# zkHubHQ/distributed-groth16

Hardware: AMD Instinct MI355X
Metric: groth16_constraints_per_sec (higher is better)
Workload: dtype u32; 1 GPU; BN254 Groth16 prove from the matrices, synthetic R1CS with 2^20 - 2 constraints (3 nonzeros per row of A and B), 2^20 wires, 2 instance variables; r, s != 0 (R1CS x witness + 6 NTTs of 2^20 + 4 G1 MSMs + 1 G2 MSM); proving key RESIDENT as window tables (built once per key outside the timed region); curve=bn254, log_domain=20, parallelism=single GPU, key_table_bytes=6039807360, key_table_stride=1

## Files before the change

### distributed-groth16_amd/csrc/capi.hip

```cpp
#include <stdio.h>
#include <stdlib.h>
#include <string.h>

#include "bounds.h"
#include "ctx.h"

using namespace dg16;

namespace dg16 {
size_t fq_bytes(int curve) { return curve == DG16_BN254 ? 32 : 48; }
size_t affine_bytes(int curve, int group) { return 2 * fq_bytes(curve) * (group == 2 ? 2 : 1); }
#ifdef DG16_BOUNDS
unsigned* bounds_sink_device() {
  static unsigned* sink = [] {
    unsigned* p = nullptr;
    if (hipMalloc((void**)&p, kBoundsWords * sizeof(unsigned)) != hipSuccess) return (unsigned*)nullptr;
    (void)hipMemset(p, 0, kBoundsWords * sizeof(unsigned));
    return p;
  }();
  return sink;
}
#endif
static void check_curve_group(int curve, int group) {
  DG_REQUIRE(curve >= 0 && curve <= 2, DG16_ERR_BAD_CURVE, "unknown curve id");
  DG_REQUIRE(group == 1 || group == 2, DG16_ERR_BAD_ARG, "group must be 1 (G1) or 2 (G2)");
}
}

extern "C" {

int dg16_ctx_create(int device, dg16_ctx** out) {
  if (!out) return DG16_ERR_BAD_ARG;
  *out = nullptr;
  dg16_ctx* ctx = new dg16_ctx();
  int rc = guarded(ctx, [&] {
    int count = 0;
    DG_HIP(hipGetDeviceCount(&count));
    DG_REQUIRE(count > 0, DG16_ERR_HIP, "no HIP device visible: libdg16 has no CPU path");
    DG_REQUIRE(device >= 0 && device < count, DG16_ERR_BAD_ARG, "device index out of range");
    DG_HIP(hipSetDevice(device));
    hipDeviceProp_t p;
    DG_HIP(hipGetDeviceProperties(&p, device));
    ctx->device = device;
    ctx->compute_units = p.multiProcessorCount;
    ctx->name = p.gcnArchName;
    int prio_lo = 0, prio_hi = 0;
    DG_HIP(hipDeviceGetStreamPriorityRange(&prio_lo, &prio_hi));
    for (int i = 0; i < kChannels; i++) {
      DG_HIP(hipStreamCreateWithPriority(&ctx->ch[i].own, hipStreamNonBlocking, i > 0 ? prio_hi : prio_lo));
      ctx->ch[i].cur = ctx->ch[i].own;
      for (int e = 0; e < 4; e++) DG_HIP(hipEventCreate(&ctx->ch[i].ev[e]));
    }
    for (auto& e : ctx->pipe_ev) DG_HIP(hipEventCreateWithFlags(&e, hipEventDisableTiming));
    DG_HIP(hipStreamCreateWithPriority(&ctx->aux[0], hipStreamNonBlocking, prio_hi));
    DG_HIP(hipHostMalloc((void**)&ctx->dev_flag_host, sizeof(unsigned), hipHostMallocMapped));
    *ctx->dev_flag_host = 0;
    DG_HIP(hipHostGetDevicePointer((void**)&ctx->dev_flag, ctx->dev_flag_host, 0));
    DG_HIP(hipMalloc((void**)&ctx->kclk, kChannels * 2 * sizeof(unsigned long long)));
    DG_HIP(hipMemset(ctx->kclk, 0, kChannels * 2 * sizeof(unsigned long long)));
  });
  if (rc != DG16_OK) {
    static thread_local std::string last;
    last = ctx->err;
    delete ctx;
    return rc;
  }
  *out = ctx;
  return DG16_OK;
}

void dg16_ctx_destroy(dg16_ctx* ctx) {
  if (!ctx) return;
  hipSetDevice(ctx->device);
  hipDeviceSynchronize();
  for (int i = 0; i < kChannels; i++) {
    for (int s = 0; s < kSlots; s++)
      if (ctx->ch[i].slot[s]) hipFree(ctx->ch[i].slot[s]);
    for (int e = 0; e < 4; e++)
      if (ctx->ch[i].ev[e]) hipEventDestroy(ctx->ch[i].ev[e]);
    if (ctx->ch[i].own) hipStreamDestroy(ctx->ch[i].own);
  }
  for (auto& x : ctx->xws)
    for (int s = 0; s < kSlots; s++)
      if (x.slot[s]) hipFree(x.slot[s]);
  for (auto& e : ctx->pipe_ev)
    if (e) hipEventDestroy(e);
  for (auto& st : ctx->aux)
    if (st) hipStreamDestroy(st);
  if (ctx->dev_flag_host) hipHostFree(ctx->dev_flag_host);
  if (ctx->kclk) hipFree(ctx->kclk);
  for (auto& kv : ctx->twiddles) {
    hipFree(kv.second.lo);
    hipFree(kv.second.hi);
    if (kv.second.hi_scaled) hipFree(kv.second.hi_scaled);
    hipFree(kv.second.small);
    hipFree(kv.second.n_inv);
    for (void* q : {kv.second.lo_i, kv.second.hi_i, kv.second.hi_scaled_i, kv.second.small_i, kv.second.n_inv_i,
                    kv.second.full[0], kv.second.full[1], kv.second.shift_full})
      if (q) hipFree(q);
  }
  delete ctx;
}

const char* dg16_last_error(dg16_ctx* ctx) {
  if (!ctx) return "null context";
  std::lock_guard<std::mutex> g(ctx->mu);
  static thread_local std::string copy;
  copy = ctx->err;
  return copy.c_str();
}

int dg16_set_stream(dg16_ctx* ctx, int channel, void* hip_stream) {
  int rc = guard_channel(ctx, channel);
  if (rc) return rc;
  std::lock_guard<std::mutex> g(ctx->ch[channel].mu);
  ctx->ch[channel].cur = hip_stream ? (hipStream_t)hip_stream : ctx->ch[channel].own;
  return DG16_OK;
}

int dg16_sync(dg16_ctx* ctx, int channel) {
  int rc = guard_channel(ctx, channel);
  if (rc) return rc;
  return guarded(ctx, [&] {
    DG_HIP(hipSetDevice(ctx->device));
    DG_HIP(hipStreamSynchronize(ctx->ch[channel].cur));
    if (ctx->dev_flag_host && *ctx->dev_flag_host) {
      const unsigned f = *ctx->dev_flag_host;
      *ctx->dev_flag_host = 0;
      throw StatusError{DG16_ERR_BAD_ARG, f & 1 ? "dg16_qap: coefficient out of range (column >= num_vars or bad row_ptr)"
                                                : "device-side argument check failed"};
    }
#ifdef DG16_BOUNDS
    if (unsigned* sink = bounds_sink_device()) {
      unsigned rec[kBoundsWords] = {};
      DG_HIP(hipDeviceSynchronize());
      DG_HIP(hipMemcpy(rec, sink, sizeof rec, hipMemcpyDeviceToHost));
      if (rec[0]) {
        DG_HIP(hipMemset(sink, 0, sizeof rec));
        char msg[256];
        snprintf(msg, sizeof msg, "DG16_BOUNDS: %u violation(s); first: site %u index %llu limit %llu (workgroup %u, lane %u)", rec[0],
                 rec[1], (unsigned long long)(rec[2] | ((uint64_t)rec[3] << 32)),
                 (unsigned long long)(rec[4] | ((uint64_t)rec[5] << 32)), rec[6], rec[7]);
        fprintf(stderr, "[dg16] %s\n", msg);
        throw StatusError{DG16_ERR_HIP, msg};
      }
    }
#endif
  });
}

int dg16_device_info(dg16_ctx* ctx, char* name, size_t name_len, int* compute_units) {
  if (!ctx) return DG16_ERR_BAD_ARG;
  if (name && name_len) {
    strncpy(name, ctx->name.c_str(), name_len - 1);
    name[name_len - 1] = 0;
  }
  if (compute_units) *compute_units = ctx->compute_units;
  return DG16_OK;
}

int dg16_last_kernel_ms(dg16_ctx* ctx, int channel, int which, float* ms) {
  int rc = guard_channel(ctx, channel);
  if (rc) return rc;
  if (!ms || which < 0 || which > 2) return DG16_ERR_BAD_ARG;
  return guarded(ctx, [&] {
    Channel& c = ctx->ch[channel];
    std::lock_guard<std::mutex> g(c.mu);
    *ms = 0.f;
    if (which == 2) {
      if (!c.ev_valid[1] || !ctx->kclk) return;
      DG_HIP(hipSetDevice(ctx->device));
      DG_HIP(hipEventSynchronize(c.ev[3]));
      unsigned long long t[2] = {0, 0};
      DG_HIP(hipMemcpy(t, ctx->kclk + 2 * channel, sizeof t, hipMemcpyDeviceToHost));
      if (t[1]) *ms = (float)((double)t[0] / (double)t[1] * 100.0);
      return;
    }
    if (!c.ev_valid[which]) return;
    DG_HIP(hipSetDevice(ctx->device));
    hipEvent_t a = c.ev[which == 0 ? 0 : 2], b = c.ev[which == 0 ? 1 : 3];
    DG_HIP(hipEventSynchronize(b));
    DG_HIP(hipEventElapsedTime(ms, a, b));
  });
}

int dg16_field_op(dg16_ctx* ctx, int field_id, int op, const void* a, const void* b, void* out,
                  size_t n, unsigned flags, int channel) {
  int rc = guard_channel(ctx, channel);
  if (rc) return rc;
  return guarded(ctx, [&] {
    int curve = field_id & 15;
    DG_REQUIRE((field_id & ~16) >= 0 && curve <= 2 && (field_id >> 4) <= 1, DG16_ERR_BAD_CURVE,
               "field id must be curve (Fq) or 16 + curve (Fr)");
    DG_REQUIRE(op >= 0 && op <= 7, DG16_ERR_BAD_ARG, "unknown field op");
    DG_REQUIRE(a && out && (b || op >= 3), DG16_ERR_BAD_ARG, "null operand");
    bool dev = flags & DG16_F_DEVICE_PTRS;
    size_t eb = (field_id & 16) ? 32 : fq_bytes(curve);
    Call k(ctx, channel);
// ... 331 lines not shown
```

### distributed-groth16_amd/csrc/ctx.h

```cpp
#pragma once
#include <hip/hip_runtime.h>
#include <stdint.h>

#include <map>
#include <atomic>
#include <mutex>
#include <string>
#include <vector>

#include "../../include/dg16.h"

namespace dg16 {

constexpr int kChannels = 3;
constexpr int kSlots = 32;

struct Channel {
  hipStream_t own = nullptr;
  hipStream_t cur = nullptr;
  std::mutex mu;
  void* slot[kSlots] = {};
  size_t slot_bytes[kSlots] = {};
  hipEvent_t ev[4] = {};
  bool ev_valid[2] = {false, false};
};

struct TwiddleKey {
  int curve;
  unsigned log_n;
  int inverse;
  bool operator<(const TwiddleKey& o) const {
    if (curve != o.curve) return curve < o.curve;
    if (log_n != o.log_n) return log_n < o.log_n;
    return inverse < o.inverse;
  }
};
struct TwiddleSet {
  void* lo = nullptr;
  void* hi = nullptr;
  void* hi_scaled = nullptr;
  void* small = nullptr;
  void* n_inv = nullptr;
  unsigned lb = 0, sm = 0;
  void *lo_i = nullptr, *hi_i = nullptr, *hi_scaled_i = nullptr, *small_i = nullptr, *n_inv_i = nullptr;
  void* full[2] = {nullptr, nullptr};
  void* shift_full = nullptr;
  bool shift_full_tried = false;
};

}

struct dg16_ctx {
  int device = 0;
  int compute_units = 0;
  std::string name;
  dg16::Channel ch[dg16::kChannels];
  std::mutex mu;
  std::mutex mpc_mu;
  std::string err;
  hipEvent_t pipe_ev[24] = {};
  std::atomic<bool> tail_pending{false};
  hipStream_t aux[1] = {};
  dg16::Channel xws[2];
  unsigned* dev_flag_host = nullptr;
  unsigned* dev_flag = nullptr;
  unsigned long long* kclk = nullptr;
  size_t table_budget = 0;
  std::map<dg16::TwiddleKey, dg16::TwiddleSet> twiddles;
};

struct dg16_bases {
  dg16_ctx* ctx = nullptr;
  int curve = 0, group = 1;
  size_t n = 0;
  unsigned c = 0, nwin = 0;
  unsigned stride = 1;
  void* table = nullptr;
  size_t bytes = 0;
};

namespace dg16 {

struct StatusError {
  int code;
  std::string msg;
};

#define DG_HIP(expr)                                                                        \
  do {                                                                                      \
    hipError_t e_ = (expr);                                                                 \
    if (e_ != hipSuccess)                                                                   \
      throw dg16::StatusError{e_ == hipErrorOutOfMemory ? DG16_ERR_OOM : DG16_ERR_HIP,      \
                              std::string(#expr) + ": " + hipGetErrorString(e_)};           \
  } while (0)

#define DG_REQUIRE(cond, code, text)                                                        \
  do {                                                                                      \
    if (!(cond)) throw dg16::StatusError{code, text};                                       \
  } while (0)

inline void* ws(Channel& c, int slot, size_t bytes) {
  if (bytes == 0) bytes = 16;
  if (c.slot_bytes[slot] < bytes) {
    if (c.slot[slot]) {
      DG_HIP(hipDeviceSynchronize());
      DG_HIP(hipFree(c.slot[slot]));
      c.slot[slot] = nullptr;
      c.slot_bytes[slot] = 0;
    }
    size_t want = bytes + bytes / 8;
    DG_HIP(hipMalloc(&c.slot[slot], want));
    c.slot_bytes[slot] = want;
  }
  return c.slot[slot];
}

struct Call {
  dg16_ctx* ctx;
  Channel& c;
  std::unique_lock<std::mutex> lk;
  Call(dg16_ctx* ctx_, int channel, bool tail_ok = false)
      : ctx(ctx_), c(ctx_->ch[channel]), lk(ctx_->ch[channel].mu) {
    DG_HIP(hipSetDevice(ctx->device));
    if (!tail_ok && ctx->tail_pending.load(std::memory_order_acquire))
      DG_HIP(hipStreamWaitEvent(c.cur, ctx->pipe_ev[18], 0));
    c.ev_valid[0] = c.ev_valid[1] = false;
    DG_HIP(hipEventRecord(c.ev[0], c.cur));
  }
  void begin_dominant() { DG_HIP(hipEventRecord(c.ev[2], c.cur)); }
  void end_dominant() {
    DG_HIP(hipEventRecord(c.ev[3], c.cur));
    c.ev_valid[1] = true;
  }
  void finish() {
    DG_HIP(hipEventRecord(c.ev[1], c.cur));
    c.ev_valid[0] = true;
  }
  hipStream_t s() const { return c.cur; }
};

inline int guard_channel(dg16_ctx* ctx, int channel) {
  if (!ctx) return DG16_ERR_BAD_ARG;
  if (channel < 0 || channel >= kChannels) {
    std::lock_guard<std::mutex> g(ctx->mu);
    ctx->err = "channel must be 0..2";
    return DG16_ERR_BAD_ARG;
  }
  return DG16_OK;
}

template <class Fn>
int guarded(dg16_ctx* ctx, Fn&& fn) {
  try {
    fn();
    return DG16_OK;
  } catch (const StatusError& e) {
    if (ctx) {
      std::lock_guard<std::mutex> g(ctx->mu);
      ctx->err = e.msg;
    }
    return e.code;
  } catch (const std::exception& e) {
    if (ctx) {
      std::lock_guard<std::mutex> g(ctx->mu);
      ctx->err = e.what();
    }
    return DG16_ERR_HIP;
  } catch (...) {
    return DG16_ERR_HIP;
  }
}

inline const void* stage_in(Call& k, int slot, const void* p, size_t bytes, bool device_ptrs) {
  if (device_ptrs || bytes == 0) return p;
  void* d = ws(k.c, slot, bytes);
  DG_HIP(hipMemcpyAsync(d, p, bytes, hipMemcpyHostToDevice, k.s()));
  return d;
}
inline void stage_out(Call& k, void* host_dst, const void* dev_src, size_t bytes, bool device_ptrs) {
  if (device_ptrs) {
    if (host_dst != dev_src) DG_HIP(hipMemcpyAsync(host_dst, dev_src, bytes, hipMemcpyDeviceToDevice, k.s()));
  } else {
    DG_HIP(hipMemcpyAsync(host_dst, dev_src, bytes, hipMemcpyDeviceToHost, k.s()));
  }
}

void field_op_launch(Call& k, int field_id, int op, const void* a, const void* b, void* out, size_t n);
void qap_launch(Call& k, int curve, const unsigned* a_ptr, const unsigned* a_col, const void* a_val,
                const unsigned* b_ptr, const unsigned* b_col, const void* b_val, const void* w, bool w_mont, size_t nc,
                size_t ni, size_t nv, size_t m, size_t row_start, size_t row_stride, void* a, void* b, void* c);
void h_poly_dist_stage(Call& k, int curve, unsigned log_m, unsigned rank, unsigned n_ranks, int stage,
                       const void* const* in, void* out);
void h_poly_dist_launch(Call& k, int curve, const dg16_comm* comm, const void* a, const void* b, const void* c,
                        unsigned log_m, void* out);
void ntt_dist_stage(Call& k, int curve, unsigned log_n_total, unsigned rank, unsigned n_ranks, int inverse, int stage,
                    const void* in, void* out);
void ntt_dist_launch(Call& k, int curve, const dg16_comm* comm, const void* in, void* out, unsigned log_n_total,
                     int inverse);
void ntt_launch(Call& k, int curve, void* data, unsigned log_n, int inverse, const void* coset_host);
void h_poly_launch(Call& k, int curve, const void* a, const void* b, const void* c, unsigned log_m,
                   void* out);
bool net_is_rccl(const dg16_net* net);
inline unsigned msm_mode(unsigned flags) {
  return ((flags & DG16_F_SCALARS_MONT) ? 1u : 0u) | ((flags & DG16_F_BASES_IN_SUBGROUP) ? 2u : 0u);
}
void msm_launch(Call& k, int curve, int group, const void* bases, const void* scalars, size_t n,
                unsigned mode, bool out_affine, void* out_dev);
// ... 11 lines not shown
```

### distributed-groth16_amd/csrc/msm_group.hip

```cpp
#include "msm_impl.h"
#include "dist_impl.h"

#define DG_CAT2(a, b) a##b
#define DG_CAT(a, b) DG_CAT2(a, b)
#define DG_FN(stem) DG_CAT(stem, DG_NAME)

namespace dg16 {
using CT = CurveTypes<DG_CURVE>;
#if DG_GROUP == 1
using GF = CT::Fq;
using GC = CT::G1c;
#else
using GF = CT::Fq2;
using GC = CT::G2c;
#endif

template void msm_accumulate_phase<GF>(hipStream_t, const MsmSort&, const MsmBuffers<GF>&, const void* const*);
template void msm_finalize_phase<GF>(hipStream_t, const MsmSort&, const MsmBuffers<GF>&);
template void msm_tail_phase<GF>(hipStream_t, const MsmSort&, const MsmBuffers<GF>&, bool, void*);
template void* msm_build_table<GF>(hipStream_t, const void*, size_t, unsigned, unsigned);
template MsmSort msm_sort_on<CT::Fr, CT::SCALAR_BITS>(hipStream_t, Channel&, const void*, size_t, unsigned, bool, unsigned,
                                                      unsigned);

void DG_FN(msm_)(Call& k, const void* bases, const void* scalars, size_t n, unsigned mode, bool affine, void* out) {
  msm_run<GF, CT::Fr, CT::SCALAR_BITS>(k, bases, scalars, n, mode, affine, out);
}
void DG_FN(gen_bases_)(Call& k, uint64_t seed, size_t n, void* out) { gen_bases_run<GF, GC>(k, seed, n, out); }
void DG_FN(to_affine_)(Call& k, const void* jac, void* out, size_t n) { to_affine_run<GF>(k, jac, out, n); }

void* DG_FN(bases_table_)(Call& k, const void* bases_dev, size_t n, size_t budget, unsigned* c_out, unsigned* rows_out,
                          unsigned* stride_out) {
  const unsigned c = msm_window_bits(n ? n : 1, true, CT::SCALAR_BITS);
  const unsigned nwin = (CT::SCALAR_BITS + 1 + c - 1) / c;
  const unsigned stride = table_stride_for((size_t)nwin * (n ? n : 1) * sizeof(Affine<GF>), budget, nwin);
  const unsigned rows = (nwin + stride - 1) / stride;
  *c_out = c;
  *rows_out = rows;
  *stride_out = stride;
  return msm_build_table<GF>(k.s(), bases_dev, n, c * stride, rows);
}
void DG_FN(msm_resident_)(Call& k, const void* table, size_t n, unsigned c, unsigned stride, const void* scalars,
                          bool mont, bool affine, void* out) {
  MsmSort st = msm_sort<CT::Fr, CT::SCALAR_BITS>(k, scalars, n, mont, true, c, stride);
  msm_reduce<GF>(k, st, table, affine, out);
}

template <class F, class Fr>
__global__ void __launch_bounds__(512) matvec_points_wave_kernel(const Fr* __restrict__ Mc, unsigned rows, unsigned cols,
                                                                   const Affine<F>* __restrict__ in,
                                                                   Affine<F>* __restrict__ out) {
  __shared__ ScalarMulLds<F> lds[8];
  __shared__ XYZZ29<F> part[8];
  const unsigned wave = threadIdx.x >> 6, lane = threadIdx.x & 63;
  const size_t e = blockIdx.x / rows;
  const unsigned r = blockIdx.x % rows;
  __builtin_amdgcn_s_setprio(DG16_CHAIN_PRIO);
  {
    const Affine<F> q = in[e * cols + wave];
    XYZZ29<F> v = XYZZ29<F>::inf();
    if (!q.is_inf()) v = XYZZ29<F>::from_xyzz32(XYZZ<F>::from_affine(q));
    const Fr k = Mc[(size_t)r * cols + wave];
    v = scalar_mul_wave29<F, Fr::NL, false>(v, k.l, &lds[wave]);
    if (lane == 0) part[wave] = v;
  }
  __syncthreads();
  if (wave != 0) return;
  const Affine<F> acc = sum_points_affine_wave<F>(part, cols);
  if (lane == 0) out[blockIdx.x] = acc;
}
template <class F, class Fr>
static void matvec_points(hipStream_t s, const Fr* Mc, unsigned rows, unsigned cols, const Affine<F>* in, Affine<F>* out,
                          size_t count) {
  if (count * rows <= 256 && cols >= 1 && cols <= 8)
    hipLaunchKernelGGL((matvec_points_wave_kernel<F, Fr>), dim3((unsigned)(count * rows)), dim3(64 * cols), 0, s, Mc, rows, cols,
                       in, out);
  else
    hipLaunchKernelGGL((matvec_points_kernel<F, Fr>), dim3((unsigned)((count * rows + 63) / 64)), dim3(64), 0, s, Mc, rows,
                       cols, in, out, count);
}

void DG_FN(d_msm_)(Call& k, const dg16_pss* pp, const dg16_net* net, int sid, const void* bases, const void* scalars,
                   size_t n, unsigned mode, void* out_jac, const void* table, unsigned table_c, unsigned table_stride) {
  const bool mont = mode & 1u;
  using F = GF;
  using Fr = CT::Fr;
  const unsigned np = pp->n;
  Affine<F>* c_share = (Affine<F>*)ws(k.c, 18, sizeof(Affine<F>));
  if (table)
    DG_FN(msm_resident_)(k, table, n, table_c, table_stride, scalars, mont, true, c_share);
  else
    msm_run<F, Fr, CT::SCALAR_BITS>(k, bases, scalars, n, mode, true, c_share);
  const bool king = net->party_id(net->self) == 0;
  Affine<F>* shares = king ? (Affine<F>*)ws(k.c, 19, np * sizeof(Affine<F>)) : nullptr;
  if (net->gather_to_king(net->self, sid, c_share, sizeof(Affine<F>), shares, k.s()) != DG16_OK)
    throw StatusError{DG16_ERR_NET, "send_to_king failed"};
  Affine<F>* send = nullptr;
  if (king) {
    send = (Affine<F>*)ws(k.c, 20, np * sizeof(Affine<F>));
    const Fr* v2 = (const Fr*)pp->mats + 6 * pp->n * pp->l;
    matvec_points<F, Fr>(k.s(), v2, 1u, np, shares, send, (size_t)1);
    for (unsigned p = 1; p < np; p++)
      DG_HIP(hipMemcpyAsync(send + p, send, sizeof(Affine<F>), hipMemcpyDeviceToDevice, k.s()));
    DG_HIP(hipGetLastError());
  }
  Affine<F>* got = (Affine<F>*)ws(k.c, 21, sizeof(Affine<F>));
  if (net->scatter_from_king(net->self, sid, send, sizeof(Affine<F>), got, k.s()) != DG16_OK)
    throw StatusError{DG16_ERR_NET, "recv_from_king failed"};
  hipLaunchKernelGGL(affine_to_jacobian_kernel<F>, dim3(1), dim3(1), 0, k.s(), got, (Jacobian<F>*)out_jac);
  DG_HIP(hipGetLastError());
}
template <class F, class Fr>
__global__ void __launch_bounds__(512) mpc_combine_kernel(const Jacobian<F>* __restrict__ terms,
                                                           const Fr* __restrict__ scalars, unsigned n_terms,
                                                           unsigned mask, int mont, Jacobian<F>* __restrict__ out) {
  __shared__ XYZZ29<F> part[8];
  __shared__ ScalarMulLds<F> lds[8];
  const unsigned wave = threadIdx.x >> 6, lane = threadIdx.x & 63;
  XYZZ29<F> v = XYZZ29<F>::from_xyzz32(XYZZ<F>::from_jacobian(terms[wave]));
  {
    Fr kk = Fr::zero();
    kk.l[0] = 1;
    if ((mask >> wave) & 1) {
      kk = scalars[wave];
      if (mont) kk = kk.from_mont();
    }
    v = scalar_mul_wave29<F, Fr::NL, false>(v, kk.l, &lds[wave]);
  }
  if (lane == 0) part[wave] = v;
  __syncthreads();
  if (wave != 0) return;
  const XYZZ29<F> acc = sum_points_wave<F>(part, n_terms);
  if (lane == 0) *out = acc.to_xyzz32().to_jacobian();
}
void DG_FN(mpc_combine_)(Call& k, const void* terms, const void* scalars, unsigned n_terms, unsigned mask, bool mont,
                         void* out_jac) {
  DG_REQUIRE(n_terms >= 1 && n_terms <= 8, DG16_ERR_BAD_ARG, "mpc_combine: 1..8 terms");
  hipLaunchKernelGGL((mpc_combine_kernel<GF, CT::Fr>), dim3(1), dim3(64 * n_terms), 0, k.s(), (const Jacobian<GF>*)terms,
                     (const CT::Fr*)scalars, n_terms, mask, (int)mont, (Jacobian<GF>*)out_jac);
  DG_HIP(hipGetLastError());
}
void DG_FN(affine_to_jac_)(Call& k, const void* aff, void* jac) {
  hipLaunchKernelGGL(affine_to_jacobian_kernel<GF>, dim3(1), dim3(1), 0, k.s(), (const Affine<GF>*)aff, (Jacobian<GF>*)jac);
  DG_HIP(hipGetLastError());
}
void DG_FN(packexp_)(Call& k, const dg16_pss* pp, int which, const void* in, size_t count, void* out) {
  using F = GF;
  using Fr = CT::Fr;
  const unsigned cols = which == 0 ? pp->l : pp->n, rows = which == 0 ? pp->n : pp->l;
  const Fr* Mc = (const Fr*)pp->mats + 3 * pp->n * pp->l + (size_t)which * pp->n * pp->l;
  matvec_points<F, Fr>(k.s(), Mc, rows, cols, (const Affine<F>*)in, (Affine<F>*)out, count);
  DG_HIP(hipGetLastError());
}
}
```

### distributed-groth16_amd/csrc/msm_impl.h

```cpp
#pragma once
#include <atomic>
#include <utility>
#include "glv.h"
#include <stdio.h>

#include <chrono>

#include "bounds.h"
#include "ctx.h"
#include "ec29.h"
#include "lane29.h"
#include "types.h"

#ifndef DG16_CHAIN_PRIO
#define DG16_CHAIN_PRIO 3
#endif
namespace dg16 {

constexpr unsigned kMinSegLog = 3, kMaxSegLog = 9;
constexpr unsigned kMinLanesLog = 18;
constexpr unsigned kGiantSegs = 64;
constexpr unsigned kGiantSlices = 64;
constexpr unsigned kGiantSliceSegs = 512;

// ... 126 lines not shown
      v >>= off;
    }
    int d = (int)((unsigned)v & ((1u << c) - 1)) + (int)carry;
    if ((unsigned)d > half) { d -= (int)(1u << c); carry = 1; } else { carry = 0; }
    if (flip) d = -d;
    if (live) digits[(size_t)w * n + i] = d;
    unsigned b = d ? (unsigned)(d < 0 ? -d : d) - 1 : 0u;
    unsigned slot = ((w % g.bw) << g.log_nb) + b;
    wave_atomic_inc(counts, slot, live && d != 0);
  }
}

constexpr unsigned kScanBlock = 4096;
template <int TU>
__global__ void __launch_bounds__(1024) msm_scan_local_kernel(const unsigned* __restrict__ counts,
                                                               unsigned* __restrict__ offsets,
                                                               unsigned* __restrict__ seg_off,
                                                               unsigned* __restrict__ block_tot, unsigned log_nb,
                                                               unsigned seg_log) {
  __shared__ unsigned sh[1024];
  __shared__ unsigned sh2[1024];
  const unsigned nb = 1u << log_nb;
  const unsigned seg_round = (1u << seg_log) - 1;
  const size_t base = (size_t)blockIdx.y << log_nb;
  const unsigned lo = blockIdx.x * kScanBlock + threadIdx.x * 4;
  unsigned cn[4], sum = 0, ssum = 0;
#pragma unroll
  for (unsigned j = 0; j < 4; j++) {
    cn[j] = (lo + j < nb) ? counts[base + lo + j] : 0;
    sum += cn[j];
    ssum += (cn[j] + seg_round) >> seg_log;
  }
  sh[threadIdx.x] = sum;
  sh2[threadIdx.x] = ssum;
  __syncthreads();
  for (unsigned d = 1; d < 1024; d <<= 1) {
    unsigned v = threadIdx.x >= d ? sh[threadIdx.x - d] : 0;
    unsigned v2 = threadIdx.x >= d ? sh2[threadIdx.x - d] : 0;
    __syncthreads();
    sh[threadIdx.x] += v;
    sh2[threadIdx.x] += v2;
    __syncthreads();
  }
  unsigned run = sh[threadIdx.x] - sum, srun = sh2[threadIdx.x] - ssum;
#pragma unroll
  for (unsigned j = 0; j < 4; j++)
    if (lo + j < nb) {
      offsets[base + lo + j] = run;
      seg_off[base + lo + j] = srun;
      run += cn[j];
      srun += (cn[j] + seg_round) >> seg_log;
    }
  if (threadIdx.x == 1023) {
    size_t t = ((size_t)blockIdx.y * gridDim.x + blockIdx.x) * 2;
    block_tot[t] = sh[1023];
    block_tot[t + 1] = sh2[1023];
  }
}
template <int TU>
__global__ void __launch_bounds__(1024) msm_scan_tops_kernel(unsigned* __restrict__ block_tot, unsigned nblocks,
                                                              unsigned* __restrict__ seg_total) {
  __shared__ unsigned sh[1024];
  __shared__ unsigned sh2[1024];
  unsigned* t = block_tot + (size_t)blockIdx.x * nblocks * 2;
  unsigned a = threadIdx.x < nblocks ? t[threadIdx.x * 2] : 0;
  unsigned b = threadIdx.x < nblocks ? t[threadIdx.x * 2 + 1] : 0;
  sh[threadIdx.x] = a;
  sh2[threadIdx.x] = b;
  __syncthreads();
  for (unsigned d = 1; d < 1024; d <<= 1) {
    unsigned v = threadIdx.x >= d ? sh[threadIdx.x - d] : 0;
    unsigned v2 = threadIdx.x >= d ? sh2[threadIdx.x - d] : 0;
    __syncthreads();
    sh[threadIdx.x] += v;
    sh2[threadIdx.x] += v2;
    __syncthreads();
  }
  if (threadIdx.x < nblocks) {
    t[threadIdx.x * 2] = sh[threadIdx.x] - a;
    t[threadIdx.x * 2 + 1] = sh2[threadIdx.x] - b;
  }
  if (threadIdx.x == 1023) seg_total[blockIdx.x] = sh2[1023];
}
template <int TU>
__global__ void __launch_bounds__(1024) msm_scan_fix_kernel(unsigned* __restrict__ offsets,
                                                             unsigned* __restrict__ seg_off,
                                                             unsigned* __restrict__ cursor,
                                                             const unsigned* __restrict__ block_tot, unsigned log_nb) {
  const unsigned nb = 1u << log_nb;
  const size_t base = (size_t)blockIdx.y << log_nb;
  const size_t t = ((size_t)blockIdx.y * gridDim.x + blockIdx.x) * 2;
  const unsigned add = block_tot[t], sadd = block_tot[t + 1];
  const unsigned lo = blockIdx.x * kScanBlock + threadIdx.x * 4;
#pragma unroll
  for (unsigned j = 0; j < 4; j++)
    if (lo + j < nb) {
      offsets[base + lo + j] += add;
      seg_off[base + lo + j] += sadd;
      cursor[base + lo + j] = 0;
    }
}

template <int TU>
__global__ void __launch_bounds__(256) msm_scatter_kernel(const int* __restrict__ digits, size_t n, MsmGeom g,
                                                           const unsigned* __restrict__ offsets,
                                                           const unsigned* __restrict__ seg_off,
                                                           unsigned* __restrict__ cursor,
                                                           unsigned* __restrict__ entries) {
  size_t i = (size_t)blockIdx.x * blockDim.x + threadIdx.x;
  const bool live = i < n;
  const unsigned w = blockIdx.y;
  int d = live ? digits[(size_t)w * n + i] : 0;
  const bool act = d != 0;
  unsigned b = act ? (unsigned)(d < 0 ? -d : d) - 1 : 0u;
  const unsigned bwin = w % g.bw;
  unsigned slot = (bwin << g.log_nb) + b;
  unsigned rank = wave_atomic_inc(cursor, slot, act);
  if (!act) return;
  unsigned ref = (unsigned)((size_t)(w / g.bw) * n + i);
  entries[DG_IDX(15, (size_t)bwin * g.region + offsets[slot] + rank, (size_t)g.bw * g.region)] = ref | (d < 0 ? 0x80000000u : 0u);
}

constexpr unsigned kPartScalars = 1024;
constexpr unsigned kPartMax = 256;
constexpr unsigned kPartMaxLowBits = 12;
constexpr unsigned kPartTileLog = 11;
constexpr unsigned kPartBlocks = 32;

struct PartGeom {
  unsigned low_bits, nparts, nblk1;
};

template <class Fr>
__device__ __forceinline__ int msm_digit(const Fr& s, unsigned w, unsigned c, unsigned& carry) {
  const unsigned half = 1u << (c - 1);
  unsigned bit = w * c;
  unsigned limb = bit >> 5, off = bit & 31;
  uint64_t v = 0;
  if (limb < (unsigned)Fr::NL) {
    v = s.l[limb];
    if (limb + 1 < (unsigned)Fr::NL) v |= (uint64_t)s.l[limb + 1] << 32;
    v >>= off;
  }
  int d = (int)((unsigned)v & ((1u << c) - 1)) + (int)carry;
  if ((unsigned)d > half) { d -= (int)(1u << c); carry = 1; } else { carry = 0; }
  return d;
}

template <class Fr>
__global__ void __launch_bounds__(256) msm_part_hist_kernel(const Fr* __restrict__ scalars, size_t n, int mont,
                                                             MsmGeom g, PartGeom pg,
                                                             unsigned* __restrict__ blockhist) {
  __shared__ unsigned hist[kPartMax];
  hist[threadIdx.x] = 0;
  __syncthreads();
  for (unsigned k = 0; k < kPartScalars / 256; k++) {
    size_t i = (size_t)blockIdx.x * kPartScalars + k * 256 + threadIdx.x;
    if (i >= n) continue;
    Fr s = scalars[i];
    if (mont & 1) s = s.from_mont();
    unsigned carry = 0;
    for (unsigned w = 0; w < g.nwin; w++) {
      int d = msm_digit(s, w, g.c, carry);
      if (d == 0) continue;
      unsigned slot = ((w % g.bw) << g.log_nb) + (unsigned)(d < 0 ? -d : d) - 1;
      atomicAdd(&hist[slot >> pg.low_bits], 1u);
    }
  }
  __syncthreads();
  if (threadIdx.x < pg.nparts) blockhist[(size_t)threadIdx.x * pg.nblk1 + blockIdx.x] = hist[threadIdx.x];
}

template <class Fr>
__global__ void __launch_bounds__(256) msm_part_scatter_kernel(const Fr* __restrict__ scalars, size_t n, int mont,
                                                                MsmGeom g, PartGeom pg,
                                                                const unsigned* __restrict__ blockoff,
                                                                uint2* __restrict__ part) {
  __shared__ unsigned cur[kPartMax];
  if (threadIdx.x < pg.nparts) cur[threadIdx.x] = blockoff[(size_t)threadIdx.x * pg.nblk1 + blockIdx.x];
  __syncthreads();
  for (unsigned k = 0; k < kPartScalars / 256; k++) {
    size_t i = (size_t)blockIdx.x * kPartScalars + k * 256 + threadIdx.x;
    if (i >= n) continue;
    Fr s = scalars[i];
    if (mont & 1) s = s.from_mont();
    const bool flip = (mont & 2) && (s.l[Fr::NL - 1] >> 31);
    unsigned carry = 0;
    for (unsigned w = 0; w < g.nwin; w++) {
      int d = msm_digit(s, w, g.c, carry);
      if (d == 0) continue;
      unsigned slot = ((w % g.bw) << g.log_nb) + (unsigned)(d < 0 ? -d : d) - 1;
      unsigned ref = (unsigned)((size_t)(w / g.bw) * n + i);
      unsigned pos = atomicAdd(&cur[slot >> pg.low_bits], 1u);
      part[DG_IDX(14, pos, (size_t)g.nwin * n)] = make_uint2(ref | (((d < 0) != flip) ? 0x80000000u : 0u), slot);
    }
  }
}

template <int TU>
__global__ void __launch_bounds__(1024) scan_chunk_kernel(unsigned* __restrict__ a, size_t len,
                                                           unsigned* __restrict__ tot) {
  __shared__ unsigned sh[1024];
  const size_t lo = (size_t)blockIdx.x * 4096 + threadIdx.x * 4;
  unsigned v[4], sum = 0;
#pragma unroll
  for (unsigned j = 0; j < 4; j++) {
    v[j] = lo + j < len ? a[lo + j] : 0;
    sum += v[j];
  }
  sh[threadIdx.x] = sum;
  __syncthreads();
  for (unsigned d = 1; d < 1024; d <<= 1) {
    unsigned t = threadIdx.x >= d ? sh[threadIdx.x - d] : 0;
    __syncthreads();
    sh[threadIdx.x] += t;
    __syncthreads();
  }
  unsigned run = sh[threadIdx.x] - sum;
#pragma unroll
  for (unsigned j = 0; j < 4; j++)
    if (lo + j < len) {
      a[lo + j] = run;
      run += v[j];
    }
  if (threadIdx.x == 1023) tot[blockIdx.x] = sh[1023];
}
template <int TU>
__global__ void __launch_bounds__(1024) scan_tops_kernel(unsigned* __restrict__ tot, unsigned nchunks) {
  __shared__ unsigned sh[1024];
  const unsigned per = (nchunks + 1023) / 1024;
  const unsigned lo = threadIdx.x * per;
  unsigned sum = 0;
  for (unsigned j = 0; j < per; j++)
    if (lo + j < nchunks) sum += tot[lo + j];
  sh[threadIdx.x] = sum;
  __syncthreads();
  for (unsigned d = 1; d < 1024; d <<= 1) {
    unsigned t = threadIdx.x >= d ? sh[threadIdx.x - d] : 0;
    __syncthreads();
    sh[threadIdx.x] += t;
    __syncthreads();
  }
  unsigned run = sh[threadIdx.x] - sum;
  for (unsigned j = 0; j < per; j++)
    if (lo + j < nchunks) {
      unsigned t = tot[lo + j];
      tot[lo + j] = run;
      run += t;
    }
}
template <int TU>
__global__ void __launch_bounds__(1024) scan_add_kernel(unsigned* __restrict__ a, size_t len,
                                                         const unsigned* __restrict__ tot) {
  const size_t lo = (size_t)blockIdx.x * 4096 + threadIdx.x * 4;
  const unsigned add = tot[blockIdx.x];
#pragma unroll
  for (unsigned j = 0; j < 4; j++)
    if (lo + j < len) a[lo + j] += add;
}

template <int TU>
__global__ void __launch_bounds__(256) msm_part_count_kernel(const uint2* __restrict__ part,
                                                              const unsigned* __restrict__ blockoff, PartGeom pg,
                                                              unsigned* __restrict__ counts) {
  __shared__ unsigned hist[1u << kPartMaxLowBits];
  const unsigned p = blockIdx.y;
  const unsigned lo = blockoff[(size_t)p * pg.nblk1];
  const unsigned size = blockoff[(size_t)(p + 1) * pg.nblk1] - lo;
  if (((size_t)blockIdx.x << kPartTileLog) >= size) return;
  const unsigned nlow = 1u << pg.low_bits;
  for (unsigned b = threadIdx.x; b < nlow; b += 256) hist[b] = 0;
  __syncthreads();
  for (size_t t = (size_t)blockIdx.x << kPartTileLog; t < size; t += (size_t)gridDim.x << kPartTileLog)
    for (unsigned j = 0; j < (1u << kPartTileLog) / 256; j++) {
      size_t idx = t + j * 256 + threadIdx.x;
      if (idx < size) atomicAdd(&hist[part[lo + idx].y & (nlow - 1)], 1u);
    }
  __syncthreads();
  for (unsigned b = threadIdx.x; b < nlow; b += 256)
    if (hist[b]) atomicAdd(&counts[((size_t)p << pg.low_bits) + b], hist[b]);
}

template <int TU>
__global__ void __launch_bounds__(256) msm_part_place_kernel(const uint2* __restrict__ part,
                                                              const unsigned* __restrict__ blockoff, PartGeom pg,
                                                              MsmGeom g, const unsigned* __restrict__ offsets,
                                                              const unsigned* __restrict__ seg_off,
                                                              unsigned* __restrict__ cursor,
                                                              unsigned* __restrict__ entries) {
  __shared__ unsigned cnt[1u << kPartMaxLowBits];
  __shared__ unsigned rank0[1u << kPartMaxLowBits];
  __shared__ unsigned dst0[1u << kPartMaxLowBits];
  const unsigned p = blockIdx.y;
  const unsigned lo = blockoff[(size_t)p * pg.nblk1];
  const unsigned size = blockoff[(size_t)(p + 1) * pg.nblk1] - lo;
  if (((size_t)blockIdx.x << kPartTileLog) >= size) return;
  const unsigned nlow = 1u << pg.low_bits;
  constexpr unsigned PER = (1u << kPartTileLog) / 256;
  for (size_t t = (size_t)blockIdx.x << kPartTileLog; t < size; t += (size_t)gridDim.x << kPartTileLog) {
    for (unsigned b = threadIdx.x; b < nlow; b += 256) cnt[b] = 0;
    __syncthreads();
    uint2 e[PER];
    unsigned lr[PER];
#pragma unroll
    for (unsigned j = 0; j < PER; j++) {
      size_t idx = t + j * 256 + threadIdx.x;
      e[j] = make_uint2(0u, 0xFFFFFFFFu);
      if (idx < size) {
        e[j] = part[lo + idx];
        lr[j] = atomicAdd(&cnt[e[j].y & (nlow - 1)], 1u);
      }
    }
    __syncthreads();
    for (unsigned b = threadIdx.x; b < nlow; b += 256)
      if (cnt[b]) {
        const size_t slot = ((size_t)p << pg.low_bits) + b;
        rank0[b] = atomicAdd(&cursor[slot], cnt[b]);
        dst0[b] = (unsigned)((slot >> g.log_nb) * g.region) + offsets[slot];
      }
    __syncthreads();
#pragma unroll
    for (unsigned j = 0; j < PER; j++) {
      if (e[j].y == 0xFFFFFFFFu) continue;
      const unsigned slot = e[j].y, b = slot & (nlow - 1);
      const unsigned rank = rank0[b] + lr[j];
      entries[DG_IDX(13, dst0[b] + rank, (size_t)g.bw * g.region)] = e[j].x;
    }
    __syncthreads();
  }
}

template <class F>
__device__ __forceinline__ Affine29<F> load_internal(const uint32_t* __restrict__ bases, unsigned idx) {
  constexpr int PW = 2 * FieldOf<F>::WORDS;
  uint32_t w[PW];
  const uint4* src = reinterpret_cast<const uint4*>(bases + (size_t)idx * PW);
#pragma unroll
  for (int i = 0; i < PW / 4; i++) {
    const uint4 v = src[i];
    w[4 * i] = v.x; w[4 * i + 1] = v.y; w[4 * i + 2] = v.z; w[4 * i + 3] = v.w;
  }
  return Affine29<F>::load(w);
}

template <class F>
struct RawPoint {
  uint4 v[2 * FieldOf<F>::WORDS / 4];
};
template <class F>
__device__ __forceinline__ RawPoint<F> load_raw(const uint32_t* __restrict__ bases, unsigned idx) {
  constexpr int PW = 2 * FieldOf<F>::WORDS;
  RawPoint<F> r;
  const uint4* src = reinterpret_cast<const uint4*>(bases + (size_t)idx * PW);
#pragma unroll
  for (int i = 0; i < PW / 4; i++) r.v[i] = src[i];
  return r;
}
template <class F>
__device__ __forceinline__ Affine29<F> unpack_raw(const RawPoint<F>& r) {
  constexpr int PW = 2 * FieldOf<F>::WORDS;
  uint32_t w[PW];
#pragma unroll
  for (int i = 0; i < PW / 4; i++) {
    w[4 * i] = r.v[i].x; w[4 * i + 1] = r.v[i].y; w[4 * i + 2] = r.v[i].z; w[4 * i + 3] = r.v[i].w;
  }
  return Affine29<F>::load(w);
}

struct SegRange {
  size_t bslot;
  unsigned first, cnt;
  unsigned j, k;
};
__device__ __forceinline__ SegRange msm_segment(const MsmGeom& g, unsigned w, unsigned t,
                                                const unsigned* __restrict__ counts,
                                                const unsigned* __restrict__ seg_off) {
  const unsigned* so = seg_off + ((size_t)w << g.log_nb);
  unsigned lo = 0, hi = 1u << g.log_nb;
  while (hi - lo > 1) {
    const unsigned mid = (lo + hi) >> 1;
    if (so[mid] <= t) lo = mid; else hi = mid;
  }
  SegRange r;
  r.bslot = DG_IDX(1, ((size_t)w << g.log_nb) + lo, (size_t)g.bw << g.log_nb);
  const unsigned c = counts[r.bslot];
  const unsigned k = (c + (1u << g.seg_log) - 1) >> g.seg_log;
  const unsigned j = t - so[lo];
  r.first = (unsigned)(((uint64_t)j * c) / k);
  r.cnt = (unsigned)(((uint64_t)(j + 1) * c) / k) - r.first;
  r.j = j;
  r.k = k;
  return r;
}

__device__ __forceinline__ unsigned msm_nparts(unsigned first_slot, unsigned k, unsigned wg_log) {
  return k ? ((first_slot + k - 1) >> wg_log) - (first_slot >> wg_log) + 1 : 0;
}
__device__ __forceinline__ unsigned msm_part_slot(unsigned first_slot, unsigned s, unsigned wg_log) {
  return s ? ((first_slot >> wg_log) + s) << wg_log : first_slot;
}
template <class F, int BLOCK>
struct ColAcc {
  using S = typename FieldOf<F>::Store;
  static constexpr int WORDS = sizeof(S) / 4;
  uint32_t (*sh)[BLOCK];
  unsigned lane;
  __device__ __forceinline__ S get(int coord) const {
    S v;
    uint32_t* w = reinterpret_cast<uint32_t*>(&v);
#pragma unroll
    for (int i = 0; i < WORDS; i++) w[i] = sh[coord * WORDS + i][lane];
    return v;
  }
  __device__ __forceinline__ void put(int coord, const S& v) const {
    const uint32_t* w = reinterpret_cast<const uint32_t*>(&v);
#pragma unroll
    for (int i = 0; i < WORDS; i++) sh[coord * WORDS + i][lane] = w[i];
  }
};
template <class F, int BLOCK>
#ifdef DG16_TREE_ADD_OUTLINE
__device__ __attribute__((noinline))
#else
__device__ __forceinline__
#endif
void wg_tree_add(uint32_t (*sh)[BLOCK], unsigned a, unsigned b) {
#ifdef DG16_TREE_ADD_INTO
  XYZZ29<F>::add_into(ColAcc<F, BLOCK>{sh, a}, ColAcc<F, BLOCK>{sh, b});
#else
  XYZZ29<F>::add_acc(ColAcc<F, BLOCK>{sh, a}, ColAcc<F, BLOCK>{sh, a}, ColAcc<F, BLOCK>{sh, b});
#endif
}
template <class F, int BLOCK>
__device__ __forceinline__ void wg_bucket_tree(uint32_t (*sh)[BLOCK], unsigned short* list, unsigned* wcnt,
                                                         unsigned lane, unsigned q, unsigned el) {
  constexpr unsigned NW = BLOCK / 64;
  if (lane == 0) wcnt[NW] = 0;
  __syncthreads();
  atomicMax(&wcnt[NW], el - (lane - q));
  __syncthreads();
  const unsigned maxlen = wcnt[NW];
#pragma unroll 1
  for (unsigned d = 1; d < maxlen; d <<= 1) {
    const bool act = (q & (2 * d - 1)) == 0 && lane + d < el;
    const unsigned long long m = __ballot(act);
    const unsigned wv = lane >> 6;
    if ((lane & 63) == 0) wcnt[wv] = (unsigned)__popcll(m);
    __syncthreads();
    unsigned base = 0, total = 0;
#pragma unroll
    for (unsigned i = 0; i < NW; i++) {
      const unsigned c = wcnt[i];
      base += i < wv ? c : 0u;
      total += c;
    }
    if (act) list[base + (unsigned)__popcll(m & ((1ull << (lane & 63)) - 1))] = (unsigned short)lane;
    __syncthreads();
    if (lane < total) {
      const unsigned a = list[lane];
      wg_tree_add<F, BLOCK>(sh, a, (unsigned)DG_IDX(16, a + d, BLOCK));
    }
    __syncthreads();
  }
}

constexpr unsigned kMaxInst = 4;
struct MsmBases {
  const uint32_t* p[kMaxInst];
};
template <class F>
constexpr bool msm_acc_tree();
template <class F>
constexpr unsigned msm_acc_block_log() {
  if constexpr (sizeof(F) > 48) return sizeof(typename FieldOf<F>::Store) * 4 * 256 <= 80 * 1024 ? 8u : 7u;
  else if constexpr (!msm_acc_tree<F>()) return 8u;
#ifdef DG16_G1_BLOCK_LOG
  else return DG16_G1_BLOCK_LOG;
#else
  else return sizeof(typename FieldOf<F>::Store) * 4 * 256 <= 40 * 1024 ? 8u : 7u;
#endif
}
// ... 868 lines not shown
      w[4] = 0;
      const bool neg_half = ((lane ? h[1][7] : h[0][7]) >> 31) != 0;
      len = wnaf4_words<5>(w, 128, neg_half, lds->naf[lane]);
    }
    __syncthreads();
    {
      Fp<P> beta32;
#pragma unroll
      for (int i = 0; i < Fp<P>::NL; i++) beta32.l[i] = GC::BETA[i];
      const uint32_t beta = FO::template from_regs<XYZZ29<F>::BS>(kc, FieldOf<F>::from32(beta32));
      const uint32_t* src = reinterpret_cast<const uint32_t*>(&lds->tab[kc.row]);
      uint32_t* dst = reinterpret_cast<uint32_t*>(&lds->tab[4 + kc.row]);
      const bool on = kc.l16 < 9u;
      const unsigned i = on ? kc.l16 : 0u;
      const uint32_t bx = lane29::mul(kc, on ? src[i] : 0u, beta);
      if (on) {
        dst[i] = bx;
        dst[9 + i] = src[9 + i];
        dst[18 + i] = src[18 + i];
        dst[27 + i] = src[27 + i];
      }
    }
    len = max(__shfl(len, 0), __shfl(len, 1));
  } else {
    if (lane == 0) len = wnaf4_words<NW>(k, NW * 32, false, lds->naf[0]);
    len = __shfl(len, 0);
  }
  __syncthreads();
  LPt acc = lane29::inf_pt<FO>(kc);
#pragma unroll 1
  for (int i = len - 1; i >= 0; i--) {
    acc = lane29::dbl_pt<FO>(kc, acc);
#pragma unroll 1
    for (int hf = 0; hf < (SPLIT ? 2 : 1); hf++) {
      const int d = lds->naf[hf][i];
      if (d == 0) continue;
      LPt o = lane29::load_pt<F>(kc, &lds->tab[4 * hf + ((d < 0 ? -d : d) >> 1)]);
      if (d < 0) o = lane29::neg_pt<FO>(kc, o);
      acc = lane29::add_pt<FO>(kc, acc, o);
    }
  }
  return p_inf ? p_in : lane29::from_pt<F>(kc, acc);
}
template <class F, int NW>
__device__ __forceinline__ XYZZ29<F> scalar_mul_two_waves_lane29(const XYZZ29<F>& p_in, const uint32_t* k,
                                                                 ScalarMulLds<F>* lds, XYZZ29<F>* xchg) {
  using P = typename FieldOf<F>::Params;
  using GC = typename GlvOf<F>::C;
  using FO = lane29::Ops<F>;
  using LPt = lane29::Pt<FO>;
  static_assert(!FO::EXT, "the endomorphism split of a cofactor-one G1");
  const unsigned lane = __lane_id(), h = (threadIdx.x >> 6) & 1u;
  typename FO::KT kc;
  kc.init();
  const bool p_inf = p_in.is_inf();
  LPt p = lane29::to_pt<F>(kc, p_in);
  if (p_inf) p = {FO::one(kc), FO::one(kc), FO::one(kc), FO::one(kc), false};
  {
    Fp<P> beta32;
#pragma unroll
    for (int i = 0; i < Fp<P>::NL; i++) beta32.l[i] = GC::BETA[i];
    const uint32_t beta = FO::template from_regs<XYZZ29<F>::BS>(kc, FieldOf<F>::from32(beta32));
    if (h) p.x = lane29::mul(kc, p.x, beta);
    const LPt p2 = lane29::dbl_pt<FO>(kc, p);
    LPt m = p;
#pragma unroll 1
    for (int j = 0; j < 4; j++) {
      if (j) m = lane29::add_pt<FO>(kc, m, p2);
      lane29::store_pt_raw<F>(kc, &lds->tab[4 * h + j], m);
    }
  }
  uint32_t hv[2][8];
  glv::split<GC>(k, hv[0], hv[1]);
  int len = 0;
  if (lane == 0) {
    uint32_t w[5];
#pragma unroll
    for (int i = 0; i < 4; i++) w[i] = h ? hv[1][i] : hv[0][i];
    w[4] = 0;
    len = wnaf4_words<5>(w, 128, ((h ? hv[1][7] : hv[0][7]) >> 31) != 0, lds->naf[h]);
  }
  len = __shfl(len, 0);
  __syncthreads();
  LPt acc = lane29::inf_pt<FO>(kc);
#pragma unroll 1
  for (int i = len - 1; i >= 0; i--) {
    acc = lane29::dbl_pt<FO>(kc, acc);
    const int d = lds->naf[h][i];
    if (d == 0) continue;
    LPt o = lane29::load_pt<F>(kc, &lds->tab[4 * h + ((d < 0 ? -d : d) >> 1)]);
    if (d < 0) o = lane29::neg_pt<FO>(kc, o);
    acc = lane29::add_pt<FO>(kc, acc, o);
  }
  if (h == 1) lane29::store_pt_raw<F>(kc, xchg, acc);
  __syncthreads();
  if (h == 0) acc = lane29::add_pt<FO>(kc, acc, lane29::load_pt<F>(kc, xchg));
  return p_inf ? p_in : lane29::from_pt<F>(kc, acc);
}
template <class F>
__device__ __forceinline__ XYZZ29<F> sum_points_wave(const XYZZ29<F>* pts, unsigned n) {
  if constexpr (lane29::enabled<F>()) {
    using FO = lane29::Ops<F>;
    typename FO::KT kc;
    kc.init();
    lane29::Pt<FO> acc = lane29::inf_pt<FO>(kc);
#pragma unroll 1
    for (unsigned i = 0; i < n; i++) acc = lane29::add_pt<FO>(kc, acc, lane29::load_pt<F>(kc, &pts[i]));
    return lane29::from_pt<F>(kc, acc);
  } else {
    XYZZ29<F> acc = XYZZ29<F>::inf();
#pragma unroll 1
    for (unsigned i = 0; i < n; i++) acc = add_wave29(acc, pts[i]);
    return acc;
  }
}

template <class F>
__device__ __forceinline__ Affine<F> sum_points_affine_wave(const XYZZ29<F>* pts, unsigned n) {
  if constexpr (lane29::enabled<F>()) {
    using FO = lane29::Ops<F>;
    typename FO::KT kc;
    kc.init();
    lane29::Pt<FO> acc = lane29::inf_pt<FO>(kc);
#pragma unroll 1
    for (unsigned i = 0; i < n; i++) acc = lane29::add_pt<FO>(kc, acc, lane29::load_pt<F>(kc, &pts[i]));
    return lane29::to_affine<F>(kc, acc);
  } else {
    return sum_points_wave<F>(pts, n).to_xyzz32().to_affine();
  }
}

constexpr unsigned kRowLog = 8;
struct RowGeom {
  unsigned row_log;
  unsigned rows_log;
};
inline RowGeom row_geometry(const MsmGeom& g) {
  RowGeom r;
  r.row_log = g.log_nb < kRowLog ? g.log_nb : kRowLog;
  r.rows_log = g.log_nb - r.row_log;
  return r;
}

struct MsmSort {
  MsmGeom g;
  size_t n = 0;
  int* digits = nullptr;
  unsigned *entries = nullptr, *counts = nullptr, *offsets = nullptr, *seg_off = nullptr, *cursor = nullptr;
  unsigned* seg_total = nullptr;
};

template <class Fr, int SCALAR_BITS>
MsmSort msm_sort_on(hipStream_t s, Channel& wsch, const void* scalars, size_t n, unsigned scalars_mont, bool table,
                    unsigned c_fixed, unsigned stride);
template <class Fr, int SCALAR_BITS>
MsmSort msm_sort(Call& k, const void* scalars, size_t n, unsigned scalars_mont, bool table, unsigned c_fixed = 0,
                 unsigned stride = 1) {
  return msm_sort_on<Fr, SCALAR_BITS>(k.s(), k.c, scalars, n, scalars_mont, table, c_fixed, stride);
}
template <class Fr, int SCALAR_BITS>
MsmSort msm_sort_on(hipStream_t s, Channel& wsch, const void* scalars, size_t n, unsigned scalars_mont, bool table,
                    unsigned c_fixed, unsigned stride) {
  MsmSort r;
  DG_BOUNDS_BIND();
  r.n = n;
  r.g = msm_geometry(n ? n : 1, SCALAR_BITS, table, c_fixed, stride);
  const MsmGeom& g = r.g;
  const size_t nbw = (size_t)g.bw << g.log_nb;
  DG_REQUIRE((size_t)g.nwin * n < ((size_t)1 << 31), DG16_ERR_BAD_ARG, "W * n must be < 2^31");
  unsigned lg_nbw = 0;
  while (((size_t)1 << lg_nbw) < nbw) lg_nbw++;
  static const int force_path = [] { const char* e = getenv("DG16_MSM_SORT"); return e ? atoi(e) : 0; }();
  PartGeom pg;
  pg.low_bits = lg_nbw > 8 ? lg_nbw - 8 : 0;
  const bool partitioned = pg.low_bits <= kPartMaxLowBits &&
                           (force_path == 2 || (force_path != 1 && (size_t)g.nwin * n >= ((size_t)1 << 18)));
  pg.nparts = (unsigned)((nbw + ((size_t)1 << pg.low_bits) - 1) >> pg.low_bits);
  pg.nblk1 = (unsigned)((n + kPartScalars - 1) / kPartScalars);
  r.digits = (int*)ws(wsch, 4, (size_t)g.nwin * n * (partitioned ? 8 : 4));
  r.entries = (unsigned*)ws(wsch, 5, (size_t)g.nwin * n * 4);
  unsigned* tabs = (unsigned*)ws(wsch, 6, (nbw * 4 + g.bw) * 4);
  r.counts = tabs;
  r.offsets = r.counts + nbw;
  r.seg_off = r.offsets + nbw;
  r.cursor = r.seg_off + nbw;
  r.seg_total = r.cursor + nbw;
  unsigned* blockoff = nullptr;
  if (n && partitioned) {
    const size_t len = (size_t)pg.nparts * pg.nblk1 + 1;
    blockoff = (unsigned*)ws(wsch, 25, (len + (unsigned)((len + 4095) / 4096)) * 4);
  }
  const unsigned scan_nblocks = ((1u << g.log_nb) + kScanBlock - 1) / kScanBlock;
  unsigned* block_tot = (unsigned*)ws(wsch, 9, (size_t)g.bw * scan_nblocks * 2 * 4);
  DG_HIP(hipMemsetAsync(r.counts, 0, nbw * 4, s));
  uint2* part = (uint2*)r.digits;
  if (n && partitioned) {
    const size_t len = (size_t)pg.nparts * pg.nblk1 + 1;
    const unsigned nchunks = (unsigned)((len + 4095) / 4096);
    unsigned* tot = blockoff + len;
    DG_HIP(hipMemsetAsync(blockoff + len - 1, 0, 4, s));
    hipLaunchKernelGGL(msm_part_hist_kernel<Fr>, dim3(pg.nblk1), dim3(256), 0, s, (const Fr*)scalars, n,
                       (int)scalars_mont, g, pg, blockoff);
    hipLaunchKernelGGL(scan_chunk_kernel<0>, dim3(nchunks), dim3(1024), 0, s, blockoff, len, tot);
    hipLaunchKernelGGL(scan_tops_kernel<0>, dim3(1), dim3(1024), 0, s, tot, nchunks);
    hipLaunchKernelGGL(scan_add_kernel<0>, dim3(nchunks), dim3(1024), 0, s, blockoff, len, tot);
    hipLaunchKernelGGL(msm_part_scatter_kernel<Fr>, dim3(pg.nblk1), dim3(256), 0, s, (const Fr*)scalars, n,
                       (int)scalars_mont, g, pg, blockoff, part);
    hipLaunchKernelGGL(msm_part_count_kernel<0>, dim3(kPartBlocks, pg.nparts), dim3(256), 0, s, part, blockoff, pg,
                       r.counts);
  } else if (n) {
    hipLaunchKernelGGL(msm_digits_kernel<Fr>, dim3((unsigned)((n + 255) / 256)), dim3(256), 0, s, (const Fr*)scalars,
                       n, (int)scalars_mont, g, r.digits, r.counts);
  }
  {
    const unsigned nblocks = ((1u << g.log_nb) + kScanBlock - 1) / kScanBlock;
    hipLaunchKernelGGL(msm_scan_local_kernel<0>, dim3(nblocks, g.bw), dim3(1024), 0, s, r.counts, r.offsets,
                       r.seg_off, block_tot, g.log_nb, g.seg_log);
    hipLaunchKernelGGL(msm_scan_tops_kernel<0>, dim3(g.bw), dim3(1024), 0, s, block_tot, nblocks, r.seg_total);
    hipLaunchKernelGGL(msm_scan_fix_kernel<0>, dim3(nblocks, g.bw), dim3(1024), 0, s, r.offsets, r.seg_off, r.cursor,
                       block_tot, g.log_nb);
  }
  if (n && partitioned)
    hipLaunchKernelGGL(msm_part_place_kernel<0>, dim3(kPartBlocks, pg.nparts), dim3(256), 0, s, part, blockoff, pg, g,
                       r.offsets, r.seg_off, r.cursor, r.entries);
  else if (n)
    hipLaunchKernelGGL(msm_scatter_kernel<0>, dim3((unsigned)((n + 255) / 256), g.nwin), dim3(256), 0, s, r.digits, n, g,
                       r.offsets, r.seg_off, r.cursor, r.entries);
  DG_HIP(hipGetLastError());
  return r;
}

constexpr size_t kLaneReduceMaxBuckets = 32768;
template <class F>
inline bool lane_reduce_applies(size_t buckets_over_all_windows) {
  if constexpr (!lane29::enabled<F>()) return false;
  else {
    static const bool off = [] { const char* e = getenv("DG16_NO_LANE_REDUCE"); return e && atoi(e) != 0; }();
    return !off && buckets_over_all_windows <= kLaneReduceMaxBuckets;
  }
}
template <class F>
struct MsmBuffers {
  XYZZ29<F>* buckets;
  XYZZ29<F>* seg_sum;
  XYZZ29<F>* row_w;
  XYZZ29<F>* row_r;
  XYZZ29<F>* fold;
  XYZZ29<F>* window_sums;
  XYZZ29<F>* lane_tmp;
  XYZZ29<F>* top_tmp;
  hipStream_t finalize_stream = nullptr;
  bool busy_chip = false;
  unsigned* giant;
  unsigned giant_cap;
  size_t nbw, nrows;
  unsigned ninst;
  RowGeom rg;
  unsigned long long* clk = nullptr;
  hipEvent_t acc_done = nullptr;
};

template <class F>
MsmBuffers<F> msm_buffers(Channel& wsch, const MsmGeom& g, unsigned ninst = 1) {
  MsmBuffers<F> b;
  DG_REQUIRE(ninst >= 1 && ninst <= kMaxInst, DG16_ERR_BAD_ARG, "1..4 MSM instances per sort");
  b.ninst = ninst;
  const size_t bwi = (size_t)g.bw * ninst;
  b.nbw = bwi << g.log_nb;
  const size_t nseg_slots = bwi * g.seg_cap;
  b.giant_cap = (unsigned)(nseg_slots / kGiantSegs + 1);
  DG_REQUIRE(nseg_slots / kGiantSegs + 1 < ((size_t)1 << 26), DG16_ERR_BAD_ARG, "giant list: id slot must fit 26 bits");
  static_assert(kGiantSlices <= 64, "a work item keeps its slice in six bits");
  static_assert(kGiantSliceSegs >= kGiantSegs, "work items <= 2 giant_cap needs slices no shorter than kGiantSegs partials");
  DG_REQUIRE(nseg_slots / kGiantSliceSegs + 1 + b.giant_cap <= 2 * (size_t)b.giant_cap + 1, DG16_ERR_BAD_ARG,
             "giant list: work-item capacity");
  b.buckets = (XYZZ29<F>*)ws(wsch, 7, b.nbw * sizeof(XYZZ29<F>));
  b.seg_sum = (XYZZ29<F>*)ws(wsch, 17, nseg_slots * sizeof(XYZZ29<F>));
  b.rg = row_geometry(g);
  b.nrows = bwi << b.rg.rows_log;
  const size_t nfold = bwi * 3 * 256;
  const size_t nlane = lane_reduce_applies<F>(b.nbw) ? b.nbw / 2 + 4 : 0;
  const size_t ntop = lane29::enabled<F>() ? bwi * 96 + 8 : 0;
  uint8_t* p15 = (uint8_t*)ws(wsch, 15, (2 * b.nrows + nfold + bwi + nlane + ntop) * sizeof(XYZZ29<F>));
  b.row_w = (XYZZ29<F>*)p15;
  b.row_r = b.row_w + b.nrows;
  b.fold = b.row_r + b.nrows;
  b.window_sums = b.fold + nfold;
  b.lane_tmp = nlane ? b.window_sums + bwi : nullptr;
  b.top_tmp = ntop ? b.window_sums + bwi + nlane : nullptr;
  b.giant = (unsigned*)ws(wsch, 10, ((size_t)b.giant_cap * 3 + 2) * 4);
  return b;
}

inline int msm_finalize_lds_lpb();
template <class F>
struct MsmBuffers;
template <class F>
void msm_finalize_lds_phase(hipStream_t s, const MsmSort& st, const MsmBuffers<F>& b);
template <class F>
void msm_accumulate_phase(hipStream_t s, const MsmSort& st, const MsmBuffers<F>& b, const void* const* bases) {
  const MsmGeom& g = st.g;
  DG_BOUNDS_BIND();
  MsmBases mb{};
  for (unsigned i = 0; i < b.ninst; i++) mb.p[i] = (const uint32_t*)bases[i];
  if (b.clk) DG_HIP(hipMemsetAsync(b.clk, 0, 16, s));
  if constexpr (sizeof(F) > 48) {
    constexpr int BLOCK = 1 << msm_acc_block_log<F>();
    const dim3 grid((g.seg_cap + BLOCK - 1) / BLOCK, g.bw * b.ninst);
    if constexpr (sizeof(F) > 64) {
      hipLaunchKernelGGL((msm_accumulate_steps_kernel<F, BLOCK>), grid, dim3(BLOCK), 0, s, mb, st.n, g, st.offsets,
                         st.counts, st.seg_off, st.seg_total, st.entries, b.seg_sum, b.buckets, b.clk);
    } else {
      hipLaunchKernelGGL((msm_accumulate_lds_kernel<F, BLOCK>), grid, dim3(BLOCK), 0, s, mb, st.n, g, st.offsets, st.counts,
                         st.seg_off, st.seg_total, st.entries, b.seg_sum, b.buckets, b.clk);
    }
    if (b.acc_done) DG_HIP(hipEventRecord(b.acc_done, s));
    if (b.finalize_stream && b.acc_done) {
      DG_HIP(hipStreamWaitEvent(b.finalize_stream, b.acc_done, 0));
      msm_finalize_lds_phase<F>(b.finalize_stream, st, b);
    } else {
      msm_finalize_lds_phase<F>(s, st, b);
    }
  } else {
    constexpr int BLOCK = 1 << msm_acc_block_log<F>();
    hipLaunchKernelGGL((msm_accumulate_kernel<F, BLOCK>), dim3((g.seg_cap + BLOCK - 1) / BLOCK, g.bw * b.ninst),
                       dim3(BLOCK), 0, s, mb, st.n, g, st.offsets, st.counts, st.seg_off, st.seg_total, st.entries,
                       b.seg_sum, b.buckets, b.clk);
    if (b.acc_done) DG_HIP(hipEventRecord(b.acc_done, s));
  }
  DG_HIP(hipGetLastError());
}
template <class F>
void msm_accumulate_phase(hipStream_t s, const MsmSort& st, const MsmBuffers<F>& b, const void* bases) {
  const void* one[1] = {bases};
  msm_accumulate_phase<F>(s, st, b, one);
}

template <class F>
__global__ void __launch_bounds__(64) msm_tail_kernel(const XYZZ29<F>* __restrict__ window_sums, MsmGeom g,
                                                       int affine, F* __restrict__ out) {
  __builtin_amdgcn_s_setprio(DG16_CHAIN_PRIO);
  window_sums += (size_t)blockIdx.x * g.bw;
  out += (size_t)blockIdx.x * (affine ? 2 : 3);
  XYZZ29<F> acc = XYZZ29<F>::inf();
  if constexpr (lane29::enabled<F>()) {
    using FO = lane29::Ops<F>;
    typename FO::KT kc;
    kc.init();
    lane29::Pt<FO> a = lane29::inf_pt<FO>(kc);
#pragma unroll 1
    for (int w = (int)g.bw - 1; w >= 0; w--) {
#pragma unroll 1
      for (unsigned k = 0; k < g.c; k++) a = lane29::dbl_pt<FO>(kc, a);
      a = lane29::add_pt<FO>(kc, a, lane29::load_pt<F>(kc, &window_sums[w]));
    }
    if (affine) {
      const Affine<F> r = lane29::to_affine<F>(kc, a);
      if (threadIdx.x == 0) {
        out[0] = r.x;
        out[1] = r.y;
      }
      return;
    }
    acc = lane29::from_pt<F>(kc, a);
  } else {
#pragma unroll 1
    for (int w = (int)g.bw - 1; w >= 0; w--) {
#pragma unroll 1
      for (unsigned k = 0; k < g.c; k++) acc = dbl_wave29(acc);
      acc = add_wave29(acc, window_sums[w]);
    }
  }
  if (threadIdx.x != 0) return;
  using FO = FieldOf<F>;
  if (affine) {
    Affine<F> a = acc.to_xyzz32().to_affine();
    out[0] = a.x;
    out[1] = a.y;
  } else if (acc.is_inf()) {
    out[0] = F::one();
    out[1] = F::one();
    out[2] = F::zero();
  } else {
    out[0] = FO::to32(fit<FO::BS>(acc.x * acc.zz));
    out[1] = FO::to32(fit<FO::BS>(acc.y * acc.zzz));
    out[2] = FO::to32(acc.zz);
  }
}

template <class F>
void msm_tail_phase(hipStream_t s, const MsmSort& st, const MsmBuffers<F>& b, bool out_affine, void* out_dev) {
  hipLaunchKernelGGL(msm_tail_kernel<F>, dim3(b.ninst), dim3(64), 0, s, b.window_sums, st.g, (int)out_affine, (F*)out_dev);
}

__device__ __forceinline__ void giant_geometry(unsigned nseg, unsigned& slices, unsigned& per) {
  slices = (nseg + kGiantSliceSegs - 1) / kGiantSliceSegs;
  if (slices > kGiantSlices) slices = kGiantSlices;
  per = (nseg + slices - 1) / slices;
  slices = (nseg + per - 1) / per;
}
__device__ __forceinline__ void msm_register_giant(unsigned gid, unsigned np, unsigned* __restrict__ giant_count,
                                                   unsigned* __restrict__ giant_list, unsigned giant_cap) {
  const unsigned slot = atomicAdd(giant_count, 1u);
  if (!DG_OK(8, slot, giant_cap) || slot >= giant_cap) return;
  giant_list[slot] = gid;
  unsigned slices, per;
  giant_geometry(np, slices, per);
  const unsigned wb = atomicAdd(giant_count + 1, slices);
  if (!DG_OK(9, (size_t)wb + slices, 2 * (size_t)giant_cap + 1) || (size_t)wb + slices > 2 * (size_t)giant_cap) return;
  unsigned* work = giant_list + giant_cap;
  for (unsigned i = 0; i < slices; i++) work[wb + i] = (slot << 6) | i;
}


template <class F, int TU = 0>
__global__ void __launch_bounds__(256) msm_finalize_thr_kernel(MsmGeom g, size_t total, unsigned wg_log,
                                                                const unsigned* __restrict__ counts,
                                                                const unsigned* __restrict__ seg_off,
                                                                const XYZZ29<F>* __restrict__ seg_sum,
                                                                XYZZ29<F>* __restrict__ buckets,
                                                                unsigned* __restrict__ giant_count,
                                                                unsigned* __restrict__ giant_list, unsigned giant_cap) {
  const size_t gid = (size_t)blockIdx.x * blockDim.x + threadIdx.x;
  if (gid >= total) return;
  const unsigned wy = (unsigned)(gid >> g.log_nb);
  const size_t gs = ((size_t)(wy % g.bw) << g.log_nb) + (gid & (((size_t)1 << g.log_nb) - 1));
  const unsigned k = (counts[gs] + (1u << g.seg_log) - 1) >> g.seg_log;
  const unsigned first = seg_off[gs];
  const unsigned np = msm_nparts(first, k, wg_log);
  if (np == 0) {
    buckets[gid] = XYZZ29<F>::inf();
    return;
  }
  if (np == 1) return;
  if (np > kGiantSegs) {
    msm_register_giant((unsigned)gid, np, giant_count, giant_list, giant_cap);
    return;
  }
  const XYZZ29<F>* sp = seg_sum + (size_t)wy * g.seg_cap;
  XYZZ29<F> acc = sp[DG_IDX(7, first, g.seg_cap)];
#pragma unroll 1
  for (unsigned s = 1; s < np; s++) acc = acc.add(sp[DG_IDX(7, msm_part_slot(first, s, wg_log), g.seg_cap)]);
  buckets[gid] = acc;
}
constexpr size_t kLaneFinalizeMaxPartials = (size_t)1 << 18;
template <class F>
__global__ void __launch_bounds__(64) msm_finalize_lane_kernel(MsmGeom g, unsigned wg_log,
                                                                const unsigned* __restrict__ counts,
                                                                const unsigned* __restrict__ seg_off,
                                                                const XYZZ29<F>* __restrict__ seg_sum,
                                                                XYZZ29<F>* __restrict__ buckets,
                                                                unsigned* __restrict__ giant_count,
                                                                unsigned* __restrict__ giant_list, unsigned giant_cap) {
  if constexpr (lane29::enabled<F>()) {
    using FO = lane29::Ops<F>;
    using LPt = lane29::Pt<FO>;
    const size_t gid = blockIdx.x;
    const unsigned wy = (unsigned)(gid >> g.log_nb);
    const size_t gs = ((size_t)(wy % g.bw) << g.log_nb) + (gid & (((size_t)1 << g.log_nb) - 1));
    const unsigned k = (counts[gs] + (1u << g.seg_log) - 1) >> g.seg_log;
    const unsigned first = seg_off[gs];
    const unsigned np = msm_nparts(first, k, wg_log);
    if (np == 0) {
      if (threadIdx.x == 0) buckets[gid] = XYZZ29<F>::inf();
      return;
    }
    if (np == 1) return;
    if (np > kGiantSegs) {
      if (threadIdx.x == 0) msm_register_giant((unsigned)gid, np, giant_count, giant_list, giant_cap);
      return;
    }
    typename FO::KT kc;
    kc.init();
    const XYZZ29<F>* sp = seg_sum + (size_t)wy * g.seg_cap;
    LPt acc = lane29::load_pt<F>(kc, &sp[DG_IDX(7, first, g.seg_cap)]);
    LPt nx = lane29::load_pt_words<F>(kc, &sp[DG_IDX(7, msm_part_slot(first, 1, wg_log), g.seg_cap)]);
#pragma unroll 1
    for (unsigned s = 1; s < np; s++) {
      const LPt cur = lane29::with_inf_flag<FO>(nx);
      if (s + 1 < np) nx = lane29::load_pt_words<F>(kc, &sp[DG_IDX(7, msm_part_slot(first, s + 1, wg_log), g.seg_cap)]);
      acc = lane29::add_pt<FO>(kc, acc, cur);
    }
    lane29::store_pt<F>(kc, &buckets[gid], acc);
  }
}
template <class F, int BLOCK>
struct PartialAcc {
  using S = typename FieldOf<F>::Store;
  const XYZZ29<F>* p;
  ColAcc<F, BLOCK> col;
  __device__ __forceinline__ S get(int coord) const {
    if (p) return coord == 0 ? p->x : coord == 1 ? p->y : coord == 2 ? p->zz : p->zzz;
    return col.get(coord);
  }
  __device__ __forceinline__ void launder() { asm volatile("" : "+v"(p)); }
};
template <class F, int BLOCK>
__global__ void __launch_bounds__(BLOCK, (BLOCK == 256 ? 2 : 1))
msm_finalize_lds_kernel(MsmGeom g, size_t total, unsigned wg_log, unsigned lpb_log,
                        const unsigned* __restrict__ counts,
                        const unsigned* __restrict__ seg_off, const XYZZ29<F>* __restrict__ seg_sum,
                        XYZZ29<F>* __restrict__ buckets, unsigned* __restrict__ giant_count,
                        unsigned* __restrict__ giant_list, unsigned giant_cap) {
  using FO = FieldOf<F>;
  constexpr int WORDS = sizeof(typename FO::Store) / 4;
  __shared__ uint32_t sh[4 * WORDS][BLOCK];
  __shared__ unsigned max_serial;
  if constexpr (sizeof(F) > 64) asm volatile("" ::: DG_ACC_FILE_CLOBBERS);
  const unsigned LPB = 1u << lpb_log;
  const unsigned lane = threadIdx.x, sub = lane & (LPB - 1);
  const size_t gid = ((size_t)blockIdx.x * BLOCK + lane) >> lpb_log;
  const ColAcc<F, BLOCK> me{sh, lane};
  unsigned np = 0, first = 0;
  unsigned wy = 0;
  if (lane == 0) max_serial = 0;
  if (gid < total) {
    wy = (unsigned)(gid >> g.log_nb);
    const size_t gs = DG_IDX(6, ((size_t)(wy % g.bw) << g.log_nb) + (gid & (((size_t)1 << g.log_nb) - 1)), (size_t)g.bw << g.log_nb);
    const unsigned k = (counts[gs] + (1u << g.seg_log) - 1) >> g.seg_log;
    first = seg_off[gs];
    np = msm_nparts(first, k, wg_log);
    if (sub == 0) {
      if (np == 0) buckets[gid] = XYZZ29<F>::inf();
      if (np > kGiantSegs) msm_register_giant((unsigned)gid, np, giant_count, giant_list, giant_cap);
    }
  }
  const bool work = np >= 2 && np <= kGiantSegs;
  const XYZZ29<F>* sp = seg_sum + (size_t)wy * g.seg_cap;
  const unsigned lo = work ? (unsigned)(((uint64_t)sub * np) >> lpb_log) : 0u;
  const unsigned hi = work ? (unsigned)(((uint64_t)(sub + 1) * np) >> lpb_log) : 0u;
  if (lo < hi) {
    const XYZZ29<F>* q = &sp[DG_IDX(7, msm_part_slot(first, lo, wg_log), g.seg_cap)];
    me.put(0, q->x); me.put(1, q->y); me.put(2, q->zz); me.put(3, q->zzz);
  } else {
    me.put(2, FO::zero());
  }
  const unsigned nser = lo < hi ? hi - lo - 1 : 0u;
  __syncthreads();
  atomicMax(&max_serial, nser);
  __syncthreads();
  const unsigned ms = max_serial;
#pragma unroll 1
  for (unsigned step = 0; step < ms + lpb_log; step++) {
    const bool tree = step >= ms;
    if (tree) __syncthreads();
    const unsigned d = tree ? 1u << (step - ms) : 0u;
    const bool on = tree ? (work && (sub & (2 * d - 1)) == 0) : step < nser;
    if (on) {
      const PartialAcc<F, BLOCK> b{tree ? nullptr : &sp[DG_IDX(7, msm_part_slot(first, lo + 1 + step, wg_log), g.seg_cap)],
                                   ColAcc<F, BLOCK>{sh, (unsigned)DG_IDX(10, lane + d, BLOCK)}};
      if constexpr (sizeof(F) > 64) xyzz_add_into_steps<F>(me, b);
      else XYZZ29<F>::add_into(me, b);
    }
  }
  if (work && sub == 0) {
    XYZZ29<F> out = XYZZ29<F>::inf();
    if (!limbs_all_zero(me.get(2))) out = XYZZ29<F>{me.get(0), me.get(1), me.get(2), me.get(3)};
    buckets[gid] = out;
  }
}
inline int msm_finalize_lds_lpb() { return 2; }
template <class F>
void msm_finalize_lds_phase(hipStream_t s, const MsmSort& st, const MsmBuffers<F>& b) {
  constexpr int BLOCK = 1 << msm_acc_block_log<F>();
  const int lpb = msm_finalize_lds_lpb();
  const unsigned lpb_log = lpb == 4 ? 2u : lpb == 2 ? 1u : 0u;
  DG_HIP(hipMemsetAsync(b.giant, 0, 8, s));
  const unsigned blocks = (unsigned)((b.nbw * (size_t)lpb + BLOCK - 1) / BLOCK);
  hipLaunchKernelGGL((msm_finalize_lds_kernel<F, BLOCK>), dim3(blocks), dim3(BLOCK), 0, s, st.g, b.nbw,
                     msm_acc_wg_log<F>(), lpb_log, st.counts, st.seg_off, b.seg_sum, b.buckets, b.giant, b.giant + 2,
                     b.giant_cap);
}

template <class F, int TU = 0>
__global__ void __launch_bounds__(256) msm_stitch_kernel(MsmGeom g, unsigned wg_log, const unsigned* __restrict__ counts,
                                                          const unsigned* __restrict__ seg_off,
                                                          const unsigned* __restrict__ seg_total,
                                                          const XYZZ29<F>* __restrict__ seg_sum,
                                                          XYZZ29<F>* __restrict__ buckets,
                                                          unsigned* __restrict__ giant_count,
                                                          unsigned* __restrict__ giant_list, unsigned giant_cap) {
  const unsigned wy = blockIdx.y, w = wy % g.bw;
  const unsigned bd = blockIdx.x * blockDim.x + threadIdx.x + 1;
  const unsigned slot = bd << wg_log;
  if (slot >= seg_total[w]) return;
  const unsigned* so = seg_off + ((size_t)w << g.log_nb);
  unsigned lo = 0, hi = 1u << g.log_nb;
  while (hi - lo > 1) {
    const unsigned mid = (lo + hi) >> 1;
    if (so[mid] <= slot) lo = mid; else hi = mid;
  }
  const unsigned first = so[lo];
  if (first == slot || (first >> wg_log) != bd - 1) return;
  const size_t gs = ((size_t)w << g.log_nb) + lo;
  const size_t gid = ((size_t)wy << g.log_nb) + lo;
  const unsigned k = (counts[gs] + (1u << g.seg_log) - 1) >> g.seg_log;
  const unsigned np = msm_nparts(first, k, wg_log);
  if (np > kGiantSegs) {
    msm_register_giant((unsigned)gid, np, giant_count, giant_list, giant_cap);
    return;
  }
  const XYZZ29<F>* sp = seg_sum + (size_t)wy * g.seg_cap;
  XYZZ29<F> acc = sp[DG_IDX(7, first, g.seg_cap)];
#pragma unroll 1
  for (unsigned s = 1; s < np; s++) acc = acc.add(sp[DG_IDX(7, msm_part_slot(first, s, wg_log), g.seg_cap)]);
  buckets[gid] = acc;
}
template <class F>
__global__ void __launch_bounds__(256) msm_empty_buckets_kernel(MsmGeom g, size_t total, const unsigned* __restrict__ counts,
                                                                 XYZZ29<F>* __restrict__ buckets) {
  const size_t gid = (size_t)blockIdx.x * blockDim.x + threadIdx.x;
  if (gid >= total) return;
  const unsigned wy = (unsigned)(gid >> g.log_nb);
  const size_t gs = ((size_t)(wy % g.bw) << g.log_nb) + (gid & (((size_t)1 << g.log_nb) - 1));
  if (counts[gs]) return;
  uint4* dst = reinterpret_cast<uint4*>(buckets + gid);
  static_assert(sizeof(XYZZ29<F>) % 16 == 0, "vector stores");
#pragma unroll
  for (unsigned i = 0; i < sizeof(XYZZ29<F>) / 16; i++) dst[i] = make_uint4(0u, 0u, 0u, 0u);
}
template <class F>
void msm_finalize_phase(hipStream_t s, const MsmSort& st, const MsmBuffers<F>& b) {
  DG_BOUNDS_BIND();
  if constexpr (msm_acc_tree<F>()) {
    hipLaunchKernelGGL(msm_empty_buckets_kernel<F>, dim3((unsigned)((b.nbw + 255) / 256)), dim3(256), 0, s, st.g, b.nbw,
                       st.counts, b.buckets);
    const unsigned nbd = (st.g.seg_cap >> msm_acc_wg_log<F>()) + 1;
    hipLaunchKernelGGL(msm_stitch_kernel<F>, dim3((nbd + 255) / 256, st.g.bw * b.ninst), dim3(256), 0, s, st.g,
                       msm_acc_wg_log<F>(), st.counts, st.seg_off, st.seg_total, b.seg_sum, b.buckets, b.giant,
                       b.giant + 2, b.giant_cap);
  } else {
    bool lane = false;
    if constexpr (lane29::enabled<F>()) {
      static const bool off = [] { const char* e = getenv("DG16_NO_LANE_FINALIZE"); return e && atoi(e) != 0; }();
      const size_t partials = ((st.g.region * st.g.bw * b.ninst) >> st.g.seg_log) + b.nbw;
      lane = !off && !b.busy_chip && partials <= kLaneFinalizeMaxPartials && b.nbw < ((size_t)1 << 31);
    }
    if (lane)
      hipLaunchKernelGGL(msm_finalize_lane_kernel<F>, dim3((unsigned)b.nbw), dim3(64), 0, s, st.g, msm_acc_wg_log<F>(),
                         st.counts, st.seg_off, b.seg_sum, b.buckets, b.giant, b.giant + 2, b.giant_cap);
    else
      hipLaunchKernelGGL(msm_finalize_thr_kernel<F>, dim3((unsigned)((b.nbw + 255) / 256)), dim3(256), 0, s, st.g, b.nbw,
                         msm_acc_wg_log<F>(), st.counts, st.seg_off, b.seg_sum, b.buckets, b.giant, b.giant + 2,
                         b.giant_cap);
  }
  DG_HIP(hipGetLastError());
}

template <class F>
void msm_bucket_phase(hipStream_t s, const MsmSort& st, const MsmBuffers<F>& b, bool out_affine, void* out_dev);

template <class F>
void msm_reduce(Call& k, const MsmSort& st, const void* bases, bool out_affine, void* out_dev) {
  MsmBuffers<F> b = msm_buffers<F>(k.c, st.g);
  k.begin_dominant();
  b.acc_done = k.c.ev[3];
  if (k.ctx->kclk) b.clk = k.ctx->kclk + 2 * (&k.c - k.ctx->ch);
  msm_accumulate_phase<F>(k.s(), st, b, bases);
  k.c.ev_valid[1] = true;
  msm_bucket_phase<F>(k.s(), st, b, out_affine, out_dev);
}

template <class F> struct GlvOf { static constexpr bool enabled = false; };
template <class F> struct GlvCofactorOne { static constexpr bool value = false; };
template <> struct GlvCofactorOne<Fp<bn254_fq_params>> { static constexpr bool value = true; };
template <class P, class GC>
struct GlvG1 {
  static constexpr bool enabled = true;
  static constexpr int DIM = 2;
  using C = GC;
  DG_HD static void endo(Affine<Fp<P>>& p) {
    Fp<P> beta;
#pragma unroll
    for (int k = 0; k < Fp<P>::NL; k++) beta.l[k] = GC::BETA[k];
    p.x = p.x * beta;
  }
};
template <> struct GlvOf<Fp<bn254_fq_params>> : GlvG1<bn254_fq_params, bn254_glv_consts> {};
template <> struct GlvOf<Fp<bls12_381_fq_params>> : GlvG1<bls12_381_fq_params, bls12_381_glv_consts> {};
template <> struct GlvOf<Fp<bls12_377_fq_params>> : GlvG1<bls12_377_fq_params, bls12_377_glv_consts> {};
template <class P, class GC, int D>
struct GlvG2 {
  static constexpr bool enabled = true;
  static constexpr int DIM = D;
  using C = GC;
  using Fq = Fp<P>;
  DG_HD static void endo(Affine<Fp2<Fq>>& p) {
    if (p.is_inf()) return;
    Fp2<Fq> gx, gy;
#pragma unroll
    for (int k = 0; k < Fq::NL; k++) {
      gx.c0.l[k] = GC::GAMMA_X_C0[k]; gx.c1.l[k] = GC::GAMMA_X_C1[k];
      gy.c0.l[k] = GC::GAMMA_Y_C0[k]; gy.c1.l[k] = GC::GAMMA_Y_C1[k];
    }
    p.x = Fp2<Fq>{p.x.c0, p.x.c1.neg()} * gx;
    p.y = Fp2<Fq>{p.y.c0, p.y.c1.neg()} * gy;
  }
};
template <> struct GlvOf<Fp2<Fp<bn254_fq_params>>> : GlvG2<bn254_fq_params, bn254_g2_glv_consts, 2> {};
template <> struct GlvOf<Fp2<Fp<bls12_381_fq_params>>> : GlvG2<bls12_381_fq_params, bls12_381_g2_glv4_consts, 4> {};
template <> struct GlvOf<Fp2<Fp<bls12_377_fq_params>>> : GlvG2<bls12_377_fq_params, bls12_377_g2_glv4_consts, 4> {};
constexpr int kGlvBits = 127;
constexpr int kGlv4Bits = 65;

template <class Fr, class GC>
__global__ void __launch_bounds__(256) glv_split_kernel(const Fr* __restrict__ scalars, size_t n, int mont,
                                                         Fr* __restrict__ halves ) {
  const size_t i = (size_t)blockIdx.x * blockDim.x + threadIdx.x;
  if (i >= n) return;
  Fr s = scalars[i];
  if (mont) s = s.from_mont();
  Fr h1, h2;
  glv::split<GC>(s.l, h1.l, h2.l);
  halves[i] = h1;
  halves[n + i] = h2;
}
template <class Fr, class GC>
__global__ void __launch_bounds__(256) glv_split4_kernel(const Fr* __restrict__ scalars, size_t n, int mont,
                                                          Fr* __restrict__ quarters ) {
  const size_t i = (size_t)blockIdx.x * blockDim.x + threadIdx.x;
  if (i >= n) return;
  Fr s = scalars[i];
  if (mont) s = s.from_mont();
  Fr h0, h1, h2, h3;
  glv::split4<GC>(s.l, h0.l, h1.l, h2.l, h3.l);
  quarters[i] = h0;
  quarters[n + i] = h1;
  quarters[2 * n + i] = h2;
  quarters[3 * n + i] = h3;
}
template <class F>
__global__ void __launch_bounds__(256) msm_to_internal_glv_kernel(const Affine<F>* __restrict__ in, size_t n,
                                                                   uint32_t* __restrict__ out) {
  const size_t i = (size_t)blockIdx.x * blockDim.x + threadIdx.x;
  if (i >= n) return;
  constexpr int PW = 2 * FieldOf<F>::WORDS;
  Affine<F> p = in[i];
  uint32_t w[PW];
  affine_to_internal(p, w);
  uint4* dst = reinterpret_cast<uint4*>(out + i * PW);
#pragma unroll
  for (int k = 0; k < PW / 4; k++) dst[k] = make_uint4(w[4 * k], w[4 * k + 1], w[4 * k + 2], w[4 * k + 3]);
#pragma unroll 1
  for (int img = 1; img < GlvOf<F>::DIM; img++) {
    GlvOf<F>::endo(p);
    affine_to_internal(p, w);
    dst = reinterpret_cast<uint4*>(out + ((size_t)img * n + i) * PW);
#pragma unroll
    for (int k = 0; k < PW / 4; k++) dst[k] = make_uint4(w[4 * k], w[4 * k + 1], w[4 * k + 2], w[4 * k + 3]);
  }
}

template <class F, class Fr, int SCALAR_BITS>
void msm_run(Call& k, const void* bases, const void* scalars, size_t n, unsigned mode, bool out_affine,
             void* out_dev) {
  const bool scalars_mont = mode & 1u;
  if (GlvOf<F>::enabled && (GlvCofactorOne<F>::value || (mode & 2u))) {
   if constexpr (GlvOf<F>::enabled) {
    constexpr size_t DIM = GlvOf<F>::DIM;
    if (n && DIM * n * 40 < ((size_t)1 << 31)) {
      using GC = typename GlvOf<F>::C;
      Fr* halves = (Fr*)ws(k.c, 30, DIM * n * sizeof(Fr));
      MsmSort st;
      if constexpr (DIM == 2) {
        hipLaunchKernelGGL((glv_split_kernel<Fr, GC>), dim3((unsigned)((n + 255) / 256)), dim3(256), 0, k.s(),
                           (const Fr*)scalars, n, (int)scalars_mont, halves);
        unsigned c_small = 0;
        {
          const unsigned c0 = msm_window_bits(2 * n, false);
          if constexpr (RR<typename FieldOf<F>::Params>::N == 9)
            if ((c0 == 7 || c0 == 9) && !getenv("DG16_MSM_C")) c_small = 8;
          if ((c0 == 14 || c0 == 15) && !getenv("DG16_MSM_C")) c_small = 16;
        }
        st = msm_sort<Fr, kGlvBits>(k, halves, 2 * n, 2u, false, c_small);
      } else {
        hipLaunchKernelGGL((glv_split4_kernel<Fr, GC>), dim3((unsigned)((n + 255) / 256)), dim3(256), 0, k.s(),
                           (const Fr*)scalars, n, (int)scalars_mont, halves);
        st = msm_sort<Fr, kGlv4Bits>(k, halves, 4 * n, 2u, false);
      }
      uint32_t* internal = (uint32_t*)ws(k.c, 24, DIM * n * sizeof(Affine<F>));
      hipLaunchKernelGGL(msm_to_internal_glv_kernel<F>, dim3((unsigned)((n + 255) / 256)), dim3(256), 0, k.s(),
                         (const Affine<F>*)bases, n, internal);
// ... 23 lines not shown
    for (unsigned w = 1; w < nwin; w++) put((size_t)w * n + i, p);
    return;
  }
  XYZZ<F> pts[kMaxTableWin];
  F pref[kMaxTableWin];
  XYZZ<F> cur = XYZZ<F>::from_affine(p);
  F run = F::one();
  for (unsigned w = 1; w < nwin; w++) {
    for (unsigned j = 0; j < c; j++) cur = cur.dbl();
    pts[w] = cur;
    pref[w] = run;
    run = run * (cur.is_inf() ? F::one() : cur.zzz);
  }
  F inv = run.inv();
  for (unsigned w = nwin - 1; w >= 1; w--) {
    if (pts[w].is_inf()) { put((size_t)w * n + i, Affine<F>::inf()); continue; }
    F zi3 = inv * pref[w];
    inv = inv * pts[w].zzz;
    F zi2 = (zi3 * pts[w].zz).sqr();
    put((size_t)w * n + i, Affine<F>{pts[w].x * zi2, pts[w].y * zi3});
  }
}

inline unsigned table_stride_for(size_t full_bytes, size_t budget, unsigned nwin) {
  if (!budget || full_bytes <= budget || nwin <= 1) return 1;
  const size_t row = full_bytes / nwin;
  size_t rows_fit = budget / (row ? row : 1);
  if (rows_fit < 1) rows_fit = 1;
  unsigned k = (unsigned)((nwin + rows_fit - 1) / rows_fit);
  return k < 1 ? 1 : k > nwin ? nwin : k;
}
template <class F>
void* msm_build_table(hipStream_t s, const void* bases, size_t n, unsigned c, unsigned nwin) {
  DG_REQUIRE(nwin <= kMaxTableWin, DG16_ERR_BAD_ARG, "too many table windows");
  void* t = nullptr;
  DG_HIP(hipMalloc(&t, (size_t)nwin * (n ? n : 1) * sizeof(Affine<F>)));
  if (n)
    hipLaunchKernelGGL(msm_table_kernel<F>, dim3((unsigned)((n + 63) / 64)), dim3(64), 0, s, (const Affine<F>*)bases, n,
                       c, nwin, (Affine<F>*)t);
  DG_HIP(hipGetLastError());
  return t;
}

constexpr unsigned kGenChunk = 64;

template <class F, class C>
__global__ void gen_setup_kernel(const uint32_t* k1_words, Affine<F>* d_out) {
  Affine<F> G = GenLoader<F, C>::get();
  XYZZ<F> d = scalar_mul<F, 4>(XYZZ<F>::from_affine(G), k1_words);
  *d_out = d.to_affine();
}

template <class F, class C>
__global__ void __launch_bounds__(64) gen_bases_kernel(const uint32_t* k0_words, const uint32_t* k1_words,
                                                        const Affine<F>* d_ptr, size_t n, Affine<F>* out) {
  size_t t = (size_t)blockIdx.x * blockDim.x + threadIdx.x;
  size_t lo = t * kGenChunk;
  if (lo >= n) return;
  size_t hi = lo + kGenChunk < n ? lo + kGenChunk : n;
  uint32_t kk[8] = {0, 0, 0, 0, 0, 0, 0, 0};
  {
    uint32_t lo_w[2] = {(uint32_t)lo, (uint32_t)((uint64_t)lo >> 32)};
    uint64_t acc[8] = {0, 0, 0, 0, 0, 0, 0, 0};
    for (int i = 0; i < 4; i++)
      for (int j = 0; j < 2; j++) {
        uint64_t pr = (uint64_t)k1_words[i] * lo_w[j];
        acc[i + j] += (uint32_t)pr;
        acc[i + j + 1] += pr >> 32;
      }
    for (int i = 0; i < 4; i++) acc[i] += k0_words[i];
    uint64_t carry = 0;
    for (int i = 0; i < 8; i++) {
      uint64_t v = acc[i] + carry;
      kk[i] = (uint32_t)v;
      carry = v >> 32;
    }
  }
  Affine<F> G = GenLoader<F, C>::get();
  Affine<F> D = *d_ptr;
  XYZZ<F> cur = scalar_mul<F, 7>(XYZZ<F>::from_affine(G), kk);
  XYZZ<F> pts[kGenChunk];
  F pref[kGenChunk];
  F run = F::one();
  size_t cnt = hi - lo;
  for (size_t i = 0; i < cnt; i++) {
    pts[i] = cur;
    pref[i] = run;
    run = run * cur.zzz;
    cur = cur.madd(D, false);
  }
  F inv = run.inv();
  for (size_t i = cnt; i-- > 0;) {
    F zi3 = inv * pref[i];
    inv = inv * pts[i].zzz;
    F zi2 = (zi3 * pts[i].zz).sqr();
    out[lo + i] = {pts[i].x * zi2, pts[i].y * zi3};
  }
}

template <class F, class C>
void gen_bases_run(Call& k, uint64_t seed, size_t n, void* out_dev);

template <class F>
__global__ void __launch_bounds__(64) to_affine_kernel(const Jacobian<F>* __restrict__ in, Affine<F>* __restrict__ out,
                                                        size_t n) {
  size_t i = (size_t)blockIdx.x * blockDim.x + threadIdx.x;
  if (i >= n) return;
  out[i] = XYZZ<F>::from_jacobian(in[i]).to_affine();
}

inline uint64_t splitmix64(uint64_t x) {
  x += 0x9E3779B97F4A7C15ULL;
  x = (x ^ (x >> 30)) * 0xBF58476D1CE4E5B9ULL;
  x = (x ^ (x >> 27)) * 0x94D049BB133111EBULL;
  return x ^ (x >> 31);
}

template <class F, class C>
void gen_bases_run(Call& k, uint64_t seed, size_t n, void* out_dev) {
  uint64_t k0[2] = {splitmix64(seed ^ 0xA5A5), splitmix64(seed ^ 0x5A5A)};
  uint64_t k1[2] = {splitmix64(seed ^ 0x1234) | 1, splitmix64(seed ^ 0x4321)};
  uint32_t host_words[8] = {(uint32_t)k0[0], (uint32_t)(k0[0] >> 32), (uint32_t)k0[1], (uint32_t)(k0[1] >> 32),
                            (uint32_t)k1[0], (uint32_t)(k1[0] >> 32), (uint32_t)k1[1], (uint32_t)(k1[1] >> 32)};
  uint8_t* scratch = (uint8_t*)ws(k.c, 16, 64 + sizeof(Affine<F>));
  uint32_t* words = (uint32_t*)scratch;
  Affine<F>* d = (Affine<F>*)(scratch + 64);
  DG_HIP(hipMemcpyAsync(words, host_words, sizeof host_words, hipMemcpyHostToDevice, k.s()));
  DG_HIP(hipStreamSynchronize(k.s()));
  hipLaunchKernelGGL((gen_setup_kernel<F, C>), dim3(1), dim3(1), 0, k.s(), words + 4, d);
  size_t threads = (n + kGenChunk - 1) / kGenChunk;
  hipLaunchKernelGGL((gen_bases_kernel<F, C>), dim3((unsigned)((threads + 63) / 64)), dim3(64), 0, k.s(), words,
                     words + 4, d, n, (Affine<F>*)out_dev);
  DG_HIP(hipGetLastError());
}

template <class F>
void to_affine_run(Call& k, const void* jac, void* out, size_t n) {
  hipLaunchKernelGGL(to_affine_kernel<F>, dim3((unsigned)((n + 63) / 64)), dim3(64), 0, k.s(),
                     (const Jacobian<F>*)jac, (Affine<F>*)out, n);
  DG_HIP(hipGetLastError());
}

}

#define DG16_MSM_EXTERN_GROUP(F)                                                                                  \
  extern template void msm_accumulate_phase<F>(hipStream_t, const MsmSort&, const MsmBuffers<F>&, const void* const*); \
  extern template void msm_finalize_phase<F>(hipStream_t, const MsmSort&, const MsmBuffers<F>&);                   \
  extern template void msm_tail_phase<F>(hipStream_t, const MsmSort&, const MsmBuffers<F>&, bool, void*);         \
  extern template void* msm_build_table<F>(hipStream_t, const void*, size_t, unsigned, unsigned);
#define DG16_MSM_EXTERN(CT)                                                                                       \
  DG16_MSM_EXTERN_GROUP(CT::Fq)                                                                                   \
  DG16_MSM_EXTERN_GROUP(CT::Fq2)                                                                                  \
  extern template MsmSort msm_sort_on<CT::Fr, CT::SCALAR_BITS>(hipStream_t, Channel&, const void*, size_t, unsigned, bool, \
                                                              unsigned, unsigned);
```

### distributed-groth16_amd/csrc/msm_reduce_impl.h

```cpp
#pragma once
#include "msm_impl.h"

#ifndef DG16_REDUCE_PRIO
#define DG16_REDUCE_PRIO 0
#endif
namespace dg16 {


template <class T>
__device__ __forceinline__ T lane_xor_words(const T& v, int mask) {
  static_assert(sizeof(T) % 4 == 0, "word-sized type");
  T r;
  const uint32_t* src = reinterpret_cast<const uint32_t*>(&v);
  uint32_t* dst = reinterpret_cast<uint32_t*>(&r);
#pragma unroll
  for (unsigned i = 0; i < sizeof(T) / 4; i++) dst[i] = (uint32_t)__shfl_xor((int)src[i], mask);
  return r;
}

template <class F>
__global__ void __launch_bounds__(256) msm_giant_kernel(MsmGeom g, unsigned wg_log, const unsigned* __restrict__ counts,
                                                         const unsigned* __restrict__ seg_off,
                                                         XYZZ29<F>* __restrict__ seg_sum,
                                                         const unsigned* __restrict__ giant_count,
                                                         const unsigned* __restrict__ giant_list, unsigned giant_cap) {
  __builtin_amdgcn_s_setprio(DG16_REDUCE_PRIO);
  __shared__ XYZZ29<F> sh[256];
  unsigned nwork = giant_count[1];
  if (nwork > 2 * giant_cap) nwork = 2 * giant_cap;
  const unsigned* work = giant_list + giant_cap;
  for (unsigned wi = blockIdx.x; wi < nwork; wi += gridDim.x) {
    const unsigned item = work[wi];
    const unsigned gid = giant_list[DG_IDX(11, item >> 6, giant_cap)], slice = item & 63;
    const unsigned wy = gid >> g.log_nb;
    const size_t gs = ((size_t)(wy % g.bw) << g.log_nb) + (gid & ((1u << g.log_nb) - 1));
    const unsigned k = (counts[gs] + (1u << g.seg_log) - 1) >> g.seg_log, first = seg_off[gs];
    const unsigned nseg = msm_nparts(first, k, wg_log);
    unsigned slices, per;
    giant_geometry(nseg, slices, per);
    XYZZ29<F>* sp = seg_sum + (size_t)wy * g.seg_cap;
    const unsigned lo = slice * per;
    const unsigned hi = lo + per < nseg ? lo + per : nseg;
    sh[threadIdx.x] = XYZZ29<F>::inf();
    __syncthreads();
    const unsigned iters = (hi - lo + 255) >> 8;
#pragma unroll 1
    for (unsigned step = 0; step < iters + 8; step++) {
      const XYZZ29<F>* b;
      bool on;
      if (step < iters) {
        const unsigned s = lo + step * 256 + threadIdx.x;
        on = s < hi;
        b = &sp[DG_IDX(12, msm_part_slot(first, on ? s : lo, wg_log), g.seg_cap)];
      } else {
        const unsigned stride = 128u >> (step - iters);
        on = threadIdx.x < stride;
        b = &sh[(threadIdx.x + stride) & 255];
      }
      if (on) XYZZ29<F>::add_mem(&sh[threadIdx.x], &sh[threadIdx.x], b);
      __syncthreads();
    }
    if (threadIdx.x == 0) sp[DG_IDX(12, msm_part_slot(first, lo, wg_log), g.seg_cap)] = sh[0];
    __syncthreads();
  }
}

template <class F>
__global__ void __launch_bounds__(64) msm_giant_fold_kernel(MsmGeom g, unsigned wg_log, const unsigned* __restrict__ counts,
                                                             const unsigned* __restrict__ seg_off,
                                                             const XYZZ29<F>* __restrict__ seg_sum,
                                                             XYZZ29<F>* __restrict__ buckets,
                                                             const unsigned* __restrict__ giant_count,
                                                             const unsigned* __restrict__ giant_list,
                                                             unsigned giant_cap) {
  __builtin_amdgcn_s_setprio(DG16_REDUCE_PRIO);
  __shared__ XYZZ29<F> sh[kGiantSlices];
  unsigned ng = *giant_count;
  if (ng > giant_cap) ng = giant_cap;
  for (unsigned gi = blockIdx.x; gi < ng; gi += gridDim.x) {
    const unsigned gid = giant_list[gi];
    const unsigned wy = gid >> g.log_nb;
    const size_t gs = ((size_t)(wy % g.bw) << g.log_nb) + (gid & ((1u << g.log_nb) - 1));
    const unsigned k = (counts[gs] + (1u << g.seg_log) - 1) >> g.seg_log, first = seg_off[gs];
    const unsigned nseg = msm_nparts(first, k, wg_log);
    unsigned slices, per;
    giant_geometry(nseg, slices, per);
    const XYZZ29<F>* sp = seg_sum + (size_t)wy * g.seg_cap;
    sh[threadIdx.x] = threadIdx.x < slices ? sp[DG_IDX(12, msm_part_slot(first, threadIdx.x * per, wg_log), g.seg_cap)] : XYZZ29<F>::inf();
    __syncthreads();
#pragma unroll 1
    for (unsigned stride = kGiantSlices / 2; stride > 0; stride >>= 1) {
      if (threadIdx.x < stride) XYZZ29<F>::add_mem(&sh[threadIdx.x], &sh[threadIdx.x], &sh[threadIdx.x + stride]);
      __syncthreads();
    }
    if (threadIdx.x == 0) buckets[gid] = sh[0];
    __syncthreads();
  }
}


constexpr unsigned kCoopTreeMax = 64;
template <class F>
__device__ __forceinline__ void tree_step_coop(XYZZ29<F>* sh, unsigned base, unsigned d) {
  const unsigned row16 = (threadIdx.x >> 4) & 15u;
#pragma unroll 1
  for (unsigned i = row16; i < d; i += 16) {
    const XYZZ29<F> v = add_wave29(sh[base + i], sh[base + i + d]);
    if ((threadIdx.x & 15u) == 0) sh[base + i] = v;
  }
}

template <class F>
__global__ void __launch_bounds__(256) msm_row_kernel(MsmGeom g, RowGeom rg, const XYZZ29<F>* __restrict__ buckets,
                                                       XYZZ29<F>* __restrict__ row_w, XYZZ29<F>* __restrict__ row_r) {
  __builtin_amdgcn_s_setprio(DG16_REDUCE_PRIO);
  __shared__ XYZZ29<F> sh[256];
  const unsigned c = threadIdx.x, row = 1u << rg.row_log;
  const size_t rid = ((size_t)blockIdx.y << rg.rows_log) + blockIdx.x;
  sh[c] = c < row ? buckets[(rid << rg.row_log) + c] : XYZZ29<F>::inf();
  __syncthreads();
#pragma unroll 1
  for (unsigned step = 0; step < 2 * rg.row_log; step++) {
    const bool scan = step < rg.row_log;
    const unsigned d = scan ? 1u << step : row >> (step - rg.row_log + 1);
    const bool on = scan ? c + d < row : c < d;
    if (step == rg.row_log && c == 0) row_r[rid] = sh[0];
    if (!scan && d <= kCoopTreeMax) {
      __syncthreads();
      tree_step_coop<F>(sh, 0u, d);
      __syncthreads();
      continue;
    }
    XYZZ29<F> v;
    if (on) XYZZ29<F>::add_mem(&v, &sh[c], &sh[(c + d) & 255]);
    __syncthreads();
    if (on) sh[c] = v;
    __syncthreads();
  }
  if (c == 0) {
    if (rg.row_log == 0) row_r[rid] = sh[0];
    row_w[rid] = sh[0];
  }
}

template <class F, int LANES>
__global__ void __launch_bounds__(LANES) msm_rowchunk_kernel(unsigned log_nb, unsigned k_log,
                                                              const XYZZ29<F>* __restrict__ buckets,
                                                              XYZZ29<F>* __restrict__ fold ) {
  __builtin_amdgcn_s_setprio(DG16_REDUCE_PRIO);
  constexpr unsigned LL = LANES == 256 ? 8u : 7u;
  static_assert(LANES == 256 || LANES == 128, "workgroup of 256 or 128 lanes");
  __shared__ XYZZ29<F> s_r[LANES];
  __shared__ XYZZ29<F> s_w[LANES];
  const unsigned j = threadIdx.x, K = 1u << k_log;
  const XYZZ29<F>* B = buckets + ((size_t)blockIdx.y << log_nb) + (((size_t)blockIdx.x * LANES + j) << k_log);
  XYZZ29<F>* out = fold + (size_t)blockIdx.y * 3 * 256;
  s_r[j] = XYZZ29<F>::inf();
  s_w[j] = XYZZ29<F>::inf();
  __syncthreads();
  const unsigned s_scan = 2 * K, s_tree = s_scan + LL, n_steps = s_tree + LL;
#pragma unroll 1
  for (unsigned step = 0; step < n_steps; step++) {
    const XYZZ29<F>*a, *b;
    XYZZ29<F>* dst;
    bool on = true;
    if (step < s_scan) {
      const bool even = (step & 1) == 0;
      dst = even ? &s_r[j] : &s_w[j];
      a = dst;
      b = even ? &B[K - 1 - (step >> 1)] : &s_r[j];
    } else if (step < s_tree) {
      const unsigned d = 1u << (step - s_scan);
      on = j + d < (unsigned)LANES;
      dst = &s_r[j];
      a = dst;
      b = &s_r[(j + d) & (LANES - 1)];
    } else {
      if (step == s_tree) {
        if (j == 0) {
          out[1 * 256 + blockIdx.x] = s_r[0];
          s_r[0] = XYZZ29<F>::inf();
        }
        __syncthreads();
      }
      const unsigned d = (unsigned)LANES >> (step - s_tree + 1);
      const unsigned c = j & (LANES / 2 - 1);
      XYZZ29<F>* arr = j < LANES / 2 ? s_r : s_w;
      on = c < d;
      dst = &arr[c];
      a = dst;
      b = &arr[(c + d) & (LANES - 1)];
    }
    XYZZ29<F> v;
    if (on) XYZZ29<F>::add_mem(&v, a, b);
    __syncthreads();
    if (on) *dst = v;
    __syncthreads();
  }
  if (j == 0) out[2 * 256 + blockIdx.x] = s_r[0];
  if (j == LANES / 2) out[0 * 256 + blockIdx.x] = s_w[0];
}

template <class F>
__global__ void __launch_bounds__(64) msm_rowfold_kernel(RowGeom rg, const XYZZ29<F>* __restrict__ row_w,
                                                          const XYZZ29<F>* __restrict__ row_r,
                                                          XYZZ29<F>* __restrict__ fold ) {
  __builtin_amdgcn_s_setprio(DG16_REDUCE_PRIO);
  __shared__ XYZZ29<F> st[64][2];
  const unsigned gid = blockIdx.x * 64 + threadIdx.x;
  const unsigned half = gid >> 8, t = gid & 255;
  const unsigned per_log = rg.rows_log - 8, per = 1u << per_log;
  const size_t base = ((size_t)blockIdx.y << rg.rows_log) + (size_t)t * per;
  XYZZ29<F>* run = &st[threadIdx.x][0];
  XYZZ29<F>* acc = &st[threadIdx.x][1];
  *run = XYZZ29<F>::inf();
  *acc = XYZZ29<F>::inf();
#pragma unroll 1
  for (unsigned k = 0; k < 2 * per; k++) {
    const unsigned j = per - 1 - (k >> 1);
    const bool first = (k & 1) == 0;
    const bool on = first ? (half == 1 && j + 1 < per) : true;
    const XYZZ29<F>* b = first ? run : (half == 0 ? row_w : row_r) + base + j;
    if (on) XYZZ29<F>::add_mem(first ? acc : run, first ? acc : run, b);
  }
  XYZZ29<F>* out = fold + (size_t)blockIdx.y * 3 * 256;
  out[half * 256 + t] = *run;
  if (half == 1) out[2 * 256 + t] = *acc;
}

struct TopGeom {
  unsigned folded, per_log, lanes, final_log, rows_log;
};
template <class F, int HALVES>
__global__ void __launch_bounds__(256 * HALVES) msm_top_kernel(TopGeom tg, const XYZZ29<F>* __restrict__ row_w,
                                                                const XYZZ29<F>* __restrict__ row_r,
                                                                const XYZZ29<F>* __restrict__ fold,
                                                                XYZZ29<F>* __restrict__ window_sums) {
  __builtin_amdgcn_s_setprio(DG16_REDUCE_PRIO);
  __shared__ XYZZ29<F> sh[256 * HALVES];
  __shared__ XYZZ29<F> keep;
  const unsigned t = threadIdx.x & 255;
  const bool folded = tg.folded != 0;
  const unsigned per_log = tg.per_log;
  const unsigned lanes = tg.lanes;
  const size_t base = (size_t)blockIdx.x << tg.rows_log;
  const XYZZ29<F>* fb = fold + (size_t)blockIdx.x * 3 * 256;
  XYZZ29<F>* me = &sh[threadIdx.x];
#pragma unroll 1
  for (int pass = 0; pass < 3 - HALVES; pass++) {
    const unsigned half = HALVES == 2 ? threadIdx.x >> 8 : (unsigned)pass;
    *me = t < lanes ? (folded ? fb[half * 256 + t] : (half == 0 ? row_w : row_r)[base + t]) : XYZZ29<F>::inf();
    __syncthreads();
    const unsigned s_tree = 9 + per_log, s_fin = s_tree + 8;
#pragma unroll 1
    for (unsigned step = 0; step < s_fin; step++) {
      XYZZ29<F> v;
      bool on = false, is_dbl = false;
      const XYZZ29<F>* b = me;
      if (step < 8) {
        const unsigned d = 1u << step;
        on = half == 1 && t + d < 256;
        b = me + (on ? d : 0);
      } else if (step < 8 + per_log) {
        on = half == 1;
        is_dbl = true;
      } else if (step == 8 + per_log) {
        on = half == 1 && folded && t < lanes;
        b = fb + 2 * 256 + (on ? t : 0);
      } else {
        const unsigned stride = 128u >> (step - s_tree);
        if (stride <= kCoopTreeMax) {
          tree_step_coop<F>(sh, (threadIdx.x >> 8) << 8, stride);
          __syncthreads();
          continue;
        }
        on = t < stride;
        b = me + (on ? stride : 0);
      }
      if (step == 8 && half == 1 && t == 0) *me = XYZZ29<F>::inf();
      if (on) {
        if (is_dbl) XYZZ29<F>::dbl_mem(&v, me);
        else XYZZ29<F>::add_mem(&v, me, b);
      }
      __syncthreads();
      if (on) *me = v;
      __syncthreads();
    }
    if (HALVES == 1 && pass == 0) {
      if (threadIdx.x == 0) keep = sh[0];
      __syncthreads();
    }
  }
  constexpr unsigned RES = HALVES == 2 ? 256u : 0u;
  if ((threadIdx.x >> 6) == (RES >> 6)) {
    if constexpr (lane29::enabled<F>()) {
      using FO = lane29::Ops<F>;
      typename FO::KT kc;
      kc.init();
      lane29::Pt<FO> a = lane29::load_pt<F>(kc, &sh[RES]);
#pragma unroll 1
      for (unsigned k = 0; k < tg.final_log; k++) a = lane29::dbl_pt<FO>(kc, a);
      a = lane29::add_pt<FO>(kc, a, lane29::load_pt<F>(kc, HALVES == 2 ? &sh[0] : &keep));
      lane29::store_pt<F>(kc, &window_sums[blockIdx.x], a);
    } else {
      XYZZ29<F> acc = sh[RES];
#pragma unroll 1
      for (unsigned k = 0; k < tg.final_log; k++) acc = dbl_wave29(acc);
      acc = add_wave29(acc, HALVES == 2 ? sh[0] : keep);
      if ((threadIdx.x & 63) == 0) window_sums[blockIdx.x] = acc;
    }
  }
}


constexpr size_t kLaneParallelMaxEntries = 4096;
template <class F>
constexpr int lane_reduce_radix_log() {
  return (FieldOf<F>::EXT || RR<typename FieldOf<F>::Params>::N > 9) ? 3 : 4;
}
template <class F, int RB>
__global__ void __launch_bounds__(64 << RB) msm_lane_reduce_kernel(const XYZZ29<F>* __restrict__ in,
                                                                    const XYZZ29<F>* __restrict__ in2, unsigned in_per_bw_log,
                                                                    unsigned g_log, unsigned u_log, int mode, unsigned k_log,
                                                                    XYZZ29<F>* __restrict__ out,
                                                                    XYZZ29<F>* __restrict__ window_sums) {
  const int level0 = mode == 0;
  if constexpr (lane29::enabled<F>()) {
    using FO = lane29::Ops<F>;
    using LPt = lane29::Pt<FO>;
    __shared__ XYZZ29<F> sA[2][1 << RB];
    __shared__ XYZZ29<F> sB[2][1 << RB];
    __builtin_amdgcn_s_setprio(DG16_REDUCE_PRIO);
    const unsigned w = threadIdx.x >> 6, G = 1u << g_log;
    typename FO::KT kc;
    kc.init();
    const size_t e = ((size_t)blockIdx.y << in_per_bw_log) + ((size_t)blockIdx.x << g_log) + w;
    LPt R, Y;
    if (mode == 0) {
      R = lane29::load_pt<F>(kc, &in[e]);
      Y = R;
    } else if (mode == 1) {
      Y = lane29::load_pt<F>(kc, &in[2 * e]);
      R = lane29::load_pt<F>(kc, &in[2 * e + 1]);
    } else if (mode == 2) {
      Y = lane29::load_pt<F>(kc, &in[e]);
      R = lane29::load_pt<F>(kc, &in2[e]);
    } else {
      const size_t t = ((size_t)blockIdx.x << g_log) + w;
      const XYZZ29<F>* f = in + (size_t)blockIdx.y * 3 * 256;
      LPt loc = lane29::load_pt<F>(kc, &f[2 * 256 + t]);
#pragma unroll 1
      for (unsigned k = 0; k < k_log; k++) loc = lane29::dbl_pt<FO>(kc, loc);
      Y = lane29::add_pt<FO>(kc, lane29::load_pt<F>(kc, &f[t]), loc);
// ... 30 lines not shown
      if (w == 0) Y = lane29::load_pt<F>(kc, &sB[buf][0]);
    }
    if (w != 0) return;
#pragma unroll 1
    for (unsigned k = 0; k < u_log; k++) X = lane29::dbl_pt<FO>(kc, X);
    const LPt Wp = lane29::add_pt<FO>(kc, level0 ? R : Y, X);
    if (window_sums) {
      lane29::store_pt<F>(kc, &window_sums[blockIdx.y], Wp);
    } else {
      const size_t o = ((size_t)blockIdx.y << (in_per_bw_log - g_log)) + blockIdx.x;
      lane29::store_pt_raw<F>(kc, &out[2 * o], Wp);
      lane29::store_pt_raw<F>(kc, &out[2 * o + 1], R);
    }
  }
}
template <class F>
__global__ void __launch_bounds__(64) msm_lane_reduce_serial_kernel(const XYZZ29<F>* __restrict__ in, unsigned in_per_bw_log,
                                                                     unsigned g_log, unsigned u_log, int level0,
                                                                     XYZZ29<F>* __restrict__ out,
                                                                     XYZZ29<F>* __restrict__ window_sums) {
  if constexpr (lane29::enabled<F>()) {
    using FO = lane29::Ops<F>;
    using LPt = lane29::Pt<FO>;
#ifdef DG16_SERIAL_REDUCE_PRIO
    __builtin_amdgcn_s_setprio(DG16_SERIAL_REDUCE_PRIO);
#endif
    const unsigned G = 1u << g_log;
    typename FO::KT kc;
    kc.init();
    const size_t e0 = ((size_t)blockIdx.y << in_per_bw_log) + ((size_t)blockIdx.x << g_log);
    const XYZZ29<F>* base = level0 ? in + e0 : in + 2 * e0;
    const unsigned stride = level0 ? 1u : 2u, roff = level0 ? 0u : 1u;
    LPt run = lane29::inf_pt<FO>(kc), acc = run, wsum = run;
    LPt rj = lane29::load_pt_words<F>(kc, base + (size_t)(G - 1) * stride + roff), wj = rj;
    if (!level0) wj = lane29::load_pt_words<F>(kc, base + (size_t)(G - 1) * stride);
#pragma unroll 1
    for (unsigned j = G - 1; j >= 1; j--) {
      const LPt rn = lane29::load_pt_words<F>(kc, base + (size_t)(j - 1) * stride + roff);
      LPt wn = rn;
      if (!level0) wn = lane29::load_pt_words<F>(kc, base + (size_t)(j - 1) * stride);
      run = lane29::add_pt<FO>(kc, run, lane29::with_inf_flag<FO>(rj));
      acc = lane29::add_pt<FO>(kc, acc, run);
      if (!level0) wsum = lane29::add_pt<FO>(kc, wsum, lane29::with_inf_flag<FO>(wj));
      rj = rn;
      wj = wn;
    }
    rj = lane29::with_inf_flag<FO>(rj);
    wj = lane29::with_inf_flag<FO>(wj);
    const LPt Rp = lane29::add_pt<FO>(kc, run, rj);
    if (!level0) wsum = lane29::add_pt<FO>(kc, wsum, wj);
#pragma unroll 1
    for (unsigned k = 0; k < u_log; k++) acc = lane29::dbl_pt<FO>(kc, acc);
    const LPt Wp = lane29::add_pt<FO>(kc, level0 ? Rp : wsum, acc);
    if (window_sums) {
      lane29::store_pt<F>(kc, &window_sums[blockIdx.y], Wp);
    } else {
      const size_t o = ((size_t)blockIdx.y << (in_per_bw_log - g_log)) + blockIdx.x;
      lane29::store_pt_raw<F>(kc, &out[2 * o], Wp);
      lane29::store_pt_raw<F>(kc, &out[2 * o + 1], Rp);
    }
  }
}
template <class F>
bool msm_lane_reduce(hipStream_t s, const MsmGeom& g, const MsmBuffers<F>& b) {
  if constexpr (!lane29::enabled<F>()) return false;
  else {
    const unsigned bwi = g.bw * b.ninst;
    if (!b.lane_tmp || !lane_reduce_applies<F>((size_t)bwi << g.log_nb)) return false;
    static const bool busy_off = [] { const char* e = getenv("DG16_NO_LANE_REDUCE_BUSY"); return e && atoi(e) != 0; }();
    if (b.busy_chip && busy_off) return false;
    constexpr int RB = lane_reduce_radix_log<F>();
    XYZZ29<F>* pong[2] = {b.lane_tmp, b.lane_tmp + (((size_t)bwi << g.log_nb) / 4 + 2)};
    const XYZZ29<F>* in = b.buckets;
    unsigned rem = g.log_nb, u_log = 0, per_log = g.log_nb, lvl = 0;
    do {
      const unsigned g_log = rem < (unsigned)RB ? rem : (unsigned)RB;
      const bool last = rem == g_log;
      XYZZ29<F>* out = pong[lvl & 1];
      const bool one_wave = b.busy_chip || ((size_t)bwi << per_log) > kLaneParallelMaxEntries;
      if (one_wave)
        hipLaunchKernelGGL((msm_lane_reduce_serial_kernel<F>), dim3(1u << (per_log - g_log), bwi), dim3(64), 0, s, in, per_log,
                           g_log, u_log, (int)(lvl == 0), out, last ? b.window_sums : (XYZZ29<F>*)nullptr);
      else
        hipLaunchKernelGGL((msm_lane_reduce_kernel<F, RB>), dim3(1u << (per_log - g_log), bwi), dim3(64u << g_log), 0, s, in,
                           (const XYZZ29<F>*)nullptr, per_log, g_log, u_log, lvl == 0 ? 0 : 1, 0u, out,
                           last ? b.window_sums : (XYZZ29<F>*)nullptr);
      in = out;
      rem -= g_log;
      per_log -= g_log;
      u_log += g_log;
      lvl++;
    } while (rem);
    return true;
  }
}

template <class F>
bool msm_lane_top(hipStream_t s, const MsmGeom& g, const MsmBuffers<F>& b, const TopGeom& tg) {
  if constexpr (!lane29::enabled<F>()) return false;
  else {
    const unsigned bwi = g.bw * b.ninst;
    static const bool off = [] { const char* e = getenv("DG16_NO_LANE_TOP"); return e && atoi(e) != 0; }();
    if (off || !b.top_tmp || b.busy_chip || (size_t)bwi * tg.lanes > kLaneParallelMaxEntries) return false;
    unsigned ll = 0;
    while ((1u << ll) < tg.lanes) ll++;
    if ((1u << ll) != tg.lanes) return false;
    constexpr int RB = lane_reduce_radix_log<F>();
    XYZZ29<F>* pong[2] = {b.top_tmp, b.top_tmp + (size_t)bwi * 64 + 4};
    const XYZZ29<F>* in = tg.folded ? b.fold : b.row_w;
    const XYZZ29<F>* in2 = tg.folded ? nullptr : b.row_r;
    unsigned rem = ll, per_log = ll, lvl = 0;
    unsigned u_log = tg.folded ? tg.final_log + tg.per_log : tg.final_log;
    do {
      const unsigned g_log = rem < (unsigned)RB ? rem : (unsigned)RB;
      const bool last = rem == g_log;
      XYZZ29<F>* out = pong[lvl & 1];
      hipLaunchKernelGGL((msm_lane_reduce_kernel<F, RB>), dim3(1u << (per_log - g_log), bwi), dim3(64u << g_log), 0, s, in, in2,
                         per_log, g_log, u_log, lvl ? 1 : (tg.folded ? 3 : 2), tg.final_log, out,
                         last ? b.window_sums : (XYZZ29<F>*)nullptr);
      in = out;
      in2 = nullptr;
      rem -= g_log;
      per_log -= g_log;
      u_log += g_log;
      lvl++;
    } while (rem);
    return true;
  }
}

inline void trace_point(hipStream_t s, const char* what) {
  static const bool on = [] { const char* e = getenv("DG16_TRACE"); return e && atoi(e) != 0; }();
  if (!on) return;
  static thread_local std::chrono::steady_clock::time_point last = std::chrono::steady_clock::now();
  hipError_t e = hipStreamSynchronize(s);
  auto now = std::chrono::steady_clock::now();
  fprintf(stderr, "[dg16 trace] %-24s %9.3f ms  %s\n", what, std::chrono::duration<double, std::milli>(now - last).count(),
          e == hipSuccess ? "" : hipGetErrorString(e));
  last = now;
}

template <class F>
void msm_bucket_phase(hipStream_t s, const MsmSort& st, const MsmBuffers<F>& b, bool out_affine, void* out_dev) {
  const MsmGeom& g = st.g;
  const unsigned bwi = g.bw * b.ninst;
  DG_BOUNDS_BIND();
  trace_point(s, "(before bucket phase)");
  if constexpr (FieldOf<F>::EXT) {
  } else {
    DG_HIP(hipMemsetAsync(b.giant, 0, 8, s));
    msm_finalize_phase<F>(s, st, b);
  }
  trace_point(s, "finalize");
  hipLaunchKernelGGL(msm_giant_kernel<F>, dim3(256), dim3(256), 0, s, g, msm_acc_wg_log<F>(), st.counts, st.seg_off,
                     b.seg_sum, b.giant, b.giant + 2, b.giant_cap);
  hipLaunchKernelGGL(msm_giant_fold_kernel<F>, dim3(64), dim3(64), 0, s, g, msm_acc_wg_log<F>(), st.counts, st.seg_off,
                     b.seg_sum, b.buckets, b.giant, b.giant + 2, b.giant_cap);
  trace_point(s, "giant + fold");
  if (msm_lane_reduce<F>(s, g, b)) {
    trace_point(s, "lane reduce");
    msm_tail_phase<F>(s, st, b, out_affine, out_dev);
    trace_point(s, "tail");
    DG_HIP(hipGetLastError());
    return;
  }
  constexpr int CH_LANES = sizeof(XYZZ29<F>) * 2 * 256 <= 150 * 1024 ? 256 : 128;
  constexpr unsigned CH_LL = CH_LANES == 256 ? 8u : 7u;
  unsigned k_log = 0;
  if (b.rg.row_log == kRowLog && g.log_nb >= CH_LL + 1) {
    const size_t total_rows = (size_t)bwi << b.rg.rows_log;
    while (k_log < 3 && (total_rows >> (k_log + 1)) >= 256 && g.log_nb >= CH_LL + k_log + 1) k_log++;
    if (total_rows < 1024) k_log = 0;
    if (total_rows < 1024 && RR<typename FieldOf<F>::Params>::N > 9 && g.table && g.region >= ((size_t)1 << 23)) {
      k_log = g.log_nb - CH_LL < 3 ? g.log_nb - CH_LL : 3;
    }
    if (k_log > 3) k_log = 3;
    if (k_log && g.log_nb - k_log - CH_LL > 8) k_log = 0;
  }
  TopGeom tg{};
  tg.rows_log = b.rg.rows_log;
  tg.final_log = b.rg.row_log;
  if (k_log) {
    const unsigned nsr_log = g.log_nb - k_log - CH_LL;
    DG_REQUIRE(nsr_log <= 8, DG16_ERR_UNSUPPORTED, "row chunks: more than 256 per bucket-window");
    hipLaunchKernelGGL((msm_rowchunk_kernel<F, CH_LANES>), dim3(1u << nsr_log, bwi), dim3(CH_LANES), 0, s, g.log_nb, k_log,
                       b.buckets, b.fold);
    trace_point(s, "row (chunks)");
    tg.folded = 1;
    tg.per_log = CH_LL;
    tg.lanes = 1u << nsr_log;
    tg.final_log = k_log;
  } else {
    hipLaunchKernelGGL(msm_row_kernel<F>, dim3(1u << b.rg.rows_log, bwi), dim3(256), 0, s, g, b.rg, b.buckets, b.row_w,
                       b.row_r);
    trace_point(s, "row");
    tg.folded = b.rg.rows_log > 8;
    tg.per_log = tg.folded ? b.rg.rows_log - 8 : 0;
    tg.lanes = tg.folded ? 256u : 1u << b.rg.rows_log;
    if (b.rg.rows_log > 8)
      hipLaunchKernelGGL(msm_rowfold_kernel<F>, dim3(8, bwi), dim3(64), 0, s, b.rg, b.row_w, b.row_r, b.fold);
  }
  constexpr int HALVES = sizeof(XYZZ29<F>) * 513 <= 160 * 1024 ? 2 : 1;
  if (!msm_lane_top<F>(s, g, b, tg))
    hipLaunchKernelGGL((msm_top_kernel<F, HALVES>), dim3(bwi), dim3(256 * HALVES), 0, s, tg, b.row_w, b.row_r,
                       b.fold, b.window_sums);
  trace_point(s, "top");
  msm_tail_phase<F>(s, st, b, out_affine, out_dev);
  trace_point(s, "tail");
  DG_HIP(hipGetLastError());
}

}
```

### distributed-groth16_amd/csrc/prover_impl.h

```cpp
#pragma once
#include "ctx.h"
#include "types.h"

#include "msm_impl.h"
#include "pk.h"

namespace dg16 {

template <class Fr>
__global__ void prover_scalar_prep_kernel(const Fr* r_s, Fr* sc, size_t n, int mont, int carries_delta) {
  Fr r = r_s[0], s = r_s[1];
  if (!carries_delta) { r = Fr::zero(); s = Fr::zero(); }
  Fr rm = mont ? r : r.to_mont(), sm = mont ? s : s.to_mont();
  Fr nrs = (rm * sm).neg();
  sc[n] = r;
  sc[n + 1] = s;
  sc[n + 2] = mont ? nrs : nrs.from_mont();
}

template <class F, class Fr>
__device__ XYZZ<F> mul_by_fr(const XYZZ<F>& p, const Fr& k_canon) {
  return scalar_mul<F, Fr::NL>(p, k_canon.l);
}

// ... 106 lines not shown
__device__ __forceinline__ Jacobian<F> xyzz29_to_record_wave(const XYZZ29<F>& a) {
  using FO = FieldOf<F>;
  using P = typename FO::Params;
  if (a.is_inf()) return {F::one(), F::one(), F::zero()};
  const unsigned slot = (__lane_id() & 15) >> 2;
  const auto a1 = select(slot == 0, a.x, select(slot == 1, a.y, a.zz));
  const auto b1 = select(slot == 0, a.zz, select(slot == 1, a.zzz, FO::one()));
  const auto r1 = SlotMulCall::mul(a1, b1);
  const auto r2 = SlotMulCall::mul(r1, konst29((const F*)nullptr, RR<P>::TO32));
  return {words32(bcast29<0>(r2)), words32(bcast29<4>(r2)), words32(bcast29<8>(r2))};
}

template <class Fq, class Fq2>
__global__ void __launch_bounds__(256, 1) prover_assemble_kernel(const uint8_t* gathered, size_t n_shards, size_t rec_bytes,
                                                                  Jacobian<Fq>* out_a, Jacobian<Fq2>* out_b,
                                                                  Jacobian<Fq>* out_c) {
  __shared__ XYZZ29<Fq> part[4];
  __shared__ XYZZ29<Fq2> part_b;
  __builtin_amdgcn_s_setprio(DG16_CHAIN_PRIO);
  const unsigned w4 = threadIdx.x >> 6, lane = threadIdx.x & 63;
  const unsigned wave = blockIdx.x == 0 ? 2 + w4 : w4 == 2 ? 6u : w4;
  if (blockIdx.x == 1 && w4 == 3) return;
  if (wave == 1 || wave == 6) {
    const size_t half = (n_shards + 1) / 2;
    const size_t lo = wave == 1 ? 0 : half, cnt = wave == 1 ? half : n_shards - half;
    const size_t steps = cnt + (wave == 1 ? 1 : 0);
    XYZZ29<Fq2> b = XYZZ29<Fq2>::inf();
#pragma unroll 1
    for (size_t k = 0; k < steps; k++) {
      if (k == cnt) __syncthreads();
      XYZZ29<Fq2> o;
      if (k < cnt)
        o = record_to_xyzz29_wave(*(const Jacobian<Fq2>*)(gathered + (lo + k) * rec_bytes + kRecG1 * sizeof(Jacobian<Fq>)));
      else
        o = part_b;
      b = add_wave29<Fq2, SlotMulCall>(b, o);
    }
    if (wave == 6) {
      if (lane == 0) part_b = b;
      __syncthreads();
      return;
    }
    const Jacobian<Fq2> r = xyzz29_to_record_wave(b);
    if (lane == 0) *out_b = r;
    return;
  }
  const int slot = wave == 0 ? kRecA : wave == 2 ? kRecL : wave == 3 ? kRecH : wave == 4 ? kRecSA : kRecRB1;
  XYZZ29<Fq> a = XYZZ29<Fq>::inf();
  const size_t steps = n_shards + (wave == 2 ? 3 : 0);
#pragma unroll 1
  for (size_t k = 0; k < steps; k++) {
    if (k == n_shards) __syncthreads();
    XYZZ29<Fq> o;
    if (k < n_shards)
      o = record_to_xyzz29_wave(*((const Jacobian<Fq>*)(gathered + k * rec_bytes) + slot));
    else
      o = part[k - n_shards + 1];
    a = add_wave29<Fq, SlotMulCall>(a, o);
    if (k + 1 == n_shards && wave >= 3 && lane == 0) part[wave - 2] = a;
  }
  if (wave != 2) __syncthreads();
  if (wave == 0 || wave == 2) {
    const Jacobian<Fq> r = xyzz29_to_record_wave(a);
    if (lane == 0) *(wave == 0 ? out_a : out_c) = r;
  }
}

template <int CURVE>
static size_t msm_results_bytes() {
  using CT = CurveTypes<CURVE>;
  return kRecG1 * sizeof(Jacobian<typename CT::Fq>) + sizeof(Jacobian<typename CT::Fq2>);
}

template <int CURVE>
static bool msms_typed(dg16_ctx* ctx, Call& k0, Call& k1, Call& k2, const PkDev& pk, const void* a, const void* b,
                       const void* c, const void* witness, const void* r_s_host, bool mont, bool dev_ptrs,
                       uint8_t* res_dev, const dg16_comm* comm = nullptr, const void* h_given = nullptr,
                       bool overlap_tail = false) {
  using CT = CurveTypes<CURVE>;
  using Fq = typename CT::Fq;
  using Fq2 = typename CT::Fq2;
  using Fr = typename CT::Fr;
  const size_t nv = pk.num_vars, ni = pk.num_inputs, m = pk.m;
  const size_t n_ab = pk.ab_hi - pk.ab_lo;
  const size_t n_h = pk.h_hi - pk.h_lo;
  unsigned log_m = 0;
  while (((size_t)1 << log_m) < m) log_m++;
  const size_t g1j = sizeof(Jacobian<Fq>);

  const bool dist = !h_given && comm && comm->n_ranks(comm->self) > 1;
  if (dist) {
    DG_REQUIRE(pk.h_cyclic && comm->n_ranks(comm->self) == pk.nshards && comm->rank(comm->self) == pk.shard,
               DG16_ERR_BAD_ARG, "distributed prove: the key must be the DG16_F_H_CYCLIC shard `rank` of `n_ranks`");
  } else if (!h_given) {
    DG_REQUIRE(!(pk.h_cyclic && pk.nshards > 1), DG16_ERR_BAD_ARG,
               "a DG16_F_H_CYCLIC shard needs the sharded h-polynomial (dg16_groth16_prove_dist / _msms_h)");
  }
  const size_t rows = dist ? m / pk.nshards : m;
  const Fr* w_dev = (const Fr*)stage_in(k0, 18, witness, nv * sizeof(Fr), dev_ptrs);
  const void* a_dev = h_given ? nullptr : stage_in(k0, 19, a, rows * sizeof(Fr), dev_ptrs);
  const void* b_dev = h_given ? nullptr : stage_in(k0, 20, b, rows * sizeof(Fr), dev_ptrs);
  const void* c_dev = h_given ? nullptr : stage_in(k0, 21, c, rows * sizeof(Fr), dev_ptrs);
  const Fr* h_in = h_given ? (const Fr*)stage_in(k0, 19, h_given, n_h * sizeof(Fr), dev_ptrs) : nullptr;
  Fr* r_s = (Fr*)ws(k0.c, 22, 4096);
  Jacobian<Fq>* rec = (Jacobian<Fq>*)res_dev;
  Jacobian<Fq>* res_h = rec + kRecH;
  Jacobian<Fq2>* res_b2 = (Jacobian<Fq2>*)(res_dev + kRecG1 * g1j);
  const int first_shard = pk.shard == 0;
  Fr* sc_ab = (Fr*)ws(k0.c, 23, (n_ab + 3) * sizeof(Fr));
  hipStream_t main = k0.s(), side = k1.s(), side2 = k2.s();
  hipEvent_t* ev = ctx->pipe_ev;
  const Affine<Fq>* fixed_g1 = (const Affine<Fq>*)pk.fixed;
  const Affine<Fq2>* fixed_g2 = (const Affine<Fq2>*)((const uint8_t*)pk.fixed + 4 * sizeof(Affine<Fq>));
  hipStream_t xch = ctx->aux[0];

  const unsigned n_ranks = dist ? comm->n_ranks(comm->self) : 1, rank = dist ? comm->rank(comm->self) : 0;
  const size_t xbytes = 3 * rows * sizeof(Fr);
  void* xbuf_a = dist ? ws(k0.c, 26, xbytes) : nullptr;
  void* xbuf_b = dist ? ws(k0.c, 27, xbytes) : nullptr;
  auto exchange = [&](int ev_ready, int ev_done) {
    DG_HIP(hipEventRecord(ev[ev_ready], main));
    DG_HIP(hipStreamWaitEvent(xch, ev[ev_ready], 0));
    int rc = comm->all_to_all(comm->self, xbuf_a, xbuf_b, xbytes / n_ranks, xch);
    DG_REQUIRE(rc == DG16_OK, DG16_ERR_NET, "all-to-all of the sharded h-polynomial failed");
    DG_HIP(hipEventRecord(ev[ev_done], xch));
  };

  static const bool queue_join = [] { const char* e = getenv("DG16_QUEUE_JOIN"); return e && atoi(e) != 0; }();
  const bool queued = overlap_tail && !h_given && !dist && !queue_join;
  Fr* h_dev = h_given ? nullptr : (Fr*)ws(k0.c, 3, rows * sizeof(Fr));
  const Fr* h_scalars = h_in;
  auto whole_h = [&] {
    h_poly_launch(k0, CURVE, a_dev, b_dev, c_dev, log_m, h_dev);
    h_scalars = h_dev + pk.h_lo;
  };
  const hipStream_t pro = queued ? side : main;
  if (queued) {
    DG_HIP(hipEventRecord(ev[8], main));
    whole_h();
    DG_HIP(hipStreamWaitEvent(side, ev[8], 0));
    DG_HIP(hipStreamWaitEvent(side, ev[5], 0));
    DG_HIP(hipStreamWaitEvent(side, ev[7], 0));
  }
  DG_HIP(hipMemcpyAsync(r_s, r_s_host, 2 * sizeof(Fr), hipMemcpyHostToDevice, pro));
  DG_HIP(hipMemcpyAsync(sc_ab, w_dev + 1 + pk.ab_lo, n_ab * sizeof(Fr), hipMemcpyDeviceToDevice, pro));
  hipLaunchKernelGGL(prover_scalar_prep_kernel<Fr>, dim3(1), dim3(1), 0, pro, r_s, sc_ab, n_ab, (int)mont,
                     (int)(pk.shard + 1 == pk.nshards));
  DG_HIP(hipGetLastError());
  if (!queued) {
    DG_HIP(hipEventRecord(ev[8], main));
    DG_HIP(hipStreamWaitEvent(side, ev[8], 0));
  }

  MsmSort st_ab = msm_sort_on<Fr, CT::SCALAR_BITS>(side, k1.c, sc_ab, n_ab + 3, mont, true, pk.c_ab, pk.stride);
  DG_HIP(hipEventRecord(ev[13], side));
  MsmBuffers<Fq2> buf_b2 = msm_buffers<Fq2>(k2.c, st_ab.g);
  buf_b2.busy_chip = true;

  if (dist) {
    const void* rows_in[3] = {a_dev, b_dev, c_dev};
    h_poly_dist_stage(k0, CURVE, log_m, rank, n_ranks, 0, rows_in, xbuf_a);
    exchange(3, 4);
  } else if (!h_given && !queued) {
    whole_h();
  }
  MsmSort st_h;
  const bool tail_fence = overlap_tail && ctx->tail_pending.load(std::memory_order_acquire);
  if (!dist) {
    DG_HIP(hipEventRecord(ev[14], main));
    DG_HIP(hipStreamWaitEvent(side, ev[14], 0));
    if (tail_fence) DG_HIP(hipStreamWaitEvent(side, ev[18], 0));
    st_h = msm_sort_on<Fr, CT::SCALAR_BITS>(side, k0.c, h_scalars, n_h, true, true, pk.c_h, pk.stride);
    DG_HIP(hipEventRecord(ev[15], side));
  }

  DG_HIP(hipStreamWaitEvent(main, ev[13], 0));
  DG_HIP(hipEventRecord(k2.c.ev[2], main));
  buf_b2.acc_done = k2.c.ev[3];
  if (ctx->kclk) buf_b2.clk = ctx->kclk + 2 * 2;
  {
    static const int fin_env = [] { const char* e = getenv("DG16_G2_FINALIZE_SIDE"); return e ? atoi(e) : -1; }();
    const bool side_fin = fin_env >= 0 ? fin_env != 0 : RR<typename FieldOf<Fq>::Params>::N == 9;
    if (side_fin) buf_b2.finalize_stream = side2;
  }
  msm_accumulate_phase<Fq2>(main, st_ab, buf_b2, pk.b2_q);
  k2.c.ev_valid[1] = true;
  DG_HIP(hipEventRecord(ev[2], main));
  DG_HIP(hipStreamWaitEvent(side2, ev[2], 0));
  msm_bucket_phase<Fq2>(side2, st_ab, buf_b2, false, res_b2);
  hipLaunchKernelGGL(prover_stage1_g2_kernel<Fq2>, dim3(1), dim3(64), 0, side2, res_b2, fixed_g2, first_shard);
  DG_HIP(hipEventRecord(ev[5], side2));
  if (dist) {
    const void* in1[1] = {xbuf_b};
    DG_HIP(hipStreamWaitEvent(main, ev[4], 0));
    h_poly_dist_stage(k0, CURVE, log_m, rank, n_ranks, 1, in1, xbuf_a);
    exchange(9, 11);
  }

  static const int abl_env = [] { const char* e = getenv("DG16_ABL_MERGED"); return e ? atoi(e) : -1; }();
  const bool abl_merged = abl_env >= 0 ? abl_env != 0 : st_ab.g.region * st_ab.g.bw <= ((size_t)1 << 22);
  if (abl_merged) {
    MsmBuffers<Fq> buf3 = msm_buffers<Fq>(k0.c, st_ab.g, 3);
    buf3.busy_chip = true;
    const void* bases3[3] = {pk.a_q, pk.b1_q, pk.l_q};
    static_assert(kRecA == 0 && kRecB1 == 1 && kRecL == 2, "the three results land back to back in the record");
    DG_HIP(hipEventRecord(k1.c.ev[2], main));
    if (ctx->kclk) buf3.clk = ctx->kclk + 2 * 1;
    msm_accumulate_phase<Fq>(main, st_ab, buf3, bases3);
    DG_HIP(hipEventRecord(k1.c.ev[3], main));
    k1.c.ev_valid[1] = true;
    DG_HIP(hipEventRecord(ev[6], main));
    DG_HIP(hipStreamWaitEvent(side, ev[6], 0));
    if (tail_fence) DG_HIP(hipStreamWaitEvent(side, ev[18], 0));
    msm_bucket_phase<Fq>(side, st_ab, buf3, false, rec + kRecA);
    DG_HIP(hipEventRecord(ev[12], side));
    DG_HIP(hipStreamWaitEvent(xch, ev[12], 0));
    hipLaunchKernelGGL((prover_stage1_g1_kernel<Fq, Fr>), dim3(2), dim3(scalar_mul_splits<Fq>() ? 128 : 64), 0, xch, rec,
                       fixed_g1, r_s, (int)mont, first_shard);
    DG_HIP(hipEventRecord(ev[7], xch));
    DG_HIP(hipStreamWaitEvent(side, ev[7], 0));
    DG_HIP(hipEventRecord(ev[10], side));
  } else
  {
    MsmBuffers<Fq> buf_a = msm_buffers<Fq>(k0.c, st_ab.g);
    MsmBuffers<Fq> buf_b1 = msm_buffers<Fq>(k1.c, st_ab.g);
    MsmBuffers<Fq> buf_l = msm_buffers<Fq>(ctx->xws[1], st_ab.g);
    buf_a.busy_chip = buf_b1.busy_chip = buf_l.busy_chip = true;
    msm_accumulate_phase<Fq>(main, st_ab, buf_a, pk.a_q);
    DG_HIP(hipEventRecord(ev[0], main));
    DG_HIP(hipEventRecord(k1.c.ev[2], main));
    if (ctx->kclk) buf_b1.clk = ctx->kclk + 2 * 1;
    msm_accumulate_phase<Fq>(main, st_ab, buf_b1, pk.b1_q);
    DG_HIP(hipEventRecord(k1.c.ev[3], main));
    k1.c.ev_valid[1] = true;
    DG_HIP(hipEventRecord(ev[1], main));
    msm_accumulate_phase<Fq>(main, st_ab, buf_l, pk.l_q);
    DG_HIP(hipEventRecord(ev[6], main));
    DG_HIP(hipStreamWaitEvent(side, ev[0], 0));
    if (tail_fence) DG_HIP(hipStreamWaitEvent(side, ev[18], 0));
    msm_bucket_phase<Fq>(side, st_ab, buf_a, false, rec + kRecA);
    DG_HIP(hipEventRecord(ev[12], side));
    DG_HIP(hipStreamWaitEvent(xch, ev[1], 0));
    if (tail_fence) DG_HIP(hipStreamWaitEvent(xch, ev[18], 0));
    msm_bucket_phase<Fq>(xch, st_ab, buf_b1, false, rec + kRecB1);
    DG_HIP(hipStreamWaitEvent(xch, ev[12], 0));
    hipLaunchKernelGGL((prover_stage1_g1_kernel<Fq, Fr>), dim3(2), dim3(scalar_mul_splits<Fq>() ? 128 : 64), 0, xch, rec,
                       fixed_g1, r_s, (int)mont, first_shard);
    DG_HIP(hipEventRecord(ev[7], xch));
    DG_HIP(hipStreamWaitEvent(side, ev[6], 0));
    msm_bucket_phase<Fq>(side, st_ab, buf_l, false, rec + kRecL);
    DG_HIP(hipStreamWaitEvent(side, ev[7], 0));
    DG_HIP(hipEventRecord(ev[10], side));
  }

  if (dist) {
    const void* in2[1] = {xbuf_b};
    DG_HIP(hipStreamWaitEvent(main, ev[11], 0));
    h_poly_dist_stage(k0, CURVE, log_m, rank, n_ranks, 2, in2, h_dev);
    if (tail_fence) DG_HIP(hipStreamWaitEvent(main, ev[18], 0));
    st_h = msm_sort_on<Fr, CT::SCALAR_BITS>(main, k0.c, h_dev, n_h, true, true, pk.c_h, pk.stride);
  } else {
    DG_HIP(hipStreamWaitEvent(main, ev[15], 0));
  }
  MsmBuffers<Fq> buf_h = msm_buffers<Fq>(ctx->xws[0], st_h.g);
  const bool tail_on_side2 = overlap_tail && !h_given;
  buf_h.busy_chip = tail_on_side2;
  if (tail_fence) DG_HIP(hipStreamWaitEvent(main, ev[18], 0));
  msm_accumulate_phase<Fq>(main, st_h, buf_h, pk.h_q);
  if (tail_on_side2) {
    DG_HIP(hipEventRecord(ev[17], main));
    DG_HIP(hipStreamWaitEvent(side2, ev[17], 0));
    msm_bucket_phase<Fq>(side2, st_h, buf_h, false, res_h);
    DG_HIP(hipStreamWaitEvent(side2, ev[10], 0));
  } else {
    msm_bucket_phase<Fq>(main, st_h, buf_h, false, res_h);
  }
  if (!queued) {
    DG_HIP(hipStreamWaitEvent(main, ev[10], 0));
    DG_HIP(hipStreamWaitEvent(main, ev[5], 0));
  }
  DG_HIP(hipGetLastError());
  return tail_on_side2;
}

template <int CURVE>
static void assemble_typed(Call& k0, const uint8_t* gathered_dev, size_t n_shards, uint8_t* proof_dev,
                           hipStream_t stream = nullptr) {
  using CT = CurveTypes<CURVE>;
  using Fq = typename CT::Fq;
  using Fq2 = typename CT::Fq2;
  const size_t g1j = sizeof(Jacobian<Fq>), g2j = sizeof(Jacobian<Fq2>);
  hipLaunchKernelGGL((prover_assemble_kernel<Fq, Fq2>), dim3(2), dim3(256), 0, stream ? stream : k0.s(), gathered_dev, n_shards,
                     msm_results_bytes<CURVE>(), (Jacobian<Fq>*)proof_dev, (Jacobian<Fq2>*)(proof_dev + g1j),
                     (Jacobian<Fq>*)(proof_dev + g1j + g2j));
  DG_HIP(hipGetLastError());
}

template <int CURVE>
static void prove_typed(dg16_ctx* ctx, const PkDev& pk, const void* a, const void* b, const void* c,
                        const void* witness, const void* r_s_host, bool mont, bool dev_ptrs, void* proof_out,
                        bool overlap_tail = false) {
  using CT = CurveTypes<CURVE>;
  const size_t g1j = sizeof(Jacobian<typename CT::Fq>), g2j = sizeof(Jacobian<typename CT::Fq2>);
  DG_REQUIRE(pk.nshards == 1, DG16_ERR_BAD_ARG, "dg16_groth16_prove needs an unsharded key; use _msms + _assemble");
  overlap_tail = overlap_tail && dev_ptrs;
  Call k0(ctx, 0, overlap_tail), k1(ctx, 1, overlap_tail), k2(ctx, 2, overlap_tail);
  uint8_t* buf = (uint8_t*)ws(k0.c, 16, 8192);
  uint8_t* res_dev = buf;
  uint8_t* proof_dev = buf + 4096;
  k0.begin_dominant();
  const bool tail = msms_typed<CURVE>(ctx, k0, k1, k2, pk, a, b, c, witness, r_s_host, mont, dev_ptrs, res_dev, nullptr,
                                      nullptr, overlap_tail);
  if (tail) {
    k0.end_dominant();
    assemble_typed<CURVE>(k0, res_dev, 1, proof_dev, k2.s());
    if (proof_out != proof_dev)
      DG_HIP(hipMemcpyAsync(proof_out, proof_dev, 2 * g1j + g2j, hipMemcpyDeviceToDevice, k2.s()));
    DG_HIP(hipEventRecord(ctx->pipe_ev[18], k2.s()));
    ctx->tail_pending.store(true, std::memory_order_release);
    k0.finish();
    k1.finish();
    k2.finish();
    return;
  }
  assemble_typed<CURVE>(k0, res_dev, 1, proof_dev);
  k0.end_dominant();
  stage_out(k0, proof_out, proof_dev, 2 * g1j + g2j, dev_ptrs);
  k0.finish();
  k1.finish();
  k2.finish();
  if (!dev_ptrs) DG_HIP(hipStreamSynchronize(k0.s()));
}

template <int CURVE>
static void prove_dist_typed(dg16_ctx* ctx, const PkDev& pk, const dg16_comm* comm, const void* a, const void* b,
                             const void* c, const void* witness, const void* r_s_host, bool mont, bool dev_ptrs,
                             void* proof_out, bool overlap_tail = false) {
  using CT = CurveTypes<CURVE>;
  const size_t g1j = sizeof(Jacobian<typename CT::Fq>), g2j = sizeof(Jacobian<typename CT::Fq2>);
  const unsigned n = comm ? comm->n_ranks(comm->self) : 1;
  DG_REQUIRE(pk.nshards == n, DG16_ERR_BAD_ARG, "distributed prove: key shards != ranks");
  overlap_tail = overlap_tail && dev_ptrs;
  Call k0(ctx, 0, overlap_tail), k1(ctx, 1, overlap_tail), k2(ctx, 2, overlap_tail);
  uint8_t* buf = (uint8_t*)ws(k0.c, 16, 8192);
  uint8_t* res_dev = buf;
  uint8_t* proof_dev = buf + 4096;
  const size_t rec = msm_results_bytes<CURVE>();
  uint8_t* gathered = n > 1 ? (uint8_t*)ws(k0.c, 28, n * rec) : res_dev;
  k0.begin_dominant();
  const bool tail = msms_typed<CURVE>(ctx, k0, k1, k2, pk, a, b, c, witness, r_s_host, mont, dev_ptrs, res_dev, comm, nullptr,
                                      overlap_tail);
  hipStream_t ts = tail ? k2.s() : k0.s();
  if (n > 1) {
    int rc = comm->all_gather(comm->self, res_dev, rec, gathered, ts);
    DG_REQUIRE(rc == DG16_OK, DG16_ERR_NET, "all-gather of the MSM records failed");
  }
  assemble_typed<CURVE>(k0, gathered, n, proof_dev, ts);
  k0.end_dominant();
  if (tail) {
    if (proof_out != proof_dev)
      DG_HIP(hipMemcpyAsync(proof_out, proof_dev, 2 * g1j + g2j, hipMemcpyDeviceToDevice, ts));
    DG_HIP(hipEventRecord(ctx->pipe_ev[18], ts));
    ctx->tail_pending.store(true, std::memory_order_release);
  } else {
    stage_out(k0, proof_out, proof_dev, 2 * g1j + g2j, dev_ptrs);
  }
  k0.finish();
  k1.finish();
  k2.finish();
  if (!dev_ptrs) DG_HIP(hipStreamSynchronize(k0.s()));
}

template <int CURVE>
static void pk_build(dg16_ctx* ctx, PkDev& d, const void* a_query, const void* b_g1_query,
                     const void* b_g2_query, const void* h_query, const void* l_query, const void* fixed_host,
                     bool dev_ptrs) {
  using CT = CurveTypes<CURVE>;
  using Fq = typename CT::Fq;
  using Fq2 = typename CT::Fq2;
  const size_t p1 = sizeof(Affine<Fq>), p2 = sizeof(Affine<Fq2>);
  const size_t nv = d.num_vars, ni = d.num_inputs, m = d.m;
  hipMemcpyKind kind = dev_ptrs ? hipMemcpyDeviceToDevice : hipMemcpyHostToDevice;
  auto slice = [&](size_t n, size_t& lo, size_t& hi) {
    lo = n * d.shard / d.nshards;
    hi = n * (d.shard + 1) / d.nshards;
  };
  slice(nv - 1, d.ab_lo, d.ab_hi);
  d.l_lo = (d.ab_lo > ni - 1 ? d.ab_lo : ni - 1) - (ni - 1);
  d.l_hi = (d.ab_hi > ni - 1 ? d.ab_hi : ni - 1) - (ni - 1);
  slice(m, d.h_lo, d.h_hi);
  if (d.h_cyclic) {
    DG_REQUIRE(!(d.nshards & (d.nshards - 1)) && (size_t)d.nshards * d.nshards <= m, DG16_ERR_BAD_ARG,
               "DG16_F_H_CYCLIC: n_shards must be a power of two with n_shards^2 <= domain_size");
    d.h_lo = 0;
    d.h_hi = m / d.nshards;
  }
  const size_t n_ab = d.ab_hi - d.ab_lo, n_l = d.l_hi - d.l_lo, n_h = d.h_hi - d.h_lo;
  DG_HIP(hipSetDevice(ctx->device));
  void *a_plain = nullptr, *b1_plain = nullptr, *b2_plain = nullptr, *l_plain = nullptr, *h_plain = nullptr;
  struct PlainGuard {
    void **p[5];
    ~PlainGuard() {
      for (void** q : p)
        if (*q) { hipFree(*q); *q = nullptr; }
    }
  } plain_guard{{&a_plain, &b1_plain, &b2_plain, &l_plain, &h_plain}};
  DG_HIP(hipMalloc(&a_plain, (n_ab + 3) * p1));
  DG_HIP(hipMalloc(&b1_plain, (n_ab + 3) * p1));
  DG_HIP(hipMalloc(&b2_plain, (n_ab + 3) * p2));
  DG_HIP(hipMalloc(&l_plain, (n_ab + 3) * p1));
  DG_HIP(hipMalloc(&h_plain, (n_h ? n_h : 1) * p1));
  DG_HIP(hipMalloc(&d.fixed, 4 * p1 + 2 * p2));
  const uint8_t* fx = (const uint8_t*)fixed_host;
// ... 57 lines not shown
```

Baseline: 109.8 million constraints/s.

## Cap side-stream MSM kernel grids so they share CUs with the main stream

Adds a SideCap policy that limits the workgroup count of kernels launched on side streams: the partition histogram, scatter and count kernels, the place kernel, the giant-bucket kernel, and the row and rowchunk reductions. These kernels become persistent grid-stride loops over work items. The aim is to stop side-stream sort and bucket work from flooding the GPU and stalling the concurrent main-stream accumulate kernels, improving overlap between them. The cost is that capped kernels get less parallelism when they run alone, and the cap can be overridden with an environment variable.

```diff
diff --git a/distributed-groth16_amd/csrc/capi.hip b/distributed-groth16_amd/csrc/capi.hip
--- a/distributed-groth16_amd/csrc/capi.hip
+++ b/distributed-groth16_amd/csrc/capi.hip
@@ -44,6 +44,8 @@
     ctx->device = device;
     ctx->compute_units = p.multiProcessorCount;
     ctx->name = p.gcnArchName;
+    ctx->side_wgs = 0;
+    if (const char* e = getenv("DG16_SIDE_WGS")) ctx->side_wgs = atoi(e) < 0 ? -1 : atoi(e);
     int prio_lo = 0, prio_hi = 0;
     DG_HIP(hipDeviceGetStreamPriorityRange(&prio_lo, &prio_hi));
     for (int i = 0; i < kChannels; i++) {
diff --git a/distributed-groth16_amd/csrc/ctx.h b/distributed-groth16_amd/csrc/ctx.h
--- a/distributed-groth16_amd/csrc/ctx.h
+++ b/distributed-groth16_amd/csrc/ctx.h
@@ -48,11 +48,36 @@
   bool shift_full_tried = false;
 };
 
+struct SideCap {
+  unsigned cus = 0;
+  int forced = -1;
+  unsigned scale = 1;
+  unsigned grid(unsigned natural, size_t lds_bytes) const {
+    if (!cus || forced == 0) return natural;
+    unsigned s;
+    if (forced > 0) {
+      s = (unsigned)forced;
+    } else {
+      constexpr size_t kSlotLds = 40 * 1024;
+      const size_t fit = lds_bytes ? kSlotLds / lds_bytes : 4;
+      s = (cus / 4 ? cus / 4 : 1u) * (unsigned)(fit < 1 ? 1 : fit > 4 ? 4 : fit) * scale;
+    }
+    return natural < s ? natural : s;
+  }
+  SideCap scaled(unsigned k) const {
+    SideCap c = *this;
+    c.scale = k;
+    return c;
+  }
+};
+
 }
 
 struct dg16_ctx {
   int device = 0;
   int compute_units = 0;
+  int side_wgs = 0;
+  dg16::SideCap side_cap() const { return dg16::SideCap{(unsigned)compute_units, side_wgs, 1}; }
   std::string name;
   dg16::Channel ch[dg16::kChannels];
   std::mutex mu;
diff --git a/distributed-groth16_amd/csrc/msm_group.hip b/distributed-groth16_amd/csrc/msm_group.hip
--- a/distributed-groth16_amd/csrc/msm_group.hip
+++ b/distributed-groth16_amd/csrc/msm_group.hip
@@ -20,7 +20,7 @@
 template void msm_tail_phase<GF>(hipStream_t, const MsmSort&, const MsmBuffers<GF>&, bool, void*);
 template void* msm_build_table<GF>(hipStream_t, const void*, size_t, unsigned, unsigned);
 template MsmSort msm_sort_on<CT::Fr, CT::SCALAR_BITS>(hipStream_t, Channel&, const void*, size_t, unsigned, bool, unsigned,
-                                                      unsigned);
+                                                      unsigned, SideCap);
 
 void DG_FN(msm_)(Call& k, const void* bases, const void* scalars, size_t n, unsigned mode, bool affine, void* out) {
   msm_run<GF, CT::Fr, CT::SCALAR_BITS>(k, bases, scalars, n, mode, affine, out);
diff --git a/distributed-groth16_amd/csrc/msm_impl.h b/distributed-groth16_amd/csrc/msm_impl.h
--- a/distributed-groth16_amd/csrc/msm_impl.h
+++ b/distributed-groth16_amd/csrc/msm_impl.h
@@ -302,23 +302,25 @@
                                                              MsmGeom g, PartGeom pg,
                                                              unsigned* __restrict__ blockhist) {
   __shared__ unsigned hist[kPartMax];
-  hist[threadIdx.x] = 0;
-  __syncthreads();
-  for (unsigned k = 0; k < kPartScalars / 256; k++) {
-    size_t i = (size_t)blockIdx.x * kPartScalars + k * 256 + threadIdx.x;
-    if (i >= n) continue;
-    Fr s = scalars[i];
-    if (mont & 1) s = s.from_mont();
-    unsigned carry = 0;
-    for (unsigned w = 0; w < g.nwin; w++) {
-      int d = msm_digit(s, w, g.c, carry);
-      if (d == 0) continue;
-      unsigned slot = ((w % g.bw) << g.log_nb) + (unsigned)(d < 0 ? -d : d) - 1;
-      atomicAdd(&hist[slot >> pg.low_bits], 1u);
-    }
-  }
-  __syncthreads();
-  if (threadIdx.x < pg.nparts) blockhist[(size_t)threadIdx.x * pg.nblk1 + blockIdx.x] = hist[threadIdx.x];
+  for (unsigned blk = blockIdx.x; blk < pg.nblk1; blk += gridDim.x) {
+    hist[threadIdx.x] = 0;
+    __syncthreads();
+    for (unsigned k = 0; k < kPartScalars / 256; k++) {
+      size_t i = (size_t)blk * kPartScalars + k * 256 + threadIdx.x;
+      if (i >= n) continue;
+      Fr s = scalars[i];
+      if (mont & 1) s = s.from_mont();
+      unsigned carry = 0;
+      for (unsigned w = 0; w < g.nwin; w++) {
+        int d = msm_digit(s, w, g.c, carry);
+        if (d == 0) continue;
+        unsigned slot = ((w % g.bw) << g.log_nb) + (unsigned)(d < 0 ? -d : d) - 1;
+        atomicAdd(&hist[slot >> pg.low_bits], 1u);
+      }
+    }
+    __syncthreads();
+    if (threadIdx.x < pg.nparts) blockhist[(size_t)threadIdx.x * pg.nblk1 + blk] = hist[threadIdx.x];
+  }
 }
 
 template <class Fr>
@@ -327,23 +329,26 @@
                                                                 const unsigned* __restrict__ blockoff,
                                                                 uint2* __restrict__ part) {
   __shared__ unsigned cur[kPartMax];
-  if (threadIdx.x < pg.nparts) cur[threadIdx.x] = blockoff[(size_t)threadIdx.x * pg.nblk1 + blockIdx.x];
-  __syncthreads();
-  for (unsigned k = 0; k < kPartScalars / 256; k++) {
-    size_t i = (size_t)blockIdx.x * kPartScalars + k * 256 + threadIdx.x;
-    if (i >= n) continue;
-    Fr s = scalars[i];
-    if (mont & 1) s = s.from_mont();
-    const bool flip = (mont & 2) && (s.l[Fr::NL - 1] >> 31);
-    unsigned carry = 0;
-    for (unsigned w = 0; w < g.nwin; w++) {
-      int d = msm_digit(s, w, g.c, carry);
-      if (d == 0) continue;
-      unsigned slot = ((w % g.bw) << g.log_nb) + (unsigned)(d < 0 ? -d : d) - 1;
-      unsigned ref = (unsigned)((size_t)(w / g.bw) * n + i);
-      unsigned pos = atomicAdd(&cur[slot >> pg.low_bits], 1u);
-      part[DG_IDX(14, pos, (size_t)g.nwin * n)] = make_uint2(ref | (((d < 0) != flip) ? 0x80000000u : 0u), slot);
-    }
+  for (unsigned blk = blockIdx.x; blk < pg.nblk1; blk += gridDim.x) {
+    if (threadIdx.x < pg.nparts) cur[threadIdx.x] = blockoff[(size_t)threadIdx.x * pg.nblk1 + blk];
+    __syncthreads();
+    for (unsigned k = 0; k < kPartScalars / 256; k++) {
+      size_t i = (size_t)blk * kPartScalars + k * 256 + threadIdx.x;
+      if (i >= n) continue;
+      Fr s = scalars[i];
+      if (mont & 1) s = s.from_mont();
+      const bool flip = (mont & 2) && (s.l[Fr::NL - 1] >> 31);
+      unsigned carry = 0;
+      for (unsigned w = 0; w < g.nwin; w++) {
+        int d = msm_digit(s, w, g.c, carry);
+        if (d == 0) continue;
+        unsigned slot = ((w % g.bw) << g.log_nb) + (unsigned)(d < 0 ? -d : d) - 1;
+        unsigned ref = (unsigned)((size_t)(w / g.bw) * n + i);
+        unsigned pos = atomicAdd(&cur[slot >> pg.low_bits], 1u);
+        part[DG_IDX(14, pos, (size_t)g.nwin * n)] = make_uint2(ref | (((d < 0) != flip) ? 0x80000000u : 0u), slot);
+      }
+    }
+    __syncthreads();
   }
 }
 
@@ -409,26 +414,40 @@
     if (lo + j < len) a[lo + j] += add;
 }
 
+struct PartItem {
+  unsigned p, bx;
+};
+__device__ __forceinline__ PartItem part_item(unsigned item, const PartGeom& pg) {
+  const bool capped = gridDim.x < kPartBlocks * pg.nparts;
+  PartItem it;
+  it.p = capped ? item % pg.nparts : item / kPartBlocks;
+  it.bx = capped ? item / pg.nparts : item % kPartBlocks;
+  return it;
+}
+
 template <int TU>
 __global__ void __launch_bounds__(256) msm_part_count_kernel(const uint2* __restrict__ part,
                                                               const unsigned* __restrict__ blockoff, PartGeom pg,
                                                               unsigned* __restrict__ counts) {
   __shared__ unsigned hist[1u << kPartMaxLowBits];
-  const unsigned p = blockIdx.y;
-  const unsigned lo = blockoff[(size_t)p * pg.nblk1];
-  const unsigned size = blockoff[(size_t)(p + 1) * pg.nblk1] - lo;
-  if (((size_t)blockIdx.x << kPartTileLog) >= size) return;
   const unsigned nlow = 1u << pg.low_bits;
-  for (unsigned b = threadIdx.x; b < nlow; b += 256) hist[b] = 0;
-  __syncthreads();
-  for (size_t t = (size_t)blockIdx.x << kPartTileLog; t < size; t += (size_t)gridDim.x << kPartTileLog)
-    for (unsigned j = 0; j < (1u << kPartTileLog) / 256; j++) {
-      size_t idx = t + j * 256 + threadIdx.x;
-      if (idx < size) atomicAdd(&hist[part[lo + idx].y & (nlow - 1)], 1u);
-    }
-  __syncthreads();
-  for (unsigned b = threadIdx.x; b < nlow; b += 256)
-    if (hist[b]) atomicAdd(&counts[((size_t)p << pg.low_bits) + b], hist[b]);
+  for (unsigned item = blockIdx.x; item < kPartBlocks * pg.nparts; item += gridDim.x) {
+    const PartItem it = part_item(item, pg);
+    const unsigned p = it.p;
+    const unsigned lo = blockoff[(size_t)p * pg.nblk1];
+    const unsigned size = blockoff[(size_t)(p + 1) * pg.nblk1] - lo;
+    if (((size_t)it.bx << kPartTileLog) >= size) continue;
+    for (unsigned b = threadIdx.x; b < nlow; b += 256) hist[b] = 0;
+    __syncthreads();
+    for (size_t t = (size_t)it.bx << kPartTileLog; t < size; t += (size_t)kPartBlocks << kPartTileLog)
+      for (unsigned j = 0; j < (1u << kPartTileLog) / 256; j++) {
+        size_t idx = t + j * 256 + threadIdx.x;
+        if (idx < size) atomicAdd(&hist[part[lo + idx].y & (nlow - 1)], 1u);
+      }
+    __syncthreads();
+    for (unsigned b = threadIdx.x; b < nlow; b += 256)
+      if (hist[b]) atomicAdd(&counts[((size_t)p << pg.low_bits) + b], hist[b]);
+  }
 }
 
 template <int TU>
@@ -441,42 +460,44 @@
   __shared__ unsigned cnt[1u << kPartMaxLowBits];
   __shared__ unsigned rank0[1u << kPartMaxLowBits];
   __shared__ unsigned dst0[1u << kPartMaxLowBits];
-  const unsigned p = blockIdx.y;
-  const unsigned lo = blockoff[(size_t)p * pg.nblk1];
-  const unsigned size = blockoff[(size_t)(p + 1) * pg.nblk1] - lo;
-  if (((size_t)blockIdx.x << kPartTileLog) >= size) return;
   const unsigned nlow = 1u << pg.low_bits;
   constexpr unsigned PER = (1u << kPartTileLog) / 256;
-  for (size_t t = (size_t)blockIdx.x << kPartTileLog; t < size; t += (size_t)gridDim.x << kPartTileLog) {
-    for (unsigned b = threadIdx.x; b < nlow; b += 256) cnt[b] = 0;
-    __syncthreads();
-    uint2 e[PER];
-    unsigned lr[PER];
-#pragma unroll
-    for (unsigned j = 0; j < PER; j++) {
-      size_t idx = t + j * 256 + threadIdx.x;
-      e[j] = make_uint2(0u, 0xFFFFFFFFu);
-      if (idx < size) {
-        e[j] = part[lo + idx];
-        lr[j] = atomicAdd(&cnt[e[j].y & (nlow - 1)], 1u);
+  for (unsigned item = blockIdx.x; item < kPartBlocks * pg.nparts; item += gridDim.x) {
+    const PartItem it = part_item(item, pg);
+    const unsigned p = it.p;
+    const unsigned lo = blockoff[(size_t)p * pg.nblk1];
+    const unsigned size = blockoff[(size_t)(p + 1) * pg.nblk1] - lo;
+    for (size_t t = (size_t)it.bx << kPartTileLog; t < size; t += (size_t)kPartBlocks << kPartTileLog) {
+      for (unsigned b = threadIdx.x; b < nlow; b += 256) cnt[b] = 0;
+      __syncthreads();
+      uint2 e[PER];
+      unsigned lr[PER];
+#pragma unroll
+      for (unsigned j = 0; j < PER; j++) {
+        size_t idx = t + j * 256 + threadIdx.x;
+        e[j] = make_uint2(0u, 0xFFFFFFFFu);
+        if (idx < size) {
+          e[j] = part[lo + idx];
+          lr[j] = atomicAdd(&cnt[e[j].y & (nlow - 1)], 1u);
+        }
       }
-    }
-    __syncthreads();
-    for (unsigned b = threadIdx.x; b < nlow; b += 256)
-      if (cnt[b]) {
-        const size_t slot = ((size_t)p << pg.low_bits) + b;
-        rank0[b] = atomicAdd(&cursor[slot], cnt[b]);
-        dst0[b] = (unsigned)((slot >> g.log_nb) * g.region) + offsets[slot];
+      __syncthreads();
+      for (unsigned b = threadIdx.x; b < nlow; b += 256)
+        if (cnt[b]) {
+          const size_t slot = ((size_t)p << pg.low_bits) + b;
+          rank0[b] = atomicAdd(&cursor[slot], cnt[b]);
+          dst0[b] = (unsigned)((slot >> g.log_nb) * g.region) + offsets[slot];
+        }
+      __syncthreads();
+#pragma unroll
+      for (unsigned j = 0; j < PER; j++) {
+        if (e[j].y == 0xFFFFFFFFu) continue;
+        const unsigned slot = e[j].y, b = slot & (nlow - 1);
+        const unsigned rank = rank0[b] + lr[j];
+        entries[DG_IDX(13, dst0[b] + rank, (size_t)g.bw * g.region)] = e[j].x;
       }
-    __syncthreads();
-#pragma unroll
-    for (unsigned j = 0; j < PER; j++) {
-      if (e[j].y == 0xFFFFFFFFu) continue;
-      const unsigned slot = e[j].y, b = slot & (nlow - 1);
-      const unsigned rank = rank0[b] + lr[j];
-      entries[DG_IDX(13, dst0[b] + rank, (size_t)g.bw * g.region)] = e[j].x;
-    }
-    __syncthreads();
+      __syncthreads();
+    }
   }
 }
 
@@ -1651,15 +1672,15 @@
 
 template <class Fr, int SCALAR_BITS>
 MsmSort msm_sort_on(hipStream_t s, Channel& wsch, const void* scalars, size_t n, unsigned scalars_mont, bool table,
-                    unsigned c_fixed, unsigned stride);
+                    unsigned c_fixed, unsigned stride, SideCap cap);
 template <class Fr, int SCALAR_BITS>
 MsmSort msm_sort(Call& k, const void* scalars, size_t n, unsigned scalars_mont, bool table, unsigned c_fixed = 0,
                  unsigned stride = 1) {
-  return msm_sort_on<Fr, SCALAR_BITS>(k.s(), k.c, scalars, n, scalars_mont, table, c_fixed, stride);
+  return msm_sort_on<Fr, SCALAR_BITS>(k.s(), k.c, scalars, n, scalars_mont, table, c_fixed, stride, SideCap{});
 }
 template <class Fr, int SCALAR_BITS>
 MsmSort msm_sort_on(hipStream_t s, Channel& wsch, const void* scalars, size_t n, unsigned scalars_mont, bool table,
-                    unsigned c_fixed, unsigned stride) {
+                    unsigned c_fixed, unsigned stride, SideCap cap) {
   MsmSort r;
   DG_BOUNDS_BIND();
   r.n = n;
@@ -1698,14 +1719,14 @@
     const unsigned nchunks = (unsigned)((len + 4095) / 4096);
     unsigned* tot = blockoff + len;
     DG_HIP(hipMemsetAsync(blockoff + len - 1, 0, 4, s));
-    hipLaunchKernelGGL(msm_part_hist_kernel<Fr>, dim3(pg.nblk1), dim3(256), 0, s, (const Fr*)scalars, n,
+    hipLaunchKernelGGL(msm_part_hist_kernel<Fr>, dim3(cap.grid(pg.nblk1, kPartMax * 4)), dim3(256), 0, s, (const Fr*)scalars, n,
                        (int)scalars_mont, g, pg, blockoff);
     hipLaunchKernelGGL(scan_chunk_kernel<0>, dim3(nchunks), dim3(1024), 0, s, blockoff, len, tot);
     hipLaunchKernelGGL(scan_tops_kernel<0>, dim3(1), dim3(1024), 0, s, tot, nchunks);
     hipLaunchKernelGGL(scan_add_kernel<0>, dim3(nchunks), dim3(1024), 0, s, blockoff, len, tot);
-    hipLaunchKernelGGL(msm_part_scatter_kernel<Fr>, dim3(pg.nblk1), dim3(256), 0, s, (const Fr*)scalars, n,
+    hipLaunchKernelGGL(msm_part_scatter_kernel<Fr>, dim3(cap.grid(pg.nblk1, kPartMax * 4)), dim3(256), 0, s, (const Fr*)scalars, n,
                        (int)scalars_mont, g, pg, blockoff, part);
-    hipLaunchKernelGGL(msm_part_count_kernel<0>, dim3(kPartBlocks, pg.nparts), dim3(256), 0, s, part, blockoff, pg,
+    hipLaunchKernelGGL(msm_part_count_kernel<0>, dim3(cap.grid(kPartBlocks * pg.nparts, 4u << kPartMaxLowBits)), dim3(256), 0, s, part, blockoff, pg,
                        r.counts);
   } else if (n) {
     hipLaunchKernelGGL(msm_digits_kernel<Fr>, dim3((unsigned)((n + 255) / 256)), dim3(256), 0, s, (const Fr*)scalars,
@@ -1720,7 +1741,7 @@
                        block_tot, g.log_nb);
   }
   if (n && partitioned)
-    hipLaunchKernelGGL(msm_part_place_kernel<0>, dim3(kPartBlocks, pg.nparts), dim3(256), 0, s, part, blockoff, pg, g,
+    hipLaunchKernelGGL(msm_part_place_kernel<0>, dim3(cap.grid(kPartBlocks * pg.nparts, 12u << kPartMaxLowBits)), dim3(256), 0, s, part, blockoff, pg, g,
                        r.offsets, r.seg_off, r.cursor, r.entries);
   else if (n)
     hipLaunchKernelGGL(msm_scatter_kernel<0>, dim3((unsigned)((n + 255) / 256), g.nwin), dim3(256), 0, s, r.digits, n, g,
@@ -1750,6 +1771,7 @@
   XYZZ29<F>* top_tmp;
   hipStream_t finalize_stream = nullptr;
   bool busy_chip = false;
+  SideCap side;
   unsigned* giant;
   unsigned giant_cap;
   size_t nbw, nrows;
@@ -1995,20 +2017,16 @@
   __device__ __forceinline__ void launder() { asm volatile("" : "+v"(p)); }
 };
 template <class F, int BLOCK>
-__global__ void __launch_bounds__(BLOCK, (BLOCK == 256 ? 2 : 1))
-msm_finalize_lds_kernel(MsmGeom g, size_t total, unsigned wg_log, unsigned lpb_log,
-                        const unsigned* __restrict__ counts,
-                        const unsigned* __restrict__ seg_off, const XYZZ29<F>* __restrict__ seg_sum,
-                        XYZZ29<F>* __restrict__ buckets, unsigned* __restrict__ giant_count,
-                        unsigned* __restrict__ giant_list, unsigned giant_cap) {
+__device__ __forceinline__ void
+msm_finalize_lds_item(const MsmGeom& g, size_t total, unsigned wg_log, unsigned lpb_log, size_t blk,
+                      uint32_t (*sh)[BLOCK], unsigned& max_serial, const unsigned* __restrict__ counts,
+                      const unsigned* __restrict__ seg_off, const XYZZ29<F>* __restrict__ seg_sum,
+                      XYZZ29<F>* __restrict__ buckets, unsigned* __restrict__ giant_count,
+                      unsigned* __restrict__ giant_list, unsigned giant_cap) {
   using FO = FieldOf<F>;
-  constexpr int WORDS = sizeof(typename FO::Store) / 4;
-  __shared__ uint32_t sh[4 * WORDS][BLOCK];
-  __shared__ unsigned max_serial;
-  if constexpr (sizeof(F) > 64) asm volatile("" ::: DG_ACC_FILE_CLOBBERS);
   const unsigned LPB = 1u << lpb_log;
   const unsigned lane = threadIdx.x, sub = lane & (LPB - 1);
-  const size_t gid = ((size_t)blockIdx.x * BLOCK + lane) >> lpb_log;
+  const size_t gid = (blk * BLOCK + lane) >> lpb_log;
   const ColAcc<F, BLOCK> me{sh, lane};
   unsigned np = 0, first = 0;
   unsigned wy = 0;
@@ -2058,6 +2076,38 @@
     buckets[gid] = out;
   }
 }
+template <class F, int BLOCK>
+__global__ void __launch_bounds__(BLOCK, (BLOCK == 256 ? 2 : 1))
+msm_finalize_lds_kernel(MsmGeom g, size_t total, unsigned wg_log, unsigned lpb_log,
+                        const unsigned* __restrict__ counts,
+                        const unsigned* __restrict__ seg_off, const XYZZ29<F>* __restrict__ seg_sum,
+                        XYZZ29<F>* __restrict__ buckets, unsigned* __restrict__ giant_count,
+                        unsigned* __restrict__ giant_list, unsigned giant_cap) {
+  constexpr int WORDS = sizeof(typename FieldOf<F>::Store) / 4;
+  __shared__ uint32_t sh[4 * WORDS][BLOCK];
+  __shared__ unsigned max_serial;
+  if constexpr (sizeof(F) > 64) asm volatile("" ::: DG_ACC_FILE_CLOBBERS);
+  msm_finalize_lds_item<F, BLOCK>(g, total, wg_log, lpb_log, blockIdx.x, sh, max_serial, counts, seg_off, seg_sum, buckets,
+                                  giant_count, giant_list, giant_cap);
+}
+template <class F, int BLOCK>
+__global__ void __launch_bounds__(BLOCK, (BLOCK == 256 ? 2 : 1))
+msm_finalize_lds_items_kernel(MsmGeom g, size_t total, unsigned wg_log, unsigned lpb_log,
+                              const unsigned* __restrict__ counts, const unsigned* __restrict__ seg_off,
+                              const XYZZ29<F>* __restrict__ seg_sum, XYZZ29<F>* __restrict__ buckets,
+                              unsigned* __restrict__ giant_count, unsigned* __restrict__ giant_list, unsigned giant_cap) {
+  constexpr int WORDS = sizeof(typename FieldOf<F>::Store) / 4;
+  __shared__ uint32_t sh[4 * WORDS][BLOCK];
+  __shared__ unsigned max_serial;
+  if constexpr (sizeof(F) > 64) asm volatile("" ::: DG_ACC_FILE_CLOBBERS);
+  const size_t nblk = ((total << lpb_log) + BLOCK - 1) / BLOCK;
+#pragma unroll 1
+  for (size_t blk = blockIdx.x; blk < nblk; blk += gridDim.x) {
+    msm_finalize_lds_item<F, BLOCK>(g, total, wg_log, lpb_log, blk, sh, max_serial, counts, seg_off, seg_sum, buckets,
+                                    giant_count, giant_list, giant_cap);
+    __syncthreads();
+  }
+}
 inline int msm_finalize_lds_lpb() { return 2; }
 template <class F>
 void msm_finalize_lds_phase(hipStream_t s, const MsmSort& st, const MsmBuffers<F>& b) {
@@ -2066,67 +2116,80 @@
   const unsigned lpb_log = lpb == 4 ? 2u : lpb == 2 ? 1u : 0u;
   DG_HIP(hipMemsetAsync(b.giant, 0, 8, s));
   const unsigned blocks = (unsigned)((b.nbw * (size_t)lpb + BLOCK - 1) / BLOCK);
-  hipLaunchKernelGGL((msm_finalize_lds_kernel<F, BLOCK>), dim3(blocks), dim3(BLOCK), 0, s, st.g, b.nbw,
-                     msm_acc_wg_log<F>(), lpb_log, st.counts, st.seg_off, b.seg_sum, b.buckets, b.giant, b.giant + 2,
-                     b.giant_cap);
+  constexpr size_t kLds = 4 * sizeof(typename FieldOf<F>::Store) * BLOCK;
+  const unsigned wgs = b.side.grid(blocks, kLds);
+  if (wgs < blocks)
+    hipLaunchKernelGGL((msm_finalize_lds_items_kernel<F, BLOCK>), dim3(wgs), dim3(BLOCK), 0, s, st.g, b.nbw,
+                       msm_acc_wg_log<F>(), lpb_log, st.counts, st.seg_off, b.seg_sum, b.buckets, b.giant, b.giant + 2,
+                       b.giant_cap);
+  else
+    hipLaunchKernelGGL((msm_finalize_lds_kernel<F, BLOCK>), dim3(blocks), dim3(BLOCK), 0, s, st.g, b.nbw,
+                       msm_acc_wg_log<F>(), lpb_log, st.counts, st.seg_off, b.seg_sum, b.buckets, b.giant, b.giant + 2,
+                       b.giant_cap);
 }
 
 template <class F, int TU = 0>
-__global__ void __launch_bounds__(256) msm_stitch_kernel(MsmGeom g, unsigned wg_log, const unsigned* __restrict__ counts,
+__global__ void __launch_bounds__(256) msm_stitch_kernel(MsmGeom g, unsigned wg_log, unsigned items_x, unsigned nwy,
+                                                          const unsigned* __restrict__ counts,
                                                           const unsigned* __restrict__ seg_off,
                                                           const unsigned* __restrict__ seg_total,
                                                           const XYZZ29<F>* __restrict__ seg_sum,
                                                           XYZZ29<F>* __restrict__ buckets,
                                                           unsigned* __restrict__ giant_count,
                                                           unsigned* __restrict__ giant_list, unsigned giant_cap) {
-  const unsigned wy = blockIdx.y, w = wy % g.bw;
-  const unsigned bd = blockIdx.x * blockDim.x + threadIdx.x + 1;
-  const unsigned slot = bd << wg_log;
-  if (slot >= seg_total[w]) return;
-  const unsigned* so = seg_off + ((size_t)w << g.log_nb);
-  unsigned lo = 0, hi = 1u << g.log_nb;
-  while (hi - lo > 1) {
-    const unsigned mid = (lo + hi) >> 1;
-    if (so[mid] <= slot) lo = mid; else hi = mid;
-  }
-  const unsigned first = so[lo];
-  if (first == slot || (first >> wg_log) != bd - 1) return;
-  const size_t gs = ((size_t)w << g.log_nb) + lo;
-  const size_t gid = ((size_t)wy << g.log_nb) + lo;
-  const unsigned k = (counts[gs] + (1u << g.seg_log) - 1) >> g.seg_log;
-  const unsigned np = msm_nparts(first, k, wg_log);
-  if (np > kGiantSegs) {
-    msm_register_giant((unsigned)gid, np, giant_count, giant_list, giant_cap);
-    return;
-  }
-  const XYZZ29<F>* sp = seg_sum + (size_t)wy * g.seg_cap;
-  XYZZ29<F> acc = sp[DG_IDX(7, first, g.seg_cap)];
-#pragma unroll 1
-  for (unsigned s = 1; s < np; s++) acc = acc.add(sp[DG_IDX(7, msm_part_slot(first, s, wg_log), g.seg_cap)]);
-  buckets[gid] = acc;
+  const unsigned nitems = items_x * nwy;
+#pragma unroll 1
+  for (unsigned item = blockIdx.x; item < nitems; item += gridDim.x) {
+    const unsigned wy = item / items_x, w = wy % g.bw;
+    const unsigned bd = (item % items_x) * blockDim.x + threadIdx.x + 1;
+    const unsigned slot = bd << wg_log;
+    if (slot >= seg_total[w]) continue;
+    const unsigned* so = seg_off + ((size_t)w << g.log_nb);
+    unsigned lo = 0, hi = 1u << g.log_nb;
+    while (hi - lo > 1) {
+      const unsigned mid = (lo + hi) >> 1;
+      if (so[mid] <= slot) lo = mid; else hi = mid;
+    }
+    const unsigned first = so[lo];
+    if (first == slot || (first >> wg_log) != bd - 1) continue;
+    const size_t gs = ((size_t)w << g.log_nb) + lo;
+    const size_t gid = ((size_t)wy << g.log_nb) + lo;
+    const unsigned k = (counts[gs] + (1u << g.seg_log) - 1) >> g.seg_log;
+    const unsigned np = msm_nparts(first, k, wg_log);
+    if (np > kGiantSegs) {
+      msm_register_giant((unsigned)gid, np, giant_count, giant_list, giant_cap);
+      continue;
+    }
+    const XYZZ29<F>* sp = seg_sum + (size_t)wy * g.seg_cap;
+    XYZZ29<F> acc = sp[DG_IDX(7, first, g.seg_cap)];
+#pragma unroll 1
+    for (unsigned s = 1; s < np; s++) acc = acc.add(sp[DG_IDX(7, msm_part_slot(first, s, wg_log), g.seg_cap)]);
+    buckets[gid] = acc;
+  }
 }
 template <class F>
 __global__ void __launch_bounds__(256) msm_empty_buckets_kernel(MsmGeom g, size_t total, const unsigned* __restrict__ counts,
                                                                  XYZZ29<F>* __restrict__ buckets) {
-  const size_t gid = (size_t)blockIdx.x * blockDim.x + threadIdx.x;
-  if (gid >= total) return;
-  const unsigned wy = (unsigned)(gid >> g.log_nb);
-  const size_t gs = ((size_t)(wy % g.bw) << g.log_nb) + (gid & (((size_t)1 << g.log_nb) - 1));
-  if (counts[gs]) return;
-  uint4* dst = reinterpret_cast<uint4*>(buckets + gid);
   static_assert(sizeof(XYZZ29<F>) % 16 == 0, "vector stores");
-#pragma unroll
-  for (unsigned i = 0; i < sizeof(XYZZ29<F>) / 16; i++) dst[i] = make_uint4(0u, 0u, 0u, 0u);
+  for (size_t gid = (size_t)blockIdx.x * blockDim.x + threadIdx.x; gid < total; gid += (size_t)gridDim.x * blockDim.x) {
+    const unsigned wy = (unsigned)(gid >> g.log_nb);
+    const size_t gs = ((size_t)(wy % g.bw) << g.log_nb) + (gid & (((size_t)1 << g.log_nb) - 1));
+    if (counts[gs]) continue;
+    uint4* dst = reinterpret_cast<uint4*>(buckets + gid);
+#pragma unroll
+    for (unsigned i = 0; i < sizeof(XYZZ29<F>) / 16; i++) dst[i] = make_uint4(0u, 0u, 0u, 0u);
+  }
 }
 template <class F>
 void msm_finalize_phase(hipStream_t s, const MsmSort& st, const MsmBuffers<F>& b) {
   DG_BOUNDS_BIND();
   if constexpr (msm_acc_tree<F>()) {
-    hipLaunchKernelGGL(msm_empty_buckets_kernel<F>, dim3((unsigned)((b.nbw + 255) / 256)), dim3(256), 0, s, st.g, b.nbw,
+    hipLaunchKernelGGL(msm_empty_buckets_kernel<F>, dim3(b.side.grid((unsigned)((b.nbw + 255) / 256), 0)), dim3(256), 0, s, st.g, b.nbw,
                        st.counts, b.buckets);
     const unsigned nbd = (st.g.seg_cap >> msm_acc_wg_log<F>()) + 1;
-    hipLaunchKernelGGL(msm_stitch_kernel<F>, dim3((nbd + 255) / 256, st.g.bw * b.ninst), dim3(256), 0, s, st.g,
-                       msm_acc_wg_log<F>(), st.counts, st.seg_off, st.seg_total, b.seg_sum, b.buckets, b.giant,
+    const unsigned items_x = (nbd + 255) / 256, nwy = st.g.bw * b.ninst;
+    hipLaunchKernelGGL(msm_stitch_kernel<F>, dim3(b.side.grid(items_x * nwy, 0)), dim3(256), 0, s, st.g,
+                       msm_acc_wg_log<F>(), items_x, nwy, st.counts, st.seg_off, st.seg_total, b.seg_sum, b.buckets, b.giant,
                        b.giant + 2, b.giant_cap);
   } else {
     bool lane = false;
@@ -2456,4 +2519,4 @@
   DG16_MSM_EXTERN_GROUP(CT::Fq)                                                                                   \
   DG16_MSM_EXTERN_GROUP(CT::Fq2)                                                                                  \
   extern template MsmSort msm_sort_on<CT::Fr, CT::SCALAR_BITS>(hipStream_t, Channel&, const void*, size_t, unsigned, bool, \
-                                                              unsigned, unsigned);
+                                                              unsigned, unsigned, SideCap);
diff --git a/distributed-groth16_amd/csrc/msm_reduce_impl.h b/distributed-groth16_amd/csrc/msm_reduce_impl.h
--- a/distributed-groth16_amd/csrc/msm_reduce_impl.h
+++ b/distributed-groth16_amd/csrc/msm_reduce_impl.h
@@ -111,12 +111,9 @@
 }
 
 template <class F>
-__global__ void __launch_bounds__(256) msm_row_kernel(MsmGeom g, RowGeom rg, const XYZZ29<F>* __restrict__ buckets,
-                                                       XYZZ29<F>* __restrict__ row_w, XYZZ29<F>* __restrict__ row_r) {
-  __builtin_amdgcn_s_setprio(DG16_REDUCE_PRIO);
-  __shared__ XYZZ29<F> sh[256];
+__device__ __forceinline__ void msm_row_item(const RowGeom& rg, size_t rid, const XYZZ29<F>* __restrict__ buckets,
+                                             XYZZ29<F>* __restrict__ row_w, XYZZ29<F>* __restrict__ row_r, XYZZ29<F>* sh) {
   const unsigned c = threadIdx.x, row = 1u << rg.row_log;
-  const size_t rid = ((size_t)blockIdx.y << rg.rows_log) + blockIdx.x;
   sh[c] = c < row ? buckets[(rid << rg.row_log) + c] : XYZZ29<F>::inf();
   __syncthreads();
 #pragma unroll 1
@@ -142,19 +139,35 @@
     row_w[rid] = sh[0];
   }
 }
+template <class F>
+__global__ void __launch_bounds__(256) msm_row_kernel(MsmGeom g, RowGeom rg, const XYZZ29<F>* __restrict__ buckets,
+                                                       XYZZ29<F>* __restrict__ row_w, XYZZ29<F>* __restrict__ row_r) {
+  __builtin_amdgcn_s_setprio(DG16_REDUCE_PRIO);
+  __shared__ XYZZ29<F> sh[256];
+  msm_row_item<F>(rg, ((size_t)blockIdx.y << rg.rows_log) + blockIdx.x, buckets, row_w, row_r, sh);
+}
+template <class F>
+__global__ void __launch_bounds__(256) msm_row_items_kernel(RowGeom rg, size_t nrows, const XYZZ29<F>* __restrict__ buckets,
+                                                             XYZZ29<F>* __restrict__ row_w, XYZZ29<F>* __restrict__ row_r) {
+  __builtin_amdgcn_s_setprio(DG16_REDUCE_PRIO);
+  __shared__ XYZZ29<F> sh[256];
+#pragma unroll 1
+  for (size_t rid = blockIdx.x; rid < nrows; rid += gridDim.x) {
+    msm_row_item<F>(rg, rid, buckets, row_w, row_r, sh);
+    __syncthreads();
+  }
+}
 
 template <class F, int LANES>
-__global__ void __launch_bounds__(LANES) msm_rowchunk_kernel(unsigned log_nb, unsigned k_log,
-                                                              const XYZZ29<F>* __restrict__ buckets,
-                                                              XYZZ29<F>* __restrict__ fold ) {
-  __builtin_amdgcn_s_setprio(DG16_REDUCE_PRIO);
+__device__ __forceinline__ void msm_rowchunk_item(unsigned log_nb, unsigned k_log, unsigned bx, unsigned by,
+                                                  const XYZZ29<F>* __restrict__ buckets, XYZZ29<F>* __restrict__ fold,
+                                                  XYZZ29<F>* s_r ,
+                                                  XYZZ29<F>* s_w ) {
   constexpr unsigned LL = LANES == 256 ? 8u : 7u;
   static_assert(LANES == 256 || LANES == 128, "workgroup of 256 or 128 lanes");
-  __shared__ XYZZ29<F> s_r[LANES];
-  __shared__ XYZZ29<F> s_w[LANES];
   const unsigned j = threadIdx.x, K = 1u << k_log;
-  const XYZZ29<F>* B = buckets + ((size_t)blockIdx.y << log_nb) + (((size_t)blockIdx.x * LANES + j) << k_log);
-  XYZZ29<F>* out = fold + (size_t)blockIdx.y * 3 * 256;
+  const XYZZ29<F>* B = buckets + ((size_t)by << log_nb) + (((size_t)bx * LANES + j) << k_log);
+  XYZZ29<F>* out = fold + (size_t)by * 3 * 256;
   s_r[j] = XYZZ29<F>::inf();
   s_w[j] = XYZZ29<F>::inf();
   __syncthreads();
@@ -178,7 +191,7 @@
     } else {
       if (step == s_tree) {
         if (j == 0) {
-          out[1 * 256 + blockIdx.x] = s_r[0];
+          out[1 * 256 + bx] = s_r[0];
           s_r[0] = XYZZ29<F>::inf();
         }
         __syncthreads();
@@ -197,8 +210,30 @@
     if (on) *dst = v;
     __syncthreads();
   }
-  if (j == 0) out[2 * 256 + blockIdx.x] = s_r[0];
-  if (j == LANES / 2) out[0 * 256 + blockIdx.x] = s_w[0];
+  if (j == 0) out[2 * 256 + bx] = s_r[0];
+  if (j == LANES / 2) out[0 * 256 + bx] = s_w[0];
+}
+template <class F, int LANES>
+__global__ void __launch_bounds__(LANES) msm_rowchunk_kernel(unsigned log_nb, unsigned k_log,
+                                                              const XYZZ29<F>* __restrict__ buckets,
+                                                              XYZZ29<F>* __restrict__ fold ) {
+  __builtin_amdgcn_s_setprio(DG16_REDUCE_PRIO);
+  __shared__ XYZZ29<F> s_r[LANES];
+  __shared__ XYZZ29<F> s_w[LANES];
+  msm_rowchunk_item<F, LANES>(log_nb, k_log, blockIdx.x, blockIdx.y, buckets, fold, s_r, s_w);
+}
+template <class F, int LANES>
+__global__ void __launch_bounds__(LANES) msm_rowchunk_items_kernel(unsigned log_nb, unsigned k_log, unsigned nchunks, unsigned nbwi,
+                                                                    const XYZZ29<F>* __restrict__ buckets,
+                                                                    XYZZ29<F>* __restrict__ fold) {
+  __builtin_amdgcn_s_setprio(DG16_REDUCE_PRIO);
+  __shared__ XYZZ29<F> s_r[LANES];
+  __shared__ XYZZ29<F> s_w[LANES];
+#pragma unroll 1
+  for (unsigned item = blockIdx.x; item < nchunks * nbwi; item += gridDim.x) {
+    msm_rowchunk_item<F, LANES>(log_nb, k_log, item % nchunks, item / nchunks, buckets, fold, s_r, s_w);
+    __syncthreads();
+  }
 }
 
 template <class F>
@@ -535,7 +570,7 @@
     msm_finalize_phase<F>(s, st, b);
   }
   trace_point(s, "finalize");
-  hipLaunchKernelGGL(msm_giant_kernel<F>, dim3(256), dim3(256), 0, s, g, msm_acc_wg_log<F>(), st.counts, st.seg_off,
+  hipLaunchKernelGGL(msm_giant_kernel<F>, dim3(b.side.grid(256, 256 * sizeof(XYZZ29<F>))), dim3(256), 0, s, g, msm_acc_wg_log<F>(), st.counts, st.seg_off,
                      b.seg_sum, b.giant, b.giant + 2, b.giant_cap);
   hipLaunchKernelGGL(msm_giant_fold_kernel<F>, dim3(64), dim3(64), 0, s, g, msm_acc_wg_log<F>(), st.counts, st.seg_off,
                      b.seg_sum, b.buckets, b.giant, b.giant + 2, b.giant_cap);
@@ -566,16 +601,25 @@
   if (k_log) {
     const unsigned nsr_log = g.log_nb - k_log - CH_LL;
     DG_REQUIRE(nsr_log <= 8, DG16_ERR_UNSUPPORTED, "row chunks: more than 256 per bucket-window");
-    hipLaunchKernelGGL((msm_rowchunk_kernel<F, CH_LANES>), dim3(1u << nsr_log, bwi), dim3(CH_LANES), 0, s, g.log_nb, k_log,
-                       b.buckets, b.fold);
+    const unsigned items = bwi << nsr_log, wgs = b.side.grid(items, 2 * CH_LANES * sizeof(XYZZ29<F>));
+    if (wgs < items)
+      hipLaunchKernelGGL((msm_rowchunk_items_kernel<F, CH_LANES>), dim3(wgs), dim3(CH_LANES), 0, s, g.log_nb, k_log,
+                         1u << nsr_log, bwi, b.buckets, b.fold);
+    else
+      hipLaunchKernelGGL((msm_rowchunk_kernel<F, CH_LANES>), dim3(1u << nsr_log, bwi), dim3(CH_LANES), 0, s, g.log_nb, k_log,
+                         b.buckets, b.fold);
     trace_point(s, "row (chunks)");
     tg.folded = 1;
     tg.per_log = CH_LL;
     tg.lanes = 1u << nsr_log;
     tg.final_log = k_log;
   } else {
-    hipLaunchKernelGGL(msm_row_kernel<F>, dim3(1u << b.rg.rows_log, bwi), dim3(256), 0, s, g, b.rg, b.buckets, b.row_w,
-                       b.row_r);
+    const unsigned wgs = b.side.grid((unsigned)b.nrows, 256 * sizeof(XYZZ29<F>));
+    if (wgs < b.nrows)
+      hipLaunchKernelGGL(msm_row_items_kernel<F>, dim3(wgs), dim3(256), 0, s, b.rg, b.nrows, b.buckets, b.row_w, b.row_r);
+    else
+      hipLaunchKernelGGL(msm_row_kernel<F>, dim3(1u << b.rg.rows_log, bwi), dim3(256), 0, s, g, b.rg, b.buckets, b.row_w,
+                         b.row_r);
     trace_point(s, "row");
     tg.folded = b.rg.rows_log > 8;
     tg.per_log = tg.folded ? b.rg.rows_log - 8 : 0;
diff --git a/distributed-groth16_amd/csrc/prover_impl.h b/distributed-groth16_amd/csrc/prover_impl.h
--- a/distributed-groth16_amd/csrc/prover_impl.h
+++ b/distributed-groth16_amd/csrc/prover_impl.h
@@ -282,10 +282,12 @@
     DG_HIP(hipStreamWaitEvent(side, ev[8], 0));
   }
 
-  MsmSort st_ab = msm_sort_on<Fr, CT::SCALAR_BITS>(side, k1.c, sc_ab, n_ab + 3, mont, true, pk.c_ab, pk.stride);
+  const SideCap cap = ctx->side_cap();
+  MsmSort st_ab = msm_sort_on<Fr, CT::SCALAR_BITS>(side, k1.c, sc_ab, n_ab + 3, mont, true, pk.c_ab, pk.stride, cap.scaled(4));
   DG_HIP(hipEventRecord(ev[13], side));
   MsmBuffers<Fq2> buf_b2 = msm_buffers<Fq2>(k2.c, st_ab.g);
   buf_b2.busy_chip = true;
+  buf_b2.side = cap;
 
   if (dist) {
     const void* rows_in[3] = {a_dev, b_dev, c_dev};
@@ -300,7 +302,7 @@
     DG_HIP(hipEventRecord(ev[14], main));
     DG_HIP(hipStreamWaitEvent(side, ev[14], 0));
     if (tail_fence) DG_HIP(hipStreamWaitEvent(side, ev[18], 0));
-    st_h = msm_sort_on<Fr, CT::SCALAR_BITS>(side, k0.c, h_scalars, n_h, true, true, pk.c_h, pk.stride);
+    st_h = msm_sort_on<Fr, CT::SCALAR_BITS>(side, k0.c, h_scalars, n_h, true, true, pk.c_h, pk.stride, cap);
     DG_HIP(hipEventRecord(ev[15], side));
   }
 
@@ -332,6 +334,7 @@
   if (abl_merged) {
     MsmBuffers<Fq> buf3 = msm_buffers<Fq>(k0.c, st_ab.g, 3);
     buf3.busy_chip = true;
+    buf3.side = cap;
     const void* bases3[3] = {pk.a_q, pk.b1_q, pk.l_q};
     static_assert(kRecA == 0 && kRecB1 == 1 && kRecL == 2, "the three results land back to back in the record");
     DG_HIP(hipEventRecord(k1.c.ev[2], main));
@@ -356,6 +359,7 @@
     MsmBuffers<Fq> buf_b1 = msm_buffers<Fq>(k1.c, st_ab.g);
     MsmBuffers<Fq> buf_l = msm_buffers<Fq>(ctx->xws[1], st_ab.g);
     buf_a.busy_chip = buf_b1.busy_chip = buf_l.busy_chip = true;
+    buf_a.side = buf_b1.side = buf_l.side = cap;
     msm_accumulate_phase<Fq>(main, st_ab, buf_a, pk.a_q);
     DG_HIP(hipEventRecord(ev[0], main));
     DG_HIP(hipEventRecord(k1.c.ev[2], main));
@@ -388,7 +392,7 @@
     DG_HIP(hipStreamWaitEvent(main, ev[11], 0));
     h_poly_dist_stage(k0, CURVE, log_m, rank, n_ranks, 2, in2, h_dev);
     if (tail_fence) DG_HIP(hipStreamWaitEvent(main, ev[18], 0));
-    st_h = msm_sort_on<Fr, CT::SCALAR_BITS>(main, k0.c, h_dev, n_h, true, true, pk.c_h, pk.stride);
+    st_h = msm_sort_on<Fr, CT::SCALAR_BITS>(main, k0.c, h_dev, n_h, true, true, pk.c_h, pk.stride, SideCap{});
   } else {
     DG_HIP(hipStreamWaitEvent(main, ev[15], 0));
   }
```

New measurement: 110.1 million constraints/s (median of 5 runs). No clear change (+0.3%).
